# tangjiapeng/DiffuScene

Hardware: AMD Instinct MI355X
Metric: denoiser steps/sec (train + 1000-step sample) at B=256, N=80 objects (higher is better)
Workload: dtype f32 (operands split 3xbf16, 6 products, f32 accumulate); 1 GPU; uncond living/dining rooms (config/uncond/diffusion_livingrooms_instancond_lat32_v.yaml scaled to N=80), B=256 scenes per GPU, N=80, C=65, T=1000, mode=both; global_batch=256, parallelism=single

## Files before the change

__graft_entry__.py:

```python
import os
import subprocess
import sys

ROOT = os.path.dirname(os.path.abspath(__file__))
CSRC = os.path.join(ROOT, "diffuscene_amd", "csrc")
LIB = os.path.join(ROOT, "diffuscene_amd", "libdiffuscene_hip.so")

SOURCES = [
    ("gemm_mfma.hip", []),
    ("gemm_split.hip", ["-fno-slp-vectorize"]),
    ("gemm_tn_split.hip", ["-fno-slp-vectorize"]),
    ("blocks.hip", []),
    ("diffusion.hip", ["-ffp-contract=off"]),
    ("train.hip", []),
    ("retrieval.hip", ["-ffp-contract=off"]),
    ("dataset.hip", ["-ffp-contract=off"]),
    ("chamfer.hip", ["-ffp-contract=off"]),
    ("optim.hip", ["-ffp-contract=off"]),
    ("foldingnet.hip", []),
]


def _hipcc():
    for c in (os.environ.get("HIPCC"), "/opt/rocm/bin/hipcc", "hipcc"):
        if c and (os.path.isabs(c) and os.path.exists(c) or not os.path.isabs(c)):
            return c
    raise RuntimeError("hipcc not found")


def _stale(target, deps):
    if not os.path.exists(target):
        return True
    t = os.path.getmtime(target)
    return any(os.path.getmtime(d) > t for d in deps)


def _stamp_git_head():
    try:
        head = subprocess.check_output(["git", "rev-parse", "--short", "HEAD"], cwd=ROOT, stderr=subprocess.DEVNULL, text=True).strip()
        dirty = subprocess.check_output(["git", "status", "--porcelain", "-uno"], cwd=ROOT, stderr=subprocess.DEVNULL, text=True).strip()
        with open(os.path.join(ROOT, "GIT_HEAD"), "w") as f:
            f.write(head + ("+" if dirty else "") + "\n")
    except Exception:
        pass


def build(force=False):
    hipcc = _hipcc()
    headers = [os.path.join(CSRC, "dsc_common.h"), os.path.join(CSRC, "gemm_core.h"), os.path.join(CSRC, "gemm_tn_split.h"),
               os.path.join(ROOT, "include", "diffuscene_hip.h")]
    objs = []
    for src, extra in SOURCES:
        s = os.path.join(CSRC, src)
        if not os.path.exists(s):
            continue
        o = os.path.join(CSRC, src.replace(".hip", ".o"))
        if force or _stale(o, [s] + headers):
            cmd = [hipcc, "--offload-arch=gfx950", "-O3", "-std=c++17", "-fPIC", "-c", s, "-o", o] + extra
            subprocess.check_call(cmd)
        objs.append(o)
    if force or _stale(LIB, objs):
        subprocess.check_call([hipcc, "--offload-arch=gfx950", "-shared", "-fPIC", "-o", LIB] + objs)
    gsrc = os.path.join(ROOT, "tools", "guard_alloc.cpp")
    gso = os.path.join(ROOT, "tools", "_build", "libdsc_guard_alloc.so")
    if os.path.exists(gsrc) and (force or _stale(gso, [gsrc])):
        os.makedirs(os.path.dirname(gso), exist_ok=True)
        try:
            subprocess.check_call([hipcc, "-O2", "-std=c++17", "-fPIC", "-shared", gsrc, "-o", gso])
        except (subprocess.CalledProcessError, OSError) as e:
            print("warning: guard allocator (tools/guard_alloc.cpp) not built: %s -- tests/test_gpu_guard.py will skip its allocator runs" % e,
                  file=sys.stderr)
    _stamp_git_head()
    if ROOT not in sys.path:
        sys.path.insert(0, ROOT)
    import diffuscene_amd
    from diffuscene_amd import _lib
    _lib.load()
    import oracle.ref_torch


def build_asan():
    hipcc = _hipcc()
    out = os.path.join(ROOT, "diffuscene_amd", "libdiffuscene_hip_asan.so")
    objs = []
    for src, extra in SOURCES:
        s = os.path.join(CSRC, src)
        o = os.path.join(CSRC, src.replace(".hip", ".asan.o"))
        subprocess.check_call([hipcc, "--offload-arch=gfx950", "-O1", "-g", "-std=c++17", "-fPIC", "-fsanitize=address", "-fno-gpu-sanitize",
                               "-shared-libsan", "-Wno-option-ignored", "-c", s, "-o", o] + extra)
        objs.append(o)
    subprocess.check_call([hipcc, "--offload-arch=gfx950", "-shared", "-fPIC", "-fsanitize=address", "-fno-gpu-sanitize", "-shared-libsan",
                           "-Wno-option-ignored", "-o", out] + objs)
    return out


def smoke():
    if ROOT not in sys.path:
        sys.path.insert(0, ROOT)
    import torch
    assert torch.cuda.is_available(), "smoke() needs a GPU"
    from diffuscene_amd.networks.denoise_net import Unet1D
    from diffuscene_amd.networks.diffusion_ddpm import DiffusionPoint
    from oracle import ref_torch as R
    from oracle import weights as W

    kw = dict(W.UNCOND_BEDROOM)
    B, N = 4, 12
    dev = torch.device("cuda:0")
    net = Unet1D(**kw)
    sd = W.synth_state_dict(kw)
    net.load_state_dict(sd)
    net.to(dev)
    cfg = dict(objectness_dim=0, class_dim=22, angle_dim=2, objfeat_dim=32)
    diff = DiffusionPoint(net, cfg, time_num=1000, model_mean_type="v")
    x = W.synth_scene_batch(B, N, 22, 32, 0)
    t = torch.tensor([3, 250, 600, 999], dtype=torch.int64)
    cond = W.synth_condition(B, N, 128, 0).contiguous()
    noise = W.synth_noise((B, N, 62), 7)
    with torch.no_grad():
        out = net(x.to(dev), t.to(dev), cond.to(dev), None).cpu()
        ref = R.unet1d_forward(sd, kw, x, t, cond, None)
        rel = float((out - ref).abs().max() / ref.abs().max())
        assert rel < 1e-4, "Unet1D forward mismatch vs oracle: %g" % rel
        tb = R.schedule_tables(1e-4, 0.02, 1000, "v")
        step = diff.diffusion.p_sample(diff._denoise, x.to(dev), t.to(dev), cond.to(dev), None,
                                       noise_fn=lambda size, dtype, device: noise.to(device), clip_denoised=True).cpu()
        ref_step = R.p_sample_step(tb, x, t, ref, noise, True, "v")
        rel2 = float((step - ref_step).abs().max() / ref_step.abs().max())
        assert rel2 < 1e-4, "p_sample mismatch vs oracle: %g" % rel2
    print("smoke ok: forward rel err %.3g, p_sample rel err %.3g" % (rel, rel2))


if __name__ == "__main__":
    if "--asan" in sys.argv:
        print("built", build_asan())
        sys.exit(0)
    build(force="--force" in sys.argv)
    if "--smoke" in sys.argv:
        smoke()
```

diffuscene_amd/_lib.py:

```python
import ctypes as C
import os

_HERE = os.path.dirname(os.path.abspath(__file__))
LIB_PATH = os.path.join(_HERE, "libdiffuscene_hip.so")
if os.environ.get("DSC_HIP_LIB"):
    LIB_PATH = os.path.abspath(os.environ["DSC_HIP_LIB"])

ACT_NONE, ACT_GELU, ACT_SILU, ACT_LEAKY01 = 0, 1, 2, 3
SS_NONE, SS_PER_TOKEN, SS_PER_SCENE, SS_PER_SLOT, SS_BY_INDEX = 0, 1, 2, 3, 4
MEAN_EPS, MEAN_X0, MEAN_V = 0, 1, 2
TILE_GN_80_W8, TILE_GN_80_W4, TILE_160x256, TILE_160x128_W4 = 1, 2, 5, 8
TILE_WAVE_GN, TILE_WAVE_DENSE, TILE_WAVE_GN_64 = 10, 11, 12
F32_TILE_160x256, F32_TILE_160x128, F32_TILE_128x128, F32_TILE_96x128, F32_TILE_64x64 = 0, 1, 2, 3, 4
DSC_PLANES_NONE = -100
GEMM_ROW_INVARIANT = 1
WS_MAX = 64
MAX_TOKENS_PER_SCENE = 160
STATS_MAX_OBJECTS, STATS_ONE_WAVE_MAX = 160, 32

_ERR = {-1: "DSC_EINVAL (bad shape / null pointer)", -2: "DSC_EALIGN (16-byte alignment required)",
        -3: "DSC_ERANGE (size outside kernel limits)"}

c_f32p = C.c_void_p
c_i64p = C.c_void_p


class GemmArgs(C.Structure):
    _fields_ = [
        ("a1", C.c_void_p), ("lda1", C.c_int64), ("k1", C.c_int32),
        ("a2", C.c_void_p), ("lda2", C.c_int64), ("k2", C.c_int32),
        ("w", C.c_void_p), ("ldw", C.c_int64),
        ("bias", C.c_void_p),
        ("residual", C.c_void_p), ("ldr", C.c_int64),
        ("y", C.c_void_p), ("ldy", C.c_int64),
        ("m", C.c_int32), ("n", C.c_int32),
        ("act_in", C.c_int32), ("act_out", C.c_int32),
        ("batch", C.c_int32),
        ("sa1", C.c_int64), ("sa2", C.c_int64), ("sw", C.c_int64), ("sbias", C.c_int64),
        ("sres", C.c_int64), ("sy", C.c_int64),
        ("gamma", C.c_void_p), ("beta", C.c_void_p), ("eps", C.c_float),
        ("tokens_per_scene", C.c_int32),
        ("scale_shift", C.c_void_p), ("ld_ss", C.c_int64), ("ss_mode", C.c_int32),
        ("preact", C.c_void_p), ("ld_preact", C.c_int64),
        ("ss_index", C.c_void_p),
        ("w_planes", C.c_void_p),
        ("actgrad_x", C.c_void_p), ("ld_actgrad", C.c_int64),
        ("ss_rows", C.c_int32),
        ("w_planes_layout", C.c_int32),
        ("gnb_z", C.c_void_p), ("ld_gnb_z", C.c_int64),
        ("gnb_dgamma", C.c_void_p), ("gnb_dbeta", C.c_void_p), ("gnb_dbias", C.c_void_p), ("gnb_pstride", C.c_int64),
        ("gnb_dss", C.c_void_p), ("ld_gnb_dss", C.c_int64),
        ("flags", C.c_int32),
    ]


class SplitItem(C.Structure):
    _fields_ = [("w", C.c_void_p), ("ldw", C.c_int64), ("rows", C.c_int32), ("cols", C.c_int32), ("planes", C.c_void_p),
                ("transpose", C.c_int32)]


class SmallKItem(C.Structure):
    _fields_ = [("x", C.c_void_p), ("ldx", C.c_int64), ("k_in", C.c_int32), ("w", C.c_void_p), ("ldw", C.c_int64), ("bias", C.c_void_p),
                ("y", C.c_void_p), ("ldy", C.c_int64)]


class ColSpan(C.Structure):
    _fields_ = [("src_col", C.c_int32), ("dst_col", C.c_int32), ("width", C.c_int32)]


SMALLK_MAX = 4


class WsItem(C.Structure):
    _fields_ = [("w", C.c_void_p), ("out", C.c_void_p), ("rows", C.c_int32), ("cols", C.c_int32)]


class TnGroup(C.Structure):
    _fields_ = [("a1", C.c_void_p), ("lda1", C.c_int64), ("k1", C.c_int32),
                ("a2", C.c_void_p), ("lda2", C.c_int64), ("k2", C.c_int32),
                ("dy", C.c_void_p), ("ldd", C.c_int64),
                ("out", C.c_void_p), ("ldo", C.c_int64),
                ("dbias", C.c_void_p),
                ("m", C.c_int32), ("n", C.c_int32), ("kvalid", C.c_int32),
                ("tile0", C.c_int32),
                ("ws_offset", C.c_int64),
                ("tile0s", C.c_int32)]


class ColsumItem(C.Structure):
    _fields_ = [("x", C.c_void_p), ("ldx", C.c_int64), ("m", C.c_int32), ("n", C.c_int32), ("out", C.c_void_p)]


class WsBwdItem(C.Structure):
    _fields_ = [("w", C.c_void_p), ("dw_std", C.c_void_p), ("dw", C.c_void_p), ("rows", C.c_int32), ("cols", C.c_int32)]


SIGNATURES = {
    "dsc_version": (C.c_int, []),
    "dsc_gemm_f32": (C.c_int, [C.POINTER(GemmArgs), C.c_void_p]),
    "dsc_gemm_gn_silu_f32": (C.c_int, [C.POINTER(GemmArgs), C.c_void_p]),
    "dsc_split_bf16x3_f32": (C.c_int, [C.POINTER(SplitItem), C.c_int32, C.c_void_p]),
    "dsc_gemm_arithmetic": (C.c_int, [C.POINTER(GemmArgs), C.c_int32]),
    "dsc_gemm_split_tile": (C.c_int, [C.POINTER(GemmArgs), C.c_int32]),
    "dsc_gemm_f32_tile": (C.c_int, [C.POINTER(GemmArgs)]),
    "dsc_gemm_planes_layout": (C.c_int, [C.POINTER(GemmArgs), C.c_int32]),
    "dsc_get_split_wave": (C.c_int, []),
    "dsc_set_split_wave": (C.c_int, [C.c_int32]),
    "dsc_gemm_skinny": (C.c_int, [C.POINTER(GemmArgs), C.c_int32]),
    "dsc_get_skinny": (C.c_int, []),
    "dsc_set_skinny": (C.c_int, [C.c_int32]),
    "dsc_get_gemm_arithmetic": (C.c_int, []),
    "dsc_set_gemm_arithmetic": (C.c_int, [C.c_int32]),
    "dsc_gemm_layernorm_f32": (C.c_int, [C.POINTER(GemmArgs), C.c_void_p]),
    "dsc_gemm_splitk_f32": (C.c_int, [C.POINTER(GemmArgs), C.c_int32, c_f32p, C.c_int64, C.c_void_p]),
    "dsc_linear_smallk_f32": (C.c_int, [c_f32p, C.c_int64, C.c_int32, c_f32p, C.c_int64, c_f32p, c_f32p, C.c_int64,
                                        C.c_int32, C.c_int32, C.c_int32, C.c_void_p]),
    "dsc_linear_smallk_grouped_f32": (C.c_int, [C.POINTER(SmallKItem), C.c_int32, C.c_int32, C.c_int32, C.c_int32, C.c_void_p]),
    "dsc_gather_columns_f32": (C.c_int, [c_f32p, C.c_int64, c_f32p, C.c_int64, C.c_int32, C.POINTER(ColSpan), C.c_int32, C.c_void_p]),
    "dsc_weight_standardize_f32": (C.c_int, [C.POINTER(WsItem), C.c_int32, C.c_float, C.c_void_p]),
    "dsc_layernorm_f32": (C.c_int, [c_f32p, C.c_int64, c_f32p, c_f32p, C.c_int64, c_f32p, C.c_int64, C.c_int32,
                                    C.c_int32, C.c_float, C.c_void_p]),
    "dsc_linear_attention_f32": (C.c_int, [c_f32p, C.c_int64, c_f32p, C.c_int64, c_f32p, C.c_int64, c_f32p, C.c_int64,
                                           C.c_int32, C.c_int32, C.c_int32, C.c_float, C.c_void_p]),
    "dsc_attention_f32": (C.c_int, [c_f32p, C.c_int64, c_f32p, C.c_int64, c_f32p, C.c_int64, c_f32p, C.c_int64,
                                    C.c_int32, C.c_int32, C.c_float, C.c_void_p]),
    "dsc_time_embedding_f32": (C.c_int, [c_i64p, C.c_int32, C.c_int32, c_f32p, C.c_int32, c_f32p, c_f32p, C.c_void_p]),
    "dsc_activation_f32": (C.c_int, [c_f32p, c_f32p, C.c_int64, C.c_int32, C.c_void_p]),
    "dsc_q_sample_f32": (C.c_int, [c_f32p, c_f32p, c_i64p, c_f32p, c_f32p, c_f32p, c_f32p, C.c_int32, C.c_int64, C.c_int32,
                                   C.c_void_p]),
    "dsc_p_sample_f32": (C.c_int, [c_f32p, c_f32p, c_f32p, c_i64p, c_f32p, c_f32p, c_f32p, c_f32p, c_f32p, c_f32p,
                                   c_f32p, C.c_int32, C.c_int32, C.c_int32, C.c_int64, C.c_int32, C.c_void_p]),
    "dsc_device_error_count": (C.c_int64, [C.c_int32]),
    "dsc_add_scalar_i64": (C.c_int, [c_i64p, C.c_int32, C.c_int64, C.c_void_p]),
    "dsc_ddim_step_f32": (C.c_int, [c_f32p, c_f32p, c_f32p, c_i64p, c_i64p, c_i64p, c_f32p, c_f32p, c_f32p, c_f32p, c_f32p,
                                    c_f32p, c_f32p, c_f32p, c_f32p, C.c_int32, C.c_int32, C.c_int64, C.c_int32, C.c_int32,
                                    C.c_void_p]),
    "dsc_ddim_advance_i64": (C.c_int, [c_i64p, c_i64p, c_i64p, C.c_int32, C.c_int32, C.c_void_p]),
    "dsc_knn16_f32": (C.c_int, [c_f32p, C.c_int64, C.c_int32, c_f32p, c_f32p, C.c_int32, C.c_int32, C.c_void_p, C.c_void_p]),
    "dsc_rowsq_f32": (C.c_int, [c_f32p, C.c_int64, C.c_int32, C.c_int64, c_f32p, C.c_void_p]),
    "dsc_knn_cov_f32": (C.c_int, [c_f32p, C.c_int64, C.c_void_p, C.c_int32, C.c_int32, c_f32p, C.c_int64, C.c_void_p]),
    "dsc_gather_max_f32": (C.c_int, [c_f32p, C.c_int64, C.c_void_p, C.c_int32, C.c_int32, C.c_int32, c_f32p, C.c_int64,
                                     C.c_void_p, C.c_void_p]),
    "dsc_gather_max_bwd_f32": (C.c_int, [c_f32p, C.c_int64, C.c_void_p, C.c_void_p, C.c_int32, C.c_int32, C.c_int32, c_f32p,
                                         C.c_int64, C.c_void_p]),
    "dsc_bn_workspace_floats": (C.c_int64, [C.c_int64, C.c_int32]),
    "dsc_batchnorm_fwd_f32": (C.c_int, [c_f32p, C.c_int64, c_f32p, c_f32p, C.c_int64, C.c_int32, C.c_float, C.c_float,
                                        C.c_int32, c_f32p, c_f32p, c_f32p, c_f32p, c_f32p, c_f32p, c_f32p, C.c_int64,
                                        C.c_void_p]),
    "dsc_batchnorm_eval_f32": (C.c_int, [c_f32p, C.c_int64, c_f32p, c_f32p, c_f32p, c_f32p, C.c_int64, C.c_int32, C.c_int32,
                                         c_f32p, C.c_void_p]),
    "dsc_batchnorm_bwd_f32": (C.c_int, [c_f32p, c_f32p, c_f32p, c_f32p, c_f32p, C.c_int64, C.c_int32, C.c_int32, c_f32p,
                                        c_f32p, c_f32p, c_f32p, C.c_int64, C.c_void_p]),
    "dsc_rowmax_f32": (C.c_int, [c_f32p, C.c_int64, C.c_int32, C.c_int32, C.c_int32, c_f32p, C.c_void_p, C.c_void_p]),
    "dsc_rowmax_bwd_f32": (C.c_int, [c_f32p, C.c_void_p, C.c_int32, C.c_int32, C.c_int32, c_f32p, C.c_void_p]),
    "dsc_point_affine_f32": (C.c_int, [c_f32p, C.c_int64, C.c_int32, c_f32p, C.c_int64, c_f32p, C.c_int32, C.c_int32,
                                       C.c_int32, C.c_int32, c_f32p, C.c_void_p]),
    "dsc_point_affine_bwd_f32": (C.c_int, [c_f32p, c_f32p, C.c_int64, C.c_int32, c_f32p, C.c_int64, C.c_int32, C.c_int32,
                                           C.c_int32, C.c_int32, c_f32p, C.c_int64, c_f32p, C.c_int64, c_f32p, c_f32p,
                                           C.c_int64, C.c_void_p]),
    "dsc_postfilter_compact_f32": (C.c_int, [c_f32p, C.c_int32, C.c_int32, C.c_int32, C.c_int32, C.c_int32, C.c_int32, c_f32p,
                                             C.c_void_p, C.c_void_p]),
    "dsc_gemm_tn_f32": (C.c_int, [c_f32p, C.c_int64, C.c_int32, c_f32p, C.c_int64, C.c_int32, c_f32p, C.c_int64, c_f32p,
                                  C.c_int64, c_f32p, C.c_int32, C.c_int32, C.c_int32, c_f32p, C.c_int64, C.c_void_p]),
    "dsc_gemm_tn_workspace_floats": (C.c_int64, [C.c_int32, C.c_int32, C.c_int32]),
    "dsc_gemm_tn_grouped_f32": (C.c_int, [C.c_void_p, C.c_int32, C.c_int32, C.c_int32, c_f32p, C.c_int64, C.c_int64,
                                          C.c_void_p]),
    "dsc_gemm_tn_grouped_split_f32": (C.c_int, [C.c_void_p, C.c_int32, C.c_int32, C.c_void_p, C.c_int32, C.c_int32, c_f32p, C.c_int64,
                                                C.c_int64, C.c_int32, C.c_void_p]),
    "dsc_set_tn_split_form": (C.c_int, [C.c_int32]),
    "dsc_get_tn_split_form": (C.c_int, []),
    "dsc_colsum_f32": (C.c_int, [c_f32p, C.c_int64, C.c_int32, C.c_int32, c_f32p, c_f32p, C.c_int64, C.c_void_p]),
    "dsc_colsum_grouped_f32": (C.c_int, [C.c_void_p, C.c_int32, C.c_int32, C.c_void_p]),
    "dsc_gn_silu_bwd_f32": (C.c_int, [c_f32p, C.c_int64, c_f32p, C.c_int64, c_f32p, c_f32p, c_f32p, C.c_int64, C.c_int32,
                                      c_f32p, C.c_int64, c_f32p, c_f32p, c_f32p, C.c_int64, c_f32p, C.c_int64, C.c_int32,
                                      C.c_int32, C.c_int32, C.c_float, C.c_void_p]),
    "dsc_weight_standardize_bwd_f32": (C.c_int, [C.POINTER(WsBwdItem), C.c_int32, C.c_float, C.c_void_p]),
    "dsc_layernorm_bwd_f32": (C.c_int, [c_f32p, C.c_int64, c_f32p, c_f32p, C.c_int64, c_f32p, C.c_int64, c_f32p, C.c_int64, c_f32p,
                                        C.c_int32, C.c_int32, C.c_int32, C.c_float, C.c_void_p]),
    "dsc_linear_attention_bwd_f32": (C.c_int, [c_f32p, C.c_int64] * 7 + [C.c_int32, C.c_int32, C.c_int32, C.c_float,
                                                                          C.c_void_p]),
    "dsc_attention_bwd_f32": (C.c_int, [c_f32p, C.c_int64] * 7 + [C.c_int32, C.c_int32, C.c_float, C.c_void_p]),
    "dsc_retrieve_nearest_f32": (C.c_int, [c_f32p, C.c_void_p, C.c_void_p, c_f32p, C.c_void_p, C.c_void_p, C.c_int32,
                                           C.c_int32, C.c_int32, C.c_void_p, c_f32p, C.c_void_p]),
    "dsc_box_bounds_f32": (C.c_int, [c_f32p, c_f32p, c_f32p, C.c_void_p, C.c_int32, C.c_int32, c_f32p, C.c_void_p]),
    "dsc_scene_stats_f32": (C.c_int, [c_f32p, c_f32p, C.c_void_p, C.c_void_p, C.c_int32, C.c_int32, C.c_int32, C.c_int32,
                                      C.c_void_p, C.c_void_p, C.c_void_p, C.c_void_p, C.c_void_p, C.c_void_p, c_f32p, C.c_void_p]),
    "dsc_encode_scene_batch_f32": (C.c_int, [c_i64p, c_f32p, c_f32p, c_f32p, c_f32p, c_f32p, C.c_int32, C.c_int32, c_i64p,
                                             C.c_void_p, C.c_void_p, C.c_void_p, C.c_int32, C.POINTER(C.c_double), c_f32p,
                                             C.c_int64, c_i64p, C.c_int32, C.c_int32, C.c_void_p]),
    "dsc_chamfer3d_forward_f32": (C.c_int, [c_f32p, c_f32p, c_f32p, c_f32p, C.c_void_p, C.c_void_p, C.c_int32, C.c_int32,
                                            C.c_int32, C.c_void_p]),
    "dsc_chamfer3d_backward_f32": (C.c_int, [c_f32p, c_f32p, c_f32p, c_f32p, C.c_void_p, C.c_void_p, c_f32p, c_f32p,
                                             C.c_int32, C.c_int32, C.c_int32, C.c_void_p]),
    "dsc_grad_sumsq_f32": (C.c_int, [C.c_void_p, C.c_int32, C.c_void_p, C.c_void_p]),
    "dsc_clip_coef_f32": (C.c_int, [C.c_void_p, C.c_int32, C.c_float, c_f32p, c_f32p, C.c_void_p]),
    "dsc_adam_step_f32": (C.c_int, [C.c_void_p, C.c_int32, C.c_float, C.c_float, C.c_float, C.c_float, C.c_float, C.c_float,
                                    c_f32p, C.c_void_p]),
    "dsc_ddpm_loss_f32": (C.c_int, [c_f32p, c_f32p, c_f32p, c_i64p, c_f32p, c_f32p, c_f32p, c_f32p, C.POINTER(C.c_float),
                                    c_f32p, c_f32p, c_f32p] + [C.c_int32] * 12 + [C.c_float, C.c_int32, C.c_void_p]),
    "dsc_copy2d_f32": (C.c_int, [c_f32p, C.c_int64, c_f32p, C.c_int64, C.c_int32, C.c_int32, C.c_void_p]),
    "dsc_add2d_f32": (C.c_int, [c_f32p, C.c_int64, c_f32p, C.c_int64, C.c_int32, C.c_int32, C.c_void_p]),
    "dsc_activation_bwd_f32": (C.c_int, [c_f32p, c_f32p, c_f32p, C.c_int64, C.c_int32, C.c_void_p]),
    "dsc_transpose_batched_f32": (C.c_int, [C.POINTER(WsItem), C.c_int32, C.c_void_p]),
    "dsc_transpose_f32": (C.c_int, [c_f32p, C.c_int64, c_f32p, C.c_int64, C.c_int32, C.c_int32, C.c_void_p]),
    "dsc_complete_overwrite_f32": (C.c_int, [c_f32p, c_f32p, c_f32p, c_i64p, c_f32p, c_f32p, C.c_int32, C.c_int32,
                                             C.c_int32, C.c_int32, C.c_int32, C.c_void_p]),
    "dsc_complete_overwrite_ragged_f32": (C.c_int, [c_f32p, c_f32p, c_f32p, c_i64p, c_i64p, c_f32p, c_f32p, C.c_int32, C.c_int32,
                                                    C.c_int32, C.c_int32, C.c_int32, C.c_void_p]),
    "dsc_p_sample_inpaint_f32": (C.c_int, [c_f32p, c_f32p, c_f32p, c_f32p, c_f32p, c_i64p, c_i64p, c_f32p, c_f32p, c_f32p, c_f32p,
                                           c_f32p, c_f32p, c_f32p, c_f32p] + [C.c_int32] * 7 + [C.c_void_p]),
    "dsc_ddim_inpaint_step_f32": (C.c_int, [c_f32p] * 5 + [c_i64p] * 4 + [c_f32p] * 10 + [C.c_int32] * 7 + [C.c_void_p]),
    "dsc_masked_overwrite_f32": (C.c_int, [c_f32p, c_f32p, c_f32p, C.c_void_p, c_i64p, c_f32p, c_f32p, C.c_int32, C.c_int64, C.c_int32,
                                           C.c_void_p]),
    "dsc_p_sample_masked_f32": (C.c_int, [c_f32p] * 5 + [C.c_void_p, c_i64p] + [c_f32p] * 8 + [C.c_int32] * 3 + [C.c_int64, C.c_int32,
                                                                                                                  C.c_void_p]),
    "dsc_ddim_masked_step_f32": (C.c_int, [c_f32p] * 5 + [C.c_void_p] + [c_i64p] * 3 + [c_f32p] * 10 + [C.c_int32] * 2 +
                                 [C.c_int64, C.c_int32, C.c_int32, C.c_void_p]),
    "dsc_cfg_combine_f32": (C.c_int, [c_f32p, c_f32p, c_f32p, C.c_int32, C.c_int64, C.c_void_p]),
    "dsc_scene_randn_f32": (C.c_int, [c_f32p, c_i64p, c_i64p, C.c_int64, C.c_int64, C.c_int64, C.c_void_p]),
    "dsc_scene_philox_u32": (C.c_int, [C.c_void_p, c_i64p, c_i64p, C.c_int64, C.c_int64, C.c_int64, C.c_void_p]),
    "dsc_p_sample_cfg_f32": (C.c_int, [c_f32p] * 4 + [c_i64p] + [c_f32p] * 8 + [C.c_int32] * 3 + [C.c_int64, C.c_int32, C.c_void_p]),
    "dsc_ddim_cfg_step_f32": (C.c_int, [c_f32p] * 4 + [c_i64p] * 3 + [c_f32p] * 10 + [C.c_int32] * 2 +
                              [C.c_int64, C.c_int32, C.c_int32, C.c_void_p]),
    "dsc_scene_gate_f32": (C.c_int, [c_f32p, C.c_void_p, c_f32p, C.c_int32, C.c_int64, C.c_void_p]),
}

_lib = None


class HipLibraryMissing(RuntimeError):
    pass


def load():
    global _lib
    if _lib is not None:
        return _lib
    if not os.path.exists(LIB_PATH):
        raise HipLibraryMissing(
            "%s not found: build it with `python __graft_entry__.py` (hipcc --offload-arch=gfx950). "
            "diffuscene_amd has no CPU or PyTorch fallback." % LIB_PATH)
    import torch
    lib = C.CDLL(LIB_PATH)
    for name, (res, args) in SIGNATURES.items():
        try:
            fn = getattr(lib, name)
        except AttributeError as e:
            raise HipLibraryMissing("symbol %s missing from %s" % (name, LIB_PATH)) from e
        fn.restype = res
        fn.argtypes = args
    if lib.dsc_get_gemm_arithmetic() < 0:
        raise ValueError("DSC_GEMM=%r: must be 'split' (default) or 'f32'" % os.environ.get("DSC_GEMM"))
    if lib.dsc_get_tn_split_form() < 0:
        raise ValueError("DSC_TN_FORM=%r: must be '2' (default), '1' or '0'" % os.environ.get("DSC_TN_FORM"))
    if lib.dsc_get_split_wave() < 0:
        raise ValueError("DSC_WAVE=%r: must be '1' / 'auto' (default) or '0'" % os.environ.get("DSC_WAVE"))
    _lib = lib
    return lib


def split_enabled():
    return load().dsc_get_gemm_arithmetic() == 1


def gemm_mode():
    lib = load()
    if lib.dsc_get_gemm_arithmetic() != 1:
        return 0
    return (2 if lib.dsc_get_split_wave() == 1 else 1) + 10 * lib.dsc_get_tn_split_form()


def set_split_wave(on):
    prev = load().dsc_get_split_wave() == 1
    check(load().dsc_set_split_wave(1 if on else 0), "dsc_set_split_wave")
    return prev


def set_gemm_arithmetic(name):
    if name not in ("split", "f32"):
        raise ValueError("gemm arithmetic must be 'split' or 'f32', got %r" % (name,))
    prev = "split" if split_enabled() else "f32"
    check(load().dsc_set_gemm_arithmetic(1 if name == "split" else 0), "dsc_set_gemm_arithmetic")
    return prev


def device_error_count(reset=False):
    n = load().dsc_device_error_count(1 if reset else 0)
    if n < 0:
        raise RuntimeError("dsc_device_error_count failed (HIP error)")
    return int(n)


def check_indices(where):
    if os.environ.get("DSC_CHECK_INDICES", "0") == "1":
        n = device_error_count(reset=True)
        if n:
            raise IndexError("%s: %d out-of-range device timestep(s) were clamped into the schedule tables" % (where, n))


def check(rc, what):
    if rc != 0:
        raise RuntimeError("%s failed: %s" % (what, _ERR.get(rc, "hipError_t %d" % rc)))


def fn(name):
    return getattr(load(), name)
```

diffuscene_amd/csrc/gemm_mfma.hip:

```cpp
#include "gemm_core.h"
#include "gemm_skinny.h"
#include <cstdlib>

namespace {

using dsc_gemm::gemm_kernel;
constexpr int BK = 32;

int check_common(const dsc_gemm_args* a) {
    if (!a || !a->a1 || !a->w || !a->y) return DSC_EINVAL;
    if (a->m <= 0 || a->n <= 0 || a->k1 <= 0 || a->k2 < 0) return DSC_EINVAL;
    if ((a->k1 % BK) || (a->k2 % BK)) return DSC_EINVAL;
    if (a->k2 > 0 && !a->a2) return DSC_EINVAL;
    if (a->batch < 1) return DSC_EINVAL;
    if (!dsc_aligned16(a->a1) || (a->lda1 & 3) || !dsc_aligned16(a->w) || (a->ldw & 3)) return DSC_EALIGN;
    if (a->k2 > 0 && (!dsc_aligned16(a->a2) || (a->lda2 & 3))) return DSC_EALIGN;
    if (a->batch > 1 && ((a->sa1 & 3) || (a->sa2 & 3) || (a->sw & 3))) return DSC_EALIGN;
    if (a->act_in != DSC_ACT_NONE) return DSC_EINVAL;
    if (a->act_out < DSC_ACT_NONE || a->act_out > DSC_ACT_SILU) return DSC_EINVAL;
    return 0;
}

template <int TM, int TN, int WM, int WN, bool GN, int IL>
int launch_il(const dsc_gemm_args* a, int rows_per_blk, hipStream_t s) {
    constexpr int BN = 32 * TN * WN;
    const int nrb = (a->m + rows_per_blk - 1) / rows_per_blk;
    const int ncb = (a->n + BN - 1) / BN;
    dim3 grid((unsigned)(nrb * ncb), (unsigned)a->batch);
    DSC_CLEAR_STALE_ERROR();
    hipLaunchKernelGGL((gemm_kernel<TM, TN, WM, WN, GN, IL>), grid, dim3(64 * WM * WN), 0, s, *a, ncb);
    DSC_LAUNCH_CHECK();
    return 0;
}

template <int TM, int TN, int WM, int WN, bool GN, int IL = 1>
int launch(const dsc_gemm_args* a, int rows_per_blk, hipStream_t s) {
    if constexpr (IL == 0) {
        return launch_il<TM, TN, WM, WN, GN, 0>(a, rows_per_blk, s);
    } else {
        const int64_t ld_max = a->lda1 > a->ldw ? a->lda1 : a->ldw;
        const bool dma = (a->k2 == 0 || a->lda1 == a->lda2) && ld_max * 4 * (32 * TM * WM + 32 * TN * WN) < (int64_t(1) << 31);
        return dma ? launch_il<TM, TN, WM, WN, GN, 2>(a, rows_per_blk, s) : launch_il<TM, TN, WM, WN, GN, 1>(a, rows_per_blk, s);
    }
}

__global__ void splitk_reduce_kernel(const float* __restrict__ slabs, long slab, int nslab, const float* __restrict__ bias,
                                     const float* __restrict__ residual, long ldr, float* __restrict__ out, long ldo, int m, int n) {
    const long total = (long)m * n;
    for (long i = (long)blockIdx.x * blockDim.x + threadIdx.x; i < total; i += (long)gridDim.x * blockDim.x) {
        const int r = (int)(i / n), c = (int)(i - (long)r * n);
        float acc = 0.f;
        for (int s2 = 0; s2 < nslab; ++s2) acc += slabs[(long)s2 * slab + i];
        if (bias) acc += bias[c];
        if (residual) acc += residual[(long)r * ldr + c];
        out[(long)r * ldo + c] = acc;
    }
}

int g_skinny = -1;

int skinny_enabled() {
    if (g_skinny < 0) {
        const char* e = std::getenv("DSC_SKINNY");
        g_skinny = (e && e[0] == '0') ? 0 : 1;
    }
    return g_skinny;
}

struct SkinnyPlan { int rows_per_blk, ng, nrb, ncb; bool r16; };

bool skinny_plan(const dsc_gemm_args* a, bool gn, SkinnyPlan* out) {
    if (!skinny_enabled() || (a->flags & DSC_GEMM_ROW_INVARIANT)) return false;
    const int K = a->k1 + a->k2;
    if ((K % 64) || (a->n % 64)) return false;
    if (a->k2 > 0 && (a->k1 % (K / dsc_skinny::NW))) return false;
    if (a->preact && !gn) return false;
    if (a->actgrad_x || a->gnb_z) return false;
    int unit = 1;
    if (gn) {
        if (a->batch != 1) return false;
        unit = a->tokens_per_scene;
        if (unit > 32) return false;
    }
    const int ncb = a->n / 64;
    int rpb = 0;
    int64_t nrb = 0;
    bool r16 = false;
    for (int rows = ((K % 512) == 0 && unit <= 16) ? 16 : 32; rows <= 32 && !rpb; rows += 16) {
        int r = (rows / unit) * unit;
        if (r > a->m) r = (int)(((int64_t)a->m + unit - 1) / unit * unit);
        if (rows == 16 && r > 16) continue;
        const int64_t nb = ((int64_t)a->m + r - 1) / r;
        if (nb * ncb * a->batch <= 256) { rpb = r; nrb = nb; r16 = rows == 16; }
    }
    if (!rpb) return false;
    auto al = [](const void* q) { return !q || dsc_aligned16(q); };
    if (!al(a->y) || !al(a->residual) || !al(a->bias) || !al(a->preact) || !al(a->gamma) || !al(a->beta) || !al(a->scale_shift)) return false;
    if ((a->ldy & 3) || (a->residual && (a->ldr & 3)) || (a->preact && (a->ld_preact & 3)) || (a->scale_shift && (a->ld_ss & 3))) return false;
    if (a->batch > 1 && ((a->sy & 3) || (a->sres & 3) || (a->sbias & 3))) return false;
    out->rows_per_blk = rpb;
    out->r16 = r16;
    out->ng = (K % 512) == 0 ? dsc_skinny::STAGED : K <= 256 ? 1 : K <= 512 ? 2 : K <= 1024 ? 4 : 0;
    out->nrb = (int)nrb;
    out->ncb = ncb;
    return true;
}

template <bool GN, int NG, bool R16 = false>
int launch_skinny_ng(const dsc_gemm_args* a, const SkinnyPlan& sp, hipStream_t s) {
    static bool attr_set = false;
    if (!attr_set) {
        hipError_t e = hipFuncSetAttribute(reinterpret_cast<const void*>(dsc_skinny::gemm_skinny_kernel<GN, NG, R16>),
                                           hipFuncAttributeMaxDynamicSharedMemorySize, (int)dsc_skinny::lds_bytes<NG>());
        if (e != hipSuccess) return (int)e;
        attr_set = true;
    }
    DSC_CLEAR_STALE_ERROR();
    hipLaunchKernelGGL((dsc_skinny::gemm_skinny_kernel<GN, NG, R16>), dim3((unsigned)(sp.nrb * sp.ncb), (unsigned)a->batch),
                       dim3(64 * dsc_skinny::NW), dsc_skinny::lds_bytes<NG>(), s, *a, sp.ncb, sp.rows_per_blk);
    DSC_LAUNCH_CHECK();
    return 0;
}

template <bool GN>
int launch_skinny(const dsc_gemm_args* a, const SkinnyPlan& sp, hipStream_t s) {
    if (sp.r16) return launch_skinny_ng<GN, dsc_skinny::STAGED, true>(a, sp, s);
    switch (sp.ng) {
        case 1: return launch_skinny_ng<GN, 1>(a, sp, s);
        case 2: return launch_skinny_ng<GN, 2>(a, sp, s);
        case 4: return launch_skinny_ng<GN, 4>(a, sp, s);
        case dsc_skinny::STAGED: return launch_skinny_ng<GN, dsc_skinny::STAGED>(a, sp, s);
        default: return launch_skinny_ng<GN, 0>(a, sp, s);
    }
}

}

extern "C" int dsc_get_skinny(void) { return skinny_enabled(); }
extern "C" int dsc_set_skinny(int32_t on) { const int prev = skinny_enabled(); g_skinny = on ? 1 : 0; return prev; }
extern "C" int dsc_gemm_skinny(const dsc_gemm_args* a, int32_t gn) {
    if (check_common(a) || dsc_gemm_arithmetic(a, gn)) return 0;
    SkinnyPlan sp;
    return skinny_plan(a, gn != 0, &sp) ? (sp.r16 ? 2 : 1) : 0;
}

static long tile_cost(long m_rows, int rows_per_blk, int n, int bm, int bn) {
    const long nblk = ((m_rows + rows_per_blk - 1) / rows_per_blk) * ((n + bn - 1) / bn);
    return ((nblk + 255) / 256) * (long)bm * bn;
}

static int select_f32_tile(const dsc_gemm_args* a) {
    if (a->flags & DSC_GEMM_ROW_INVARIANT) return DSC_F32_TILE_64x64;
    const bool wide = (a->n % 256) == 0;
    struct Cand { int bm, bn, id; };
    const Cand cands[5] = {{160, 128, DSC_F32_TILE_160x128}, {160, 256, DSC_F32_TILE_160x256}, {128, 128, DSC_F32_TILE_128x128},
                           {96, 128, DSC_F32_TILE_96x128}, {64, 64, DSC_F32_TILE_64x64}};
    int best = -1;
    long best_cost = 0;
    for (int i = 0; i < 5; ++i) {
        if (cands[i].id == DSC_F32_TILE_160x256 && !wide) continue;
        const long c = tile_cost(a->m, cands[i].bm, a->n, cands[i].bm, cands[i].bn) * a->batch;
        if (best < 0 || c < best_cost) { best = cands[i].id; best_cost = c; }
    }
    return best;
}

extern "C" int dsc_gemm_f32_tile(const dsc_gemm_args* a) {
    const int rc = check_common(a);
    return rc ? rc : select_f32_tile(a);
}

extern "C" int dsc_gemm_f32(const dsc_gemm_args* a, dsc_stream_t stream) {
    int rc = check_common(a);
    if (rc) return rc;
    hipStream_t s = static_cast<hipStream_t>(stream);
    rc = dsc_gemm_try_split(a, false, s);
    if (rc != DSC_SPLIT_NOT_TAKEN) return rc;
    if (a->preact || a->actgrad_x || a->gnb_z) return DSC_EINVAL;
    {
        SkinnyPlan sp;
        if (skinny_plan(a, false, &sp)) return launch_skinny<false>(a, sp, s);
    }
    switch (select_f32_tile(a)) {
        case DSC_F32_TILE_160x256: return launch<5, 1, 1, 8, false>(a, 160, s);
        case DSC_F32_TILE_160x128: return launch<5, 1, 1, 4, false>(a, 160, s);
        case DSC_F32_TILE_128x128: return launch<2, 2, 2, 2, false>(a, 128, s);
        case DSC_F32_TILE_96x128: return launch<3, 1, 1, 4, false>(a, 96, s);
        default: return launch<1, 1, 2, 2, false, 0>(a, 64, s);
    }
}

extern "C" int dsc_gemm_gn_silu_f32(const dsc_gemm_args* a, dsc_stream_t stream) {
    int rc = check_common(a);
    if (rc) return rc;
    if (!a->gamma || !a->beta || !a->bias) return DSC_EINVAL;
    const int N = a->tokens_per_scene;
    if (N < 4 || N > 160) return DSC_ERANGE;
    if (a->m % N) return DSC_EINVAL;
    if (a->n % 128) return DSC_EINVAL;
    if (a->act_in != DSC_ACT_NONE) return DSC_EINVAL;
    if (!dsc_aligned16(a->gamma) || !dsc_aligned16(a->beta)) return DSC_EALIGN;
    if (a->preact && (!dsc_aligned16(a->preact) || (a->ld_preact & 3))) return DSC_EALIGN;
    if (a->ss_mode != DSC_SS_NONE) {
        if (!a->scale_shift) return DSC_EINVAL;
        if (!dsc_aligned16(a->scale_shift) || (a->ld_ss & 3)) return DSC_EALIGN;
        if (a->ss_mode < DSC_SS_NONE || a->ss_mode > DSC_SS_BY_INDEX) return DSC_EINVAL;
        if (a->ss_mode == DSC_SS_BY_INDEX && (!a->ss_index || a->ss_rows < 1)) return DSC_EINVAL;
    } else if (a->scale_shift) return DSC_EINVAL;
    hipStream_t s = static_cast<hipStream_t>(stream);
    rc = dsc_gemm_try_split(a, true, s);
    if (rc != DSC_SPLIT_NOT_TAKEN) return rc;
    {
        SkinnyPlan sp;
        if (skinny_plan(a, true, &sp)) return launch_skinny<true>(a, sp, s);
    }
    struct Cand { int bm, bn; };
    const Cand cands[5] = {{160, 128}, {160, 256}, {128, 128}, {96, 128}, {64, 64}};
    int best = -1;
    long best_cost = 0;
    const bool per_scene_ss = a->ss_mode == DSC_SS_PER_SCENE || a->ss_mode == DSC_SS_BY_INDEX;
    for (int pass = 0; pass < 2 && best < 0; ++pass)
        for (int i = 0; i < 5; ++i) {
            if (cands[i].bm < N) continue;
            if (cands[i].bn == 256 && (a->n % 256)) continue;
            if (pass == 0 && per_scene_ss && cands[i].bm / N > ((cands[i].bm == 160 && cands[i].bn == 128) ? 4 : 8)) continue;
            const int rpb = (cands[i].bm / N) * N;
            const long c = tile_cost(a->m, rpb, a->n, cands[i].bm, cands[i].bn);
            if (best < 0 || c < best_cost) { best = i; best_cost = c; }
        }
    if (best < 0) return DSC_ERANGE;
    const int rpb = (cands[best].bm / N) * N;
    switch (best) {
        case 0: return launch<5, 1, 1, 4, true>(a, rpb, s);
        case 1: return launch<5, 1, 1, 8, true>(a, rpb, s);
        case 2: return launch<2, 2, 2, 2, true>(a, rpb, s);
        case 3: return launch<3, 1, 1, 4, true>(a, rpb, s);
        default: return launch<1, 1, 2, 2, true, 0>(a, rpb, s);
    }
}

extern "C" int dsc_gemm_splitk_f32(const dsc_gemm_args* a, int32_t splits, float* workspace, int64_t workspace_floats,
                                   dsc_stream_t stream) {
    int rc = check_common(a);
    if (rc) return rc;
    if (splits < 2 || splits > 64 || !workspace) return DSC_EINVAL;
    if (a->batch != 1 || a->k2 != 0 || a->act_out != DSC_ACT_NONE) return DSC_EINVAL;
    if (a->k1 % (BK * splits)) return DSC_EINVAL;
    if (workspace_floats < (int64_t)splits * a->m * a->n) return DSC_EINVAL;
    if ((reinterpret_cast<uintptr_t>(workspace) & 15) || (((int64_t)a->m * a->n) & 3)) return DSC_EALIGN;
    dsc_gemm_args p = *a;
    const int kc = a->k1 / splits;
    p.k1 = kc;
    p.batch = splits;
    p.sa1 = kc; p.sw = kc; p.sa2 = 0; p.sbias = 0; p.sres = 0;
    p.bias = nullptr; p.residual = nullptr;
    p.y = workspace; p.ldy = a->n; p.sy = (int64_t)a->m * a->n;
    rc = dsc_gemm_f32(&p, stream);
    if (rc) return rc;
    const long total = (long)a->m * a->n;
    long blocks = (total + 255) / 256;
    if (blocks > 2048) blocks = 2048;
    DSC_CLEAR_STALE_ERROR();
    hipLaunchKernelGGL(splitk_reduce_kernel, dim3((unsigned)blocks), dim3(256), 0, static_cast<hipStream_t>(stream), workspace,
                       (long)a->m * a->n, splits, a->bias, a->residual, (long)a->ldr, a->y, (long)a->ldy, a->m, a->n);
    DSC_LAUNCH_CHECK();
    return 0;
}

extern "C" int dsc_gemm_layernorm_f32(const dsc_gemm_args* a, dsc_stream_t stream) {
    int rc = check_common(a);
    if (rc) return rc;
    if (a->n != 512 || a->batch != 1 || a->act_out != DSC_ACT_NONE || !a->gamma) return DSC_EINVAL;
    if (!dsc_aligned16(a->gamma) || !dsc_aligned16(a->y) || (a->ldy & 3)) return DSC_EALIGN;
    if (a->residual && (!dsc_aligned16(a->residual) || (a->ldr & 3))) return DSC_EALIGN;
    if (a->bias && !dsc_aligned16(a->bias)) return DSC_EALIGN;
    const int64_t ld_max = a->lda1 > a->ldw ? a->lda1 : a->ldw;
    if (!(a->k2 == 0 || a->lda1 == a->lda2) || ld_max * 4 * (96 + 512) >= (int64_t(1) << 31)) return DSC_ERANGE;
    const int nrb = (a->m + 95) / 96;
    DSC_CLEAR_STALE_ERROR();
    hipLaunchKernelGGL((gemm_kernel<3, 2, 1, 8, false, 2, 0, true>), dim3((unsigned)nrb, 1), dim3(512), 0,
                       static_cast<hipStream_t>(stream), *a, 1);
    DSC_LAUNCH_CHECK();
    return 0;
}
```

diffuscene_amd/csrc/gemm_split.hip:

```cpp
#include "dsc_common.h"
#include "gemm_split_wave.h"
#include <atomic>
#include <cstring>

#ifndef DSC_SPLIT_DSPREAD
#define DSC_SPLIT_DSPREAD true
#endif

namespace dsc_split {

typedef unsigned u32x4 __attribute__((ext_vector_type(4)));
typedef __bf16 bf16x8 __attribute__((ext_vector_type(8)));
typedef __bf16 bf16x2 __attribute__((ext_vector_type(2)));

constexpr int BK = 32;

__device__ __forceinline__ unsigned cvt_pk_bf16(float a, float b) {
    f32x2 v = {a, b};
    return __builtin_bit_cast(unsigned, __builtin_convertvector(v, bf16x2));
}
__device__ __forceinline__ float bf_lo(unsigned p) { return __builtin_bit_cast(float, p << 16); }
__device__ __forceinline__ float bf_hi(unsigned p) { return __builtin_bit_cast(float, p & 0xffff0000u); }

__device__ __forceinline__ void split8(const f32x4 lo, const f32x4 hi, bf16x8& p1, bf16x8& p2, bf16x8& p3) {
// ... 246 lines not shown
            if constexpr (DSPREAD) {
                if (i * PER < NI) {
#pragma unroll
                    for (int q = 0; q < PER; ++q) {
                        __builtin_amdgcn_sched_group_barrier(0x008, 2, 0);
                        __builtin_amdgcn_sched_group_barrier(0x020, 1, 0);
                    }
                }
            }
            if (i >= RB - NIT) {
#pragma unroll
                for (int q = 0; q < NMMA - 2; ++q) {
                    __builtin_amdgcn_sched_group_barrier(0x008, 1, 0);
                    __builtin_amdgcn_sched_group_barrier(0x002, (44 + NMMA - 3) / (NMMA - 2), 0);
                }
                __builtin_amdgcn_sched_group_barrier(0x008, 1, 0);
                __builtin_amdgcn_sched_group_barrier(0x200, 3, 0);
            }
            __builtin_amdgcn_sched_barrier(0);
        }
    }
    __builtin_amdgcn_s_waitcnt(0x0f70);

    const int cbase = col0 + wn * 64 + 4 * g;
    const int srow = wm * ntok;
    bool valid[RB];
#pragma unroll
    for (int i = 0; i < RB; ++i) valid[i] = i * 16 + l15 < ntok && srow + i * 16 + l15 < rows_here;
    float* const ob = p.y + (int64_t)z * p.sy + (int64_t)(row0 + srow + l15) * p.ldy + cbase;
    const float* const rbp = p.residual ? p.residual + (int64_t)z * p.sres + (int64_t)(row0 + srow + l15) * p.ldr + cbase : nullptr;
    if constexpr (!GN) {
        float* const ub = p.preact ? p.preact + (int64_t)z * p.sy + (int64_t)(row0 + srow + l15) * p.ld_preact + cbase : nullptr;
        const float* const gb = p.actgrad_x ? p.actgrad_x + (int64_t)z * p.sy + (int64_t)(row0 + srow + l15) * p.ld_actgrad + cbase : nullptr;
#pragma unroll
        for (int i = 0; i < RB; ++i) {
            if (valid[i]) {
#pragma unroll
                for (int j = 0; j < 4; ++j) {
                    f32x4 y = acc[i][j];
                    if (ub) *reinterpret_cast<f32x4*>(ub + (int64_t)i * 16 * p.ld_preact + j * 16) = y;
                    if (gb) {
                        const f32x4 u = *reinterpret_cast<const f32x4*>(gb + (int64_t)i * 16 * p.ld_actgrad + j * 16);
#pragma unroll
                        for (int e = 0; e < 4; ++e) y[e] *= dsc_act_grad(u[e], p.act_out);
                    } else if (p.act_out != DSC_ACT_NONE) {
#pragma unroll
                        for (int e = 0; e < 4; ++e) y[e] = dsc_act(y[e], p.act_out);
                    }
                    if (rbp) y += *reinterpret_cast<const f32x4*>(rbp + (int64_t)i * 16 * p.ldr + j * 16);
                    *reinterpret_cast<f32x4*>(ob + (int64_t)i * 16 * p.ldy + j * 16) = y;
                }
            }
        }
    } else {
        const int scene = min(row0 / ntok + wm, p.m / ntok - 1);
        const bool per_row = p.ss_mode == DSC_SS_PER_TOKEN || p.ss_mode == DSC_SS_PER_SLOT;
        f32x4 ga[4], be[4], sc[4], sh[4];
        int64_t ssrow = scene;
        if (p.ss_mode == DSC_SS_BY_INDEX) ssrow = dsc_clamp_index(p.ss_index[scene], p.ss_rows);
#pragma unroll
        for (int j = 0; j < 4; ++j) {
            ga[j] = *reinterpret_cast<const f32x4*>(p.gamma + cbase + j * 16);
            be[j] = *reinterpret_cast<const f32x4*>(p.beta + cbase + j * 16);
            if (p.ss_mode == DSC_SS_PER_SCENE || p.ss_mode == DSC_SS_BY_INDEX) {
                const float* ssr = p.scale_shift + ssrow * p.ld_ss + cbase + j * 16;
                sc[j] = *reinterpret_cast<const f32x4*>(ssr);
                sh[j] = *reinterpret_cast<const f32x4*>(ssr + p.n);
            } else {
                sc[j] = f32x4{0.f, 0.f, 0.f, 0.f};
                sh[j] = sc[j];
            }
        }
        if (p.preact) {
            float* const pb = p.preact + (int64_t)(row0 + srow + l15) * p.ld_preact + cbase;
#pragma unroll
            for (int i = 0; i < RB; ++i)
                if (valid[i]) {
#pragma unroll
                    for (int j = 0; j < 4; ++j) *reinterpret_cast<f32x4*>(pb + (int64_t)i * 16 * p.ld_preact + j * 16) = acc[i][j];
                }
        }
        const float inv_cnt = 1.f / (float)(ntok * 64);
        float s0 = 0.f;
#pragma unroll
        for (int i = 0; i < RB; ++i)
#pragma unroll
            for (int j = 0; j < 4; ++j)
                s0 += valid[i] ? (acc[i][j][0] + acc[i][j][1]) + (acc[i][j][2] + acc[i][j][3]) : 0.f;
        const float mean = wave_sum_dpp(s0) * inv_cnt;
        float q0 = 0.f;
#pragma unroll
        for (int i = 0; i < RB; ++i)
#pragma unroll
            for (int j = 0; j < 4; ++j)
#pragma unroll
                for (int e = 0; e < 4; ++e) {
                    const float d = valid[i] ? acc[i][j][e] - mean : 0.f;
                    q0 = fmaf(d, d, q0);
                }
        const float rstd = 1.f / sqrtf(wave_sum_dpp(q0) * inv_cnt + p.eps);
#pragma unroll
        for (int j = 0; j < 4; ++j)
#pragma unroll
            for (int e = 0; e < 4; ++e) {
                const float a = rstd * ga[j][e], sp1 = sc[j][e] + 1.f;
                ga[j][e] = a * sp1;
                be[j][e] = fmaf(be[j][e] - mean * a, sp1, sh[j][e]);
            }
#pragma unroll
        for (int i = 0; i < RB; ++i) {
            if (valid[i]) {
#pragma unroll
                for (int j = 0; j < 4; ++j) {
                    f32x4 y, s1 = {1.f, 1.f, 1.f, 1.f}, s2 = {0.f, 0.f, 0.f, 0.f};
                    if (per_row) {
                        const int64_t row = p.ss_mode == DSC_SS_PER_TOKEN ? (int64_t)row0 + srow + i * 16 + l15 : (int64_t)i * 16 + l15;
                        const float* ssr = p.scale_shift + row * p.ld_ss + cbase + j * 16;
                        s1 = *reinterpret_cast<const f32x4*>(ssr) + 1.f;
                        s2 = *reinterpret_cast<const f32x4*>(ssr + p.n);
                    }
#pragma unroll
                    for (int e = 0; e < 4; ++e) {
                        float t = fmaf(acc[i][j][e], ga[j][e], be[j][e]);
                        if (per_row) t = fmaf(t, s1[e], s2[e]);
                        y[e] = dsc_silu_fast(t);
                    }
                    if (rbp) y += *reinterpret_cast<const f32x4*>(rbp + (int64_t)i * 16 * p.ldr + j * 16);
                    *reinterpret_cast<f32x4*>(ob + (int64_t)i * 16 * p.ldy + j * 16) = y;
                }
            }
        }
    }
}

template <bool GN, int WM, int WN, int RB, bool DSPREAD = DSC_SPLIT_DSPREAD>
__global__ __launch_bounds__(64 * WM * WN, 1) void gemm_split_kernel(const dsc_gemm_args p, const int ntok) {
    __shared__ __attribute__((aligned(16))) char smem[split_smem_bytes<WM, WN, RB>()];
    gemm_split_tile<GN, WM, WN, RB, DSPREAD>(p, ntok, blockIdx.x, blockIdx.y, smem);
}

template <bool GN, int WM, int WN, int RB>
int launch(const dsc_gemm_args* a, int ntok, hipStream_t s) {
    constexpr int BN = 64 * WN;
    const int scenes = (a->m + ntok - 1) / ntok;
    const unsigned grid = (unsigned)(((scenes + WM - 1) / WM) * (a->n / BN));
    DSC_CLEAR_STALE_ERROR();
    hipLaunchKernelGGL((gemm_split_kernel<GN, WM, WN, RB>), dim3(grid, (unsigned)a->batch), dim3(64 * WM * WN), 0, s, *a, ntok);
    DSC_LAUNCH_CHECK();
    return 0;
}

}

enum { T_GN_32 = 0, T_GN_80_W8, T_GN_80_W4, T_GN_48, T_GN_64, T_160x256, T_256x128, T_128x128, T_160x128_W4, T_64x256, T_WAVE_GN, T_WAVE_DENSE, T_WAVE_GN_64 };

static std::atomic<int> g_gemm_arith{-1000};

extern "C" int dsc_get_gemm_arithmetic(void) {
    int m = g_gemm_arith.load(std::memory_order_relaxed);
    if (m == -1000) {
        const char* e = getenv("DSC_GEMM");
        m = (!e || !e[0] || !strcmp(e, "split")) ? 1 : !strcmp(e, "f32") ? 0 : DSC_EINVAL;
        g_gemm_arith.store(m, std::memory_order_relaxed);
    }
    return m;
}

extern "C" int dsc_set_gemm_arithmetic(int32_t mode) {
    if (mode != 0 && mode != 1) return DSC_EINVAL;
    g_gemm_arith.store(mode, std::memory_order_relaxed);
    return 0;
}

static std::atomic<int> g_split_wave{-1000};

extern "C" int dsc_get_split_wave(void) {
    int m = g_split_wave.load(std::memory_order_relaxed);
    if (m == -1000) {
        const char* e = getenv("DSC_WAVE");
        m = (!e || !e[0] || !strcmp(e, "1") || !strcmp(e, "auto")) ? 1 : !strcmp(e, "0") ? 0 : DSC_EINVAL;
        g_split_wave.store(m, std::memory_order_relaxed);
    }
    return m;
}

extern "C" int dsc_set_split_wave(int32_t mode) {
    if (mode != 0 && mode != 1) return DSC_EINVAL;
    g_split_wave.store(mode, std::memory_order_relaxed);
    return 0;
}

static int select_wave(const dsc_gemm_args* a, bool gn) {
    if (dsc_get_split_wave() != 1) return -1;
    const int K = a->k1 + a->k2;
    if ((a->n % 128) || (a->k1 % 64) || (a->k2 % 64) || K < 256) return -1;
    if (a->batch != 1 && (gn || a->sw != (int64_t)a->n * K || a->ldw != K || (a->sy & 3) || (a->sres & 3) || (a->sbias & 3))) return -1;
    if (!dsc_aligned16(a->y) || (a->ldy & 3) || a->ldy < a->n) return -1;
    if (a->bias && !dsc_aligned16(a->bias)) return -1;
    if (a->residual && (!dsc_aligned16(a->residual) || (a->ldr & 3) || a->ldr < a->n)) return -1;
    if (a->preact && (!dsc_aligned16(a->preact) || (a->ld_preact & 3) || a->ld_preact < a->n || a->batch != 1)) return -1;
    if (a->actgrad_x && (gn || !dsc_aligned16(a->actgrad_x) || (a->ld_actgrad & 3) || a->ld_actgrad < a->n || a->batch != 1)) return -1;
    if (3LL * a->batch * a->n * K * 2 >= 0x7fffffffLL) return -1;
    const int64_t ld_max = a->lda1 > a->lda2 ? a->lda1 : a->lda2;
    if (ld_max * 4 * 96 >= 0x7fffffffLL) return -1;
    long waves;
    if (a->gnb_z) {
        const int N = a->tokens_per_scene;
        if (gn || a->batch != 1 || N <= 64 || N > 80 || (a->m % N) || a->bias || a->residual || a->preact || a->actgrad_x || a->act_out != DSC_ACT_NONE) return -1;
        if (!a->gamma || !a->beta || !a->gnb_dgamma || !a->gnb_dbeta || !a->gnb_dbias || (a->ss_mode != DSC_SS_NONE && a->ss_mode != DSC_SS_PER_SCENE)) return -1;
        if (!dsc_aligned16(a->gnb_z) || (a->ld_gnb_z & 3) || a->ld_gnb_z < a->n || !dsc_aligned16(a->gamma) || !dsc_aligned16(a->beta)) return -1;
        if (!dsc_aligned16(a->gnb_dgamma) || !dsc_aligned16(a->gnb_dbeta) || !dsc_aligned16(a->gnb_dbias) || (a->gnb_pstride & 3)) return -1;
        if (a->ss_mode == DSC_SS_PER_SCENE && (!a->scale_shift || !dsc_aligned16(a->scale_shift) || (a->ld_ss & 3))) return -1;
        if (a->gnb_dss && (!dsc_aligned16(a->gnb_dss) || (a->ld_gnb_dss & 3))) return -1;
        waves = (long)(a->m / N) * (a->n / 128);
        const long r = (waves + 1023) / 1024;
        return waves * 5 >= r * 1024 * 4 ? T_WAVE_DENSE : -1;
    }
    if (gn) {
        const int N = a->tokens_per_scene;
        if (N <= 16 || N > 80) return -1;
        const bool perrow = a->ss_mode == DSC_SS_PER_TOKEN || a->ss_mode == DSC_SS_PER_SLOT;
        if (perrow && a->ld_ss < 2 * (int64_t)a->n) return -1;
        waves = (long)(a->m / N) * (a->n / 128);
    } else {
        waves = (long)((a->m + 79) / 80) * (a->n / 128) * a->batch;
    }
    const long rounds = (waves + 1023) / 1024;
    if (waves * 5 >= rounds * 1024 * 4) return gn ? T_WAVE_GN : T_WAVE_DENSE;
    if (gn && a->tokens_per_scene > 64) {
        const long w4 = 2 * waves, r4 = (w4 + 1023) / 1024;
        if (r4 == 1 && w4 * 5 >= 1024 * 4) return T_WAVE_GN_64;
    }
    return -1;
}

static int select_block_tile(const dsc_gemm_args* a, bool gn);

static int select_tile(const dsc_gemm_args* a, bool gn, bool assume_planes = false) {
    if (dsc_get_gemm_arithmetic() != 1 || (!assume_planes && !a->w_planes)) return -1;
    if (a->flags & DSC_GEMM_ROW_INVARIANT) return -1;
    const int w = select_wave(a, gn);
    return w >= 0 ? w : select_block_tile(a, gn);
}

static int select_block_tile(const dsc_gemm_args* a, bool gn) {
    if (a->gnb_z) return -1;
    const int K = a->k1 + a->k2;
    if (a->batch != 1 && (gn || a->sw != (int64_t)a->n * K || a->ldw != K || (a->sy & 3) || (a->sres & 3) || (a->sbias & 3))) return -1;
    if ((a->n % 128) || (K % 32)) return -1;
    if (!dsc_aligned16(a->w_planes) || !dsc_aligned16(a->y) || (a->ldy & 3)) return -1;
    if (a->bias && !dsc_aligned16(a->bias)) return -1;
    if (a->residual && (!dsc_aligned16(a->residual) || (a->ldr & 3))) return -1;
    if (!gn && a->preact && (!dsc_aligned16(a->preact) || (a->ld_preact & 3) || a->batch != 1)) return -1;
    if (a->actgrad_x && (gn || !dsc_aligned16(a->actgrad_x) || (a->ld_actgrad & 3) || a->batch != 1)) return -1;
    if (3LL * a->batch * a->n * K * 2 >= 0x7fffffffLL) return -1;
    const int64_t ld_max = a->lda1 > a->lda2 ? a->lda1 : a->lda2;
    if (ld_max * 4 * 320 >= 0x7fffffffLL) return -1;
    const bool wide = (a->n % 256) == 0;
    constexpr long MIN_BLOCKS = 160;
    if (gn) {
        const int N = a->tokens_per_scene;
        if (N <= 16 || N > 80) return -1;
        const long S = a->m / N;
        if (N <= 32) return ((S + 3) / 4) * (a->n / 128) >= MIN_BLOCKS ? T_GN_32 : -1;
        const long b8 = wide ? ((S + 1) / 2) * (a->n / 256) : 0, b4 = ((S + 1) / 2) * (a->n / 128);
        if (N > 64) return b8 >= MIN_BLOCKS + 32 ? T_GN_80_W8 : b4 >= MIN_BLOCKS ? T_GN_80_W4 : -1;
        if (b8 < MIN_BLOCKS) return -1;
        return N <= 48 ? T_GN_48 : T_GN_64;
    }
    struct Cand { int bm, bn, id; };
    const Cand cands[5] = {{160, 256, T_160x256}, {256, 128, T_256x128}, {160, 128, T_160x128_W4}, {128, 128, T_128x128}, {64, 256, T_64x256}};
    int best = -1;
    long best_cost = 0, best_blk = 0;
    for (int i = 0; i < 5; ++i) {
        if (cands[i].bn == 256 && !wide) continue;
        const long nblk = (long)((a->m + cands[i].bm - 1) / cands[i].bm) * (a->n / cands[i].bn) * a->batch;
        const long c = ((nblk + 255) / 256) * (long)cands[i].bm * cands[i].bn;
        if (best < 0 || c < best_cost) { best = cands[i].id; best_cost = c; best_blk = nblk; }
    }
    return best_blk >= MIN_BLOCKS ? best : -1;
}

int dsc_gemm_try_split(const dsc_gemm_args* a, bool gn, hipStream_t s) {
    using namespace dsc_split;
    if (dsc_get_gemm_arithmetic() < 0 || dsc_get_split_wave() < 0) return DSC_EINVAL;
    const int N = a->tokens_per_scene;
    const int tile = select_tile(a, gn);
    if (tile < 0) return DSC_SPLIT_NOT_TAKEN;
    const int want = (tile == T_WAVE_GN || tile == T_WAVE_DENSE || tile == T_WAVE_GN_64) ? DSC_PLANES_FRAGMENT : DSC_PLANES_ROWMAJOR;
    if (a->w_planes_layout != want) return DSC_EINVAL;
    switch (tile) {
        case T_GN_32: return launch<true, 4, 2, 2>(a, N, s);
        case T_GN_80_W8: return launch<true, 2, 4, 5>(a, N, s);
        case T_GN_80_W4: return launch<true, 2, 2, 5>(a, N, s);
        case T_GN_48: return launch<true, 2, 4, 3>(a, N, s);
        case T_GN_64: return launch<true, 2, 4, 4>(a, N, s);
        case T_160x256: return launch<false, 2, 4, 5>(a, 80, s);
        case T_256x128: return launch<false, 4, 2, 4>(a, 64, s);
        case T_128x128: return launch<false, 4, 2, 2>(a, 32, s);
        case T_160x128_W4: return launch<false, 2, 2, 5>(a, 80, s);
        case T_64x256: return launch<false, 2, 4, 2>(a, 32, s);
        case T_WAVE_DENSE:
            if (a->gnb_z) return dsc_wave::launch<false, 5, false, 8, true>(a, a->w_planes, N, s);
            return dsc_wave::launch<false, 5>(a, a->w_planes, 80, s);
        case T_WAVE_GN_64:
            return (a->ss_mode == DSC_SS_PER_TOKEN || a->ss_mode == DSC_SS_PER_SLOT) ? dsc_wave::launch<true, 5, true, 4>(a, a->w_planes, N, s)
                                                                                     : dsc_wave::launch<true, 5, false, 4>(a, a->w_planes, N, s);
        case T_WAVE_GN: {
            const bool perrow = a->ss_mode == DSC_SS_PER_TOKEN || a->ss_mode == DSC_SS_PER_SLOT;
            const int rb = (N + 15) / 16;
            if (perrow) {
                return rb == 5 ? dsc_wave::launch<true, 5, true>(a, a->w_planes, N, s) : rb == 4 ? dsc_wave::launch<true, 4, true>(a, a->w_planes, N, s)
                     : rb == 3 ? dsc_wave::launch<true, 3, true>(a, a->w_planes, N, s) : dsc_wave::launch<true, 2, true>(a, a->w_planes, N, s);
            }
            return rb == 5 ? dsc_wave::launch<true, 5>(a, a->w_planes, N, s) : rb == 4 ? dsc_wave::launch<true, 4>(a, a->w_planes, N, s)
                 : rb == 3 ? dsc_wave::launch<true, 3>(a, a->w_planes, N, s) : dsc_wave::launch<true, 2>(a, a->w_planes, N, s);
        }
        default: return DSC_SPLIT_NOT_TAKEN;
    }
}

extern "C" int dsc_gemm_arithmetic(const dsc_gemm_args* a, int32_t gn) {
    if (!a || a->m <= 0 || a->n <= 0 || a->k1 <= 0) return DSC_EINVAL;
    return select_tile(a, gn != 0) >= 0 ? 1 : 0;
}

extern "C" int dsc_gemm_split_tile(const dsc_gemm_args* a, int32_t gn) {
    if (!a || a->m <= 0 || a->n <= 0 || a->k1 <= 0) return DSC_EINVAL;
    return select_tile(a, gn != 0);
}

extern "C" int dsc_gemm_planes_layout(const dsc_gemm_args* a, int32_t gn) {
    if (!a || a->m <= 0 || a->n <= 0 || a->k1 <= 0) return DSC_EINVAL;
    const int tile = select_tile(a, gn != 0, true);
    return tile < 0 ? DSC_PLANES_NONE : (tile == T_WAVE_GN || tile == T_WAVE_DENSE || tile == T_WAVE_GN_64) ? DSC_PLANES_FRAGMENT : DSC_PLANES_ROWMAJOR;
}

extern "C" int dsc_split_bf16x3_f32(const dsc_split_item* items, int32_t count, dsc_stream_t stream) {
    using namespace dsc_split;
    if (!items || count < 1 || count > DSC_WS_MAX) return DSC_EINVAL;
    SplitBatch b;
    long max_items = 0;
    for (int i = 0; i < count; ++i) {
        const dsc_split_item& it = items[i];
        if (!it.w || !it.planes || it.rows <= 0 || it.cols <= 0) return DSC_EINVAL;
        if (it.transpose & ~(DSC_SPLIT_TRANSPOSE | DSC_SPLIT_FRAGMENT)) return DSC_EINVAL;
        const bool tr = (it.transpose & DSC_SPLIT_TRANSPOSE) != 0;
        const int co = tr ? it.rows : it.cols, ro = tr ? it.cols : it.rows;
        if (co % 8) return DSC_EINVAL;
        if ((it.transpose & DSC_SPLIT_FRAGMENT) && ((ro % 16) || (co % 32))) return DSC_EINVAL;
        if (!dsc_aligned16(it.planes) || (!tr && (!dsc_aligned16(it.w) || (it.ldw & 3)))) return DSC_EALIGN;
        b.it[i] = it;
        const long n = (long)it.rows * it.cols / 8;
        if (n > max_items) max_items = n;
    }
    long bx = (max_items + 255) / 256;
    if (bx > 1024) bx = 1024;
    DSC_CLEAR_STALE_ERROR();
    hipLaunchKernelGGL(split_planes_kernel, dim3((unsigned)bx, (unsigned)count), dim3(256), 0, static_cast<hipStream_t>(stream), b);
    DSC_LAUNCH_CHECK();
    return 0;
}
```

diffuscene_amd/csrc/gemm_split_wave.h:

```cpp
#pragma once
#include "dsc_common.h"
#include <utility>

#ifndef DSC_WAVE_STAMP_ARGS
#define DSC_WAVE_STAMP_ARGS
#define DSC_WAVE_STAMP_PASS
#define DSC_WAVE_STAMP_DECL
#define DSC_WAVE_STAMP_KERNEL(id)
#define DSC_WAVE_STAMP_TILE(id)
#define DSC_WAVE_STAMP_FLUSH(kt)
#define DSC_WAVE_STAMP_END
#endif

namespace dsc_wave {

typedef unsigned u32x4 __attribute__((ext_vector_type(4)));
typedef __bf16 bf16x8 __attribute__((ext_vector_type(8)));
typedef __bf16 bf16x2 __attribute__((ext_vector_type(2)));

constexpr int BK = 32;
constexpr int WAVES = 4;

__device__ __forceinline__ unsigned cvt_pk_bf16(float a, float b) {
    f32x2 v = {a, b};
    return __builtin_bit_cast(unsigned, __builtin_convertvector(v, bf16x2));
}
__device__ __forceinline__ float bf_lo(unsigned p) { return __builtin_bit_cast(float, p << 16); }
__device__ __forceinline__ float bf_hi(unsigned p) { return __builtin_bit_cast(float, p & 0xffff0000u); }

__device__ __forceinline__ void split8(const f32x4 lo, const f32x4 hi, bf16x8& p1, bf16x8& p2, bf16x8& p3) {
    u32x4 a, b, c;
#pragma unroll
    for (int q = 0; q < 4; ++q) {
        const float x0 = q < 2 ? lo[2 * q] : hi[2 * q - 4], x1 = q < 2 ? lo[2 * q + 1] : hi[2 * q - 3];
        const unsigned u1 = cvt_pk_bf16(x0, x1);
        const float r0 = x0 - bf_lo(u1), r1 = x1 - bf_hi(u1);
        const unsigned u2 = cvt_pk_bf16(r0, r1);
        const float s0 = r0 - bf_lo(u2), s1 = r1 - bf_hi(u2);
        a[q] = u1;
        b[q] = u2;
        c[q] = cvt_pk_bf16(s0, s1);
    }
    p1 = __builtin_bit_cast(bf16x8, a);
    p2 = __builtin_bit_cast(bf16x8, b);
    p3 = __builtin_bit_cast(bf16x8, c);
}

template <int RB>
constexpr int wave_smem_bytes() { return WAVES * 2 * 3 * (16 * RB) * 64; }

template <bool GN, int RB, bool PERROW = false, int J = 8, bool GB = false>
__global__ __launch_bounds__(64 * WAVES, 1) void gemm_split_wave_kernel(const dsc_gemm_args p, const uint16_t* const planes_f, const int ntok DSC_WAVE_STAMP_ARGS) {
    static_assert(J == 8 || J == 4, "wave tile: 128 or 64 channels");
    static_assert(!GB || (!GN && J == 8), "the GroupNorm-backward epilogue rides on the dense 80 x 128 form");
    constexpr int NWF = 3 * J;
    constexpr int CW = 16 * J;
    constexpr int ROWS = 16 * RB, XP = ROWS * 64, STAGE = 3 * XP;
    constexpr int NWB = RB > 4 ? RB - 2 : RB > 3 ? RB - 1 : RB;
    constexpr int PERW = (NWF + NWB - 1) / NWB;
    __shared__ __attribute__((aligned(16))) char smem[wave_smem_bytes<RB>()];
    const int lane = threadIdx.x & 63;
    const int wave = __builtin_amdgcn_readfirstlane(threadIdx.x >> 6);
    const int K = p.k1 + p.k2, KT = K / BK;
    const int scenes = (p.m + ntok - 1) / ntok;
    const int sgs = (scenes + WAVES - 1) / WAVES, chunks = p.n / CW;
    const int bid = blockIdx.x;
    int sg, ch;
    if ((sgs & 7) == 0) {
        const int xcd = bid & 7, idx = bid >> 3;
        sg = xcd * (sgs >> 3) + idx / chunks;
        ch = idx % chunks;
    } else {
        sg = bid / chunks;
        ch = bid % chunks;
    }
    const int scene = sg * WAVES + wave;
    if (scene >= scenes) return;
    DSC_WAVE_STAMP_DECL
    DSC_WAVE_STAMP_KERNEL(0)
    const int z = blockIdx.y;
    const int row0 = scene * ntok, col0 = ch * CW;
    const int rows_here = min(ntok, p.m - row0);
    const float* const xb1 = p.a1 + (int64_t)z * p.sa1 + (int64_t)row0 * p.lda1;
    const float* const xb2 = p.a2 ? p.a2 + (int64_t)z * p.sa2 + (int64_t)row0 * p.lda2 : xb1;
    const float* const bias = p.bias ? p.bias + (int64_t)z * p.sbias : nullptr;
    const int64_t rec1 = ((int64_t)(p.m - row0 - 1) * p.lda1 + p.k1) * 4;
    const int64_t rec2 = p.a2 ? ((int64_t)(p.m - row0 - 1) * p.lda2 + p.k2) * 4 : rec1;
    const int64_t recw = (int64_t)3 * p.batch * p.n * K * 2;
    const int64_t rec1c = rec1 < 0x7fffffffLL ? rec1 : 0x7fffffffLL, rec2c = rec2 < 0x7fffffffLL ? rec2 : 0x7fffffffLL;
#if defined(__HIP_DEVICE_COMPILE__)
    const __amdgpu_buffer_rsrc_t r1 = __builtin_amdgcn_make_buffer_rsrc(const_cast<float*>(xb1), 0, (int)rec1c, 0x00020000);
    const __amdgpu_buffer_rsrc_t r2 = __builtin_amdgcn_make_buffer_rsrc(const_cast<float*>(xb2), 0, (int)rec2c, 0x00020000);
#endif
#if defined(__HIP_DEVICE_COMPILE__)
    const __amdgpu_buffer_rsrc_t rw = __builtin_amdgcn_make_buffer_rsrc(const_cast<uint16_t*>(planes_f), 0, (int)recw, 0x00020000);
#endif
    const int plane_bytes = p.batch * p.n * K * 2;
    const int nb0 = (z * p.n + col0) / 16;

    const int q4 = lane & 3, r16 = lane >> 2, g = lane >> 4, l15 = lane & 15;
    const int tvo1 = (r16 * (int)p.lda1 + q4 * 8) * 4, tvo2 = (r16 * (int)p.lda2 + q4 * 8) * 4;
    const int ildso = r16 * 64 + ((q4 ^ ((r16 >> 1) & 3)) << 4);
    const int xoff = l15 * 64 + ((g ^ ((l15 >> 1) & 3)) << 4);
    const int wvo = lane * 16;
    char* const wl = smem + wave * (2 * STAGE);

    f32x4 acc[RB][J];
#pragma unroll
    for (int j = 0; j < J; ++j) {
        f32x4 b4 = {0.f, 0.f, 0.f, 0.f};
        if (bias) b4 = *reinterpret_cast<const f32x4*>(bias + col0 + j * 16 + 4 * g);
#pragma unroll
        for (int i = 0; i < RB; ++i) acc[i][j] = b4;
    }

    f32x4 ld[RB][2];
    bf16x8 wf[2][J][3], xf[2][3];
    const int lda2e = p.a2 ? (int)p.lda2 : (int)p.lda1, kshift = p.a2 ? p.k1 : 0;
    const int tvo2e = p.a2 ? tvo2 : tvo1;
    auto load_tok = [&](int kt, int u, auto segc) {
#if defined(__HIP_DEVICE_COMPILE__)
        constexpr int SEG = decltype(segc)::value;
        const int k0 = kt * BK;
        if constexpr (SEG == 0) {
            const int so = (u * 16 * (int)p.lda1 + k0) * 4;
            ld[u][0] = __builtin_bit_cast(f32x4, __builtin_amdgcn_raw_buffer_load_b128(r1, tvo1, so, 0));
            ld[u][1] = __builtin_bit_cast(f32x4, __builtin_amdgcn_raw_buffer_load_b128(r1, tvo1 + 16, so, 0));
        } else {
            const int so = (u * 16 * lda2e + k0 - kshift) * 4;
            ld[u][0] = __builtin_bit_cast(f32x4, __builtin_amdgcn_raw_buffer_load_b128(r2, tvo2e, so, 0));
            ld[u][1] = __builtin_bit_cast(f32x4, __builtin_amdgcn_raw_buffer_load_b128(r2, tvo2e + 16, so, 0));
        }
#else
        (void)kt; (void)u;
#endif
    };
    auto load_w = [&](int kt, int j, int pl) -> bf16x8 {
#if defined(__HIP_DEVICE_COMPILE__)
        return __builtin_bit_cast(bf16x8, __builtin_amdgcn_raw_buffer_load_b128(rw, wvo, pl * plane_bytes + ((nb0 + j) * KT + kt) * 1024, 0));
#else
        (void)kt; (void)j; (void)pl;
        return bf16x8{};
#endif
    };
    constexpr int NMMA = 6 * J;

    auto tile = [&](const int kt, auto curc, auto segc) {
        constexpr int CUR = decltype(curc)::value, NXT = CUR ^ 1;
        char* const cur = wl + CUR * STAGE;
        char* const nxt = wl + NXT * STAGE;
        const int kn1 = min(kt + 1, KT - 1), kn2 = min(kt + 2, KT - 1);
        constexpr int X0 = CUR ? (RB & 1) : 0;
        DSC_WAVE_STAMP_TILE(0)
        auto block = [&](auto ic) {
            constexpr int i = decltype(ic)::value;
            constexpr int NR = 3;
            constexpr int W0 = i * PERW < NWF ? i * PERW : NWF, W1 = (i + 1) * PERW < NWF ? (i + 1) * PERW : NWF;
            constexpr int VPS = J == 8 ? 2 : 4, NVS = 44 / VPS;
            constexpr int S0 = NR + (W1 - W0), S1 = S0 + NVS, S2 = S1 + 3, S3 = S2 + 1;
            static_assert(S3 <= NMMA, "one MFMA per filler slot");
            unsigned su1[4], su2[4], su3[4];
            float sr0[4], sr1[4], st0[4], st1[4];
            auto xin = [&](int q, int h) -> float { return q < 2 ? ld[i][0][2 * q + h] : ld[i][1][2 * q - 4 + h]; };
            auto split_op = [&](auto nc) {
                constexpr int n = decltype(nc)::value;
                constexpr int q = 2 * (n / 22) + (n & 1), o = (n % 22) >> 1;
                if constexpr (o == 0) su1[q] = cvt_pk_bf16(xin(q, 0), xin(q, 1));
                if constexpr (o == 1) st0[q] = bf_lo(su1[q]);
                if constexpr (o == 2) st1[q] = bf_hi(su1[q]);
                if constexpr (o == 3) sr0[q] = xin(q, 0) - st0[q];
                if constexpr (o == 4) sr1[q] = xin(q, 1) - st1[q];
                if constexpr (o == 5) su2[q] = cvt_pk_bf16(sr0[q], sr1[q]);
                if constexpr (o == 6) st0[q] = bf_lo(su2[q]);
                if constexpr (o == 7) st1[q] = bf_hi(su2[q]);
                if constexpr (o == 8) sr0[q] = sr0[q] - st0[q];
                if constexpr (o == 9) sr1[q] = sr1[q] - st1[q];
                if constexpr (o == 10) su3[q] = cvt_pk_bf16(sr0[q], sr1[q]);
            };
            char* const d0 = nxt + i * 1024 + ildso;
            auto filler = [&](auto kc) {
                constexpr int k = decltype(kc)::value;
                if constexpr (k < NR) {
                    if constexpr (i + 1 < RB) xf[(X0 + i + 1) & 1][k] = *reinterpret_cast<const bf16x8*>(cur + k * XP + (i + 1) * 1024 + xoff);
                    else xf[(X0 + i + 1) & 1][k] = *reinterpret_cast<const bf16x8*>(nxt + k * XP + xoff);
                } else if constexpr (k < S0) {
                    constexpr int w = W0 + (k - NR);
                    wf[NXT][w / 3][w % 3] = load_w(kn1, w / 3, w % 3);
                } else if constexpr (k < S1) {
                    dsc_static_for<VPS>([&](auto vc) { split_op(std::integral_constant<int, VPS * (k - S0) + decltype(vc)::value>{}); });
                } else if constexpr (k < S2) {
                    constexpr int pl = k - S1;
                    const u32x4 v = pl == 0 ? u32x4{su1[0], su1[1], su1[2], su1[3]} : pl == 1 ? u32x4{su2[0], su2[1], su2[2], su2[3]}
                                                                                              : u32x4{su3[0], su3[1], su3[2], su3[3]};
                    *reinterpret_cast<u32x4*>(d0 + pl * XP) = v;
                } else if constexpr (k == S2) {
                    load_tok(kn2, i, segc);
                }
            };
            auto product = [&](auto pc) {
                constexpr int pr = decltype(pc)::value;
                constexpr int wp = pr == 0 ? 2 : (pr == 1 || pr >= 4) ? 0 : 1;
                constexpr int xp = pr == 0 ? 0 : pr == 1 ? 2 : pr == 2 ? 1 : pr == 3 ? 0 : pr == 4 ? 1 : 0;
                dsc_static_for<J>([&](auto jc) {
                    constexpr int j = decltype(jc)::value;
                    acc[i][j] = __builtin_amdgcn_mfma_f32_16x16x32_bf16(wf[CUR][j][wp], xf[(X0 + i) & 1][xp], acc[i][j], 0, 0, 0);
                    filler(std::integral_constant<int, pr * J + j>{});
                    __builtin_amdgcn_sched_barrier(0);
                });
            };
            dsc_static_for<6>(product);
            DSC_WAVE_STAMP_TILE(1 + i)
        };
        dsc_static_for<RB>(block);
        DSC_WAVE_STAMP_FLUSH(kt)
    };

    using std::integral_constant;
#pragma unroll
    for (int u = 0; u < RB; ++u) load_tok(0, u, integral_constant<int, 0>{});
#pragma unroll
    for (int w = 0; w < NWF; ++w) wf[0][w / 3][w % 3] = load_w(0, w / 3, w % 3);
#pragma unroll
    for (int u = 0; u < RB; ++u) {
        bf16x8 a, b, c;
        split8(ld[u][0], ld[u][1], a, b, c);
        char* d0 = wl + u * 1024 + ildso;
        *reinterpret_cast<bf16x8*>(d0) = a;
        *reinterpret_cast<bf16x8*>(d0 + XP) = b;
        *reinterpret_cast<bf16x8*>(d0 + 2 * XP) = c;
        load_tok(1, u, integral_constant<int, 0>{});
    }
#pragma unroll
    for (int pl = 0; pl < 3; ++pl) xf[0][pl] = *reinterpret_cast<const bf16x8*>(wl + pl * XP + xoff);
    const int KT1 = p.k1 / BK;
    int kt = 0;
    DSC_WAVE_STAMP_KERNEL(1)
    for (; kt + 2 < KT1; kt += 2) {
        tile(kt, integral_constant<int, 0>{}, integral_constant<int, 0>{});
        tile(kt + 1, integral_constant<int, 1>{}, integral_constant<int, 0>{});
    }
    f32x4 ep_ga[2], ep_be[2], ep_sc[2], ep_sh[2];
    if constexpr (GN) {
        const bool per_scene_e = p.ss_mode == DSC_SS_PER_SCENE || p.ss_mode == DSC_SS_BY_INDEX;
        int64_t ssrow_e = scene;
        if (p.ss_mode == DSC_SS_BY_INDEX) ssrow_e = dsc_clamp_index(p.ss_index[scene], p.ss_rows);
#pragma unroll
        for (int c2 = 0; c2 < J / 4; ++c2) {
            const int ch = col0 + 64 * c2 + 4 * (lane & 15);
            ep_ga[c2] = *reinterpret_cast<const f32x4*>(p.gamma + ch);
            ep_be[c2] = *reinterpret_cast<const f32x4*>(p.beta + ch);
            ep_sc[c2] = f32x4{0.f, 0.f, 0.f, 0.f};
            ep_sh[c2] = ep_sc[c2];
            if (per_scene_e) {
                const float* ssr = p.scale_shift + ssrow_e * p.ld_ss + ch;
                ep_sc[c2] = *reinterpret_cast<const f32x4*>(ssr);
                ep_sh[c2] = *reinterpret_cast<const f32x4*>(ssr + p.n);
            }
        }
    }
    for (; kt < KT; kt += 2) {
        tile(kt, integral_constant<int, 0>{}, integral_constant<int, 1>{});
        tile(kt + 1, integral_constant<int, 1>{}, integral_constant<int, 1>{});
    }

    DSC_WAVE_STAMP_KERNEL(2)
    constexpr int ERS = 64 * 4 + 16;
    static_assert(ROWS * ERS <= 2 * STAGE, "the transposed cell fits the wave's LDS image");
    const int er = lane >> 4, ec = lane & 15;
#if defined(__HIP_DEVICE_COMPILE__)
    auto row_rsrc = [&](const float* base, int64_t ld, int rows, int cols) {
        return __builtin_amdgcn_make_buffer_rsrc(const_cast<float*>(base), 0, rows > 0 ? (int)(((int64_t)(rows - 1) * ld + cols) * 4) : 0, 0x00020000);
    };
    const __amdgpu_buffer_rsrc_t ry = row_rsrc(p.y + (int64_t)z * p.sy + (int64_t)row0 * p.ldy, p.ldy, rows_here, p.n);
    const __amdgpu_buffer_rsrc_t rr = row_rsrc(p.residual ? p.residual + (int64_t)z * p.sres + (int64_t)row0 * p.ldr : p.y, p.ldr, p.residual ? rows_here : 0, p.n);
    const __amdgpu_buffer_rsrc_t rpa = row_rsrc(p.preact ? p.preact + (int64_t)z * p.sy + (int64_t)row0 * p.ld_preact : p.y, p.ld_preact, p.preact ? rows_here : 0, p.n);
    auto ld4 = [&](const __amdgpu_buffer_rsrc_t& r, int voff, int soff) { return __builtin_bit_cast(f32x4, __builtin_amdgcn_raw_buffer_load_b128(r, voff, soff, 0)); };
    auto st4 = [&](const f32x4 v, const __amdgpu_buffer_rsrc_t& r, int voff, int soff) { __builtin_amdgcn_raw_buffer_store_b128(__builtin_bit_cast(u32x4, v), r, voff, soff, 0); };
#else
    const int ry = 0, rr = 0, rpa = 0;
    auto ld4 = [&](int, int, int) { return f32x4{}; };
    auto st4 = [&](const f32x4, int, int, int) {};
#endif
    const bool has_res = p.residual != nullptr, has_pre = p.preact != nullptr;
    auto to_lds = [&](const int c2) {
#pragma unroll
        for (int i = 0; i < RB; ++i)
#pragma unroll
            for (int j = 0; j < 4; ++j) *reinterpret_cast<f32x4*>(wl + (i * 16 + l15) * ERS + (j * 16 + 4 * g) * 4) = acc[i][4 * c2 + j];
    };
    constexpr int NQ = ROWS / 4, QH = NQ % 10 == 0 ? 10 : NQ % 8 == 0 ? 8 : NQ % 6 == 0 ? 6 : 4;
    static_assert(NQ % QH == 0, "row groups per pass");
    if constexpr (GB) {
        const float inv_cnt = 1.f / (float)(ntok * 64);
        const bool per_scene = p.ss_mode == DSC_SS_PER_SCENE && p.scale_shift;
#if defined(__HIP_DEVICE_COMPILE__)
        const __amdgpu_buffer_rsrc_t rz = row_rsrc(p.gnb_z + (int64_t)row0 * p.ld_gnb_z, p.ld_gnb_z, rows_here, p.n);
#else
        const int rz = 0;
#endif
        dsc_static_for<2>([&](auto c2c) {
            constexpr int c2 = decltype(c2c)::value;
            const int ch = col0 + 64 * c2 + 4 * ec, cc = ch * 4;
            const int vy = er * (int)p.ldy * 4 + cc, vz = er * (int)p.ld_gnb_z * 4 + cc;
            f32x4 zv[NQ], dv[NQ];
#pragma unroll
            for (int q = 0; q < NQ; ++q) zv[q] = ld4(rz, vz, 4 * q * (int)p.ld_gnb_z * 4);
            const f32x4 ga = *reinterpret_cast<const f32x4*>(p.gamma + ch), be = *reinterpret_cast<const f32x4*>(p.beta + ch);
            f32x4 s1 = {1.f, 1.f, 1.f, 1.f}, sh = {0.f, 0.f, 0.f, 0.f};
            if (per_scene) {
                const float* ssr = p.scale_shift + (int64_t)scene * p.ld_ss + ch;
                s1 = *reinterpret_cast<const f32x4*>(ssr) + 1.f;
                sh = *reinterpret_cast<const f32x4*>(ssr + p.n);
            }
            to_lds(c2);
            float s = 0.f;
#pragma unroll
            for (int q = 0; q < NQ; ++q) {
                dv[q] = *reinterpret_cast<const f32x4*>(wl + (4 * q + er) * ERS + ec * 16);
                const bool ok = 4 * q + er < rows_here;
                if (!ok) dv[q] = f32x4{0.f, 0.f, 0.f, 0.f};
                s += ok ? (zv[q][0] + zv[q][1]) + (zv[q][2] + zv[q][3]) : 0.f;
            }
            const float mu = wave_sum_dpp(s) * inv_cnt;
            s = 0.f;
#pragma unroll
            for (int q = 0; q < NQ; ++q) {
                const bool ok = 4 * q + er < rows_here;
#pragma unroll
                for (int e = 0; e < 4; ++e) { const float d = ok ? zv[q][e] - mu : 0.f; s = fmaf(d, d, s); }
            }
            const float rs = 1.0f / sqrtf(wave_sum_dpp(s) * inv_cnt + p.eps);
            float S1 = 0.f, S2 = 0.f;
            f32x4 Gg = {0.f, 0.f, 0.f, 0.f}, Gb = Gg, Gsc = Gg, Gsh = Gg, Gz = Gg;
#pragma unroll
            for (int q = 0; q < NQ; ++q) {
#pragma unroll
                for (int e = 0; e < 4; ++e) {
                    const float xh = (zv[q][e] - mu) * rs;
                    const float gh = ga[e] * xh + be[e];
                    const float u = gh * s1[e] + sh[e];
                    const float sig = __builtin_amdgcn_rcpf(1.0f + __expf(-u));
                    const float du = dv[q][e] * (sig * (1.0f + u * (1.0f - sig)));
                    const float dgh = du * s1[e];
                    const float dxh = dgh * ga[e];
                    S1 += dxh; S2 += dxh * xh;
                    Gg[e] += dgh * xh; Gb[e] += dgh; Gsc[e] += du * gh; Gsh[e] += du;
                    zv[q][e] = xh;
                    dv[q][e] = dxh;
                }
            }
            const float m1 = wave_sum_dpp(S1) * inv_cnt, m2 = wave_sum_dpp(S2) * inv_cnt;
#pragma unroll
            for (int q = 0; q < NQ; ++q) {
                const bool ok = 4 * q + er < rows_here;
                f32x4 dzv;
#pragma unroll
                for (int e = 0; e < 4; ++e) { dzv[e] = rs * (dv[q][e] - m1 - zv[q][e] * m2); Gz[e] += ok ? dzv[e] : 0.f; }
                st4(dzv, ry, vy, 4 * q * (int)p.ldy * 4);
            }
            auto fold = [&](f32x4 v) {
#pragma unroll
                for (int e = 0; e < 4; ++e) { v[e] += __shfl_xor(v[e], 16, 64); v[e] += __shfl_xor(v[e], 32, 64); }
                return v;
            };
            Gg = fold(Gg); Gb = fold(Gb); Gz = fold(Gz);
            if (per_scene && p.gnb_dss) { Gsc = fold(Gsc); Gsh = fold(Gsh); }
            if (lane < 16) {
                const int64_t o = (int64_t)scene * p.gnb_pstride + ch;
                *reinterpret_cast<f32x4*>(p.gnb_dgamma + o) = Gg;
                *reinterpret_cast<f32x4*>(p.gnb_dbeta + o) = Gb;
                *reinterpret_cast<f32x4*>(p.gnb_dbias + o) = Gz;
                if (per_scene && p.gnb_dss) {
                    *reinterpret_cast<f32x4*>(p.gnb_dss + (int64_t)scene * p.ld_gnb_dss + ch) = Gsc;
                    *reinterpret_cast<f32x4*>(p.gnb_dss + (int64_t)scene * p.ld_gnb_dss + p.n + ch) = Gsh;
                }
            }
        });
    } else if constexpr (!GN) {
#if defined(__HIP_DEVICE_COMPILE__)
        const __amdgpu_buffer_rsrc_t rg = row_rsrc(p.actgrad_x ? p.actgrad_x + (int64_t)z * p.sy + (int64_t)row0 * p.ld_actgrad : p.y, p.ld_actgrad, p.actgrad_x ? rows_here : 0, p.n);
#else
        const int rg = 0;
#endif
        auto cell = [&](auto c2c, auto modec, auto actc) {
            constexpr int c2 = decltype(c2c)::value, MODE = decltype(modec)::value, ACT = decltype(actc)::value;
            const int cc = (col0 + 64 * c2 + 4 * ec) * 4;
            const int vy = er * (int)p.ldy * 4 + cc, vr = er * (int)p.ldr * 4 + cc, vp = er * (int)p.ld_preact * 4 + cc, vg = er * (int)p.ld_actgrad * 4 + cc;
            to_lds(c2);
#pragma unroll 1
            for (int h = 0; h < NQ; h += QH) {
                f32x4 rres[QH], gx[QH];
                if (has_res) {
#pragma unroll
                    for (int qq = 0; qq < QH; ++qq) rres[qq] = ld4(rr, vr, 4 * (h + qq) * (int)p.ldr * 4);
                }
                if constexpr (MODE == 2) {
#pragma unroll
                    for (int qq = 0; qq < QH; ++qq) gx[qq] = ld4(rg, vg, 4 * (h + qq) * (int)p.ld_actgrad * 4);
                }
#pragma unroll
                for (int qq = 0; qq < QH; ++qq) {
                    f32x4 y = *reinterpret_cast<const f32x4*>(wl + (4 * (h + qq) + er) * ERS + ec * 16);
                    if (has_pre) st4(y, rpa, vp, 4 * (h + qq) * (int)p.ld_preact * 4);
#pragma unroll
                    for (int e = 0; e < 4; ++e) {
                        if constexpr (MODE == 1) y[e] = dsc_act(y[e], ACT);
                        if constexpr (MODE == 2) y[e] *= dsc_act_grad(gx[qq][e], ACT);
                    }
                    if (has_res) y += rres[qq];
                    st4(y, ry, vy, 4 * (h + qq) * (int)p.ldy * 4);
                }
            }
        };
        auto cells = [&](auto modec, auto actc) {
            cell(std::integral_constant<int, 0>{}, modec, actc);
            if constexpr (J == 8) cell(std::integral_constant<int, 1>{}, modec, actc);
        };
        using std::integral_constant;
        const int act = p.act_out;
        if (p.actgrad_x) {
            if (act == DSC_ACT_GELU) cells(integral_constant<int, 2>{}, integral_constant<int, DSC_ACT_GELU>{});
            else if (act == DSC_ACT_SILU) cells(integral_constant<int, 2>{}, integral_constant<int, DSC_ACT_SILU>{});
            else if (act == DSC_ACT_LEAKY01) cells(integral_constant<int, 2>{}, integral_constant<int, DSC_ACT_LEAKY01>{});
            else cells(integral_constant<int, 0>{}, integral_constant<int, DSC_ACT_NONE>{});
        } else {
            if (act == DSC_ACT_GELU) cells(integral_constant<int, 1>{}, integral_constant<int, DSC_ACT_GELU>{});
            else if (act == DSC_ACT_SILU) cells(integral_constant<int, 1>{}, integral_constant<int, DSC_ACT_SILU>{});
            else if (act == DSC_ACT_LEAKY01) cells(integral_constant<int, 1>{}, integral_constant<int, DSC_ACT_LEAKY01>{});
            else cells(integral_constant<int, 0>{}, integral_constant<int, DSC_ACT_NONE>{});
        }
    } else {
#if defined(__HIP_DEVICE_COMPILE__)
        const __amdgpu_buffer_rsrc_t rs = row_rsrc(PERROW ? p.scale_shift + (p.ss_mode == DSC_SS_PER_TOKEN ? (int64_t)row0 * p.ld_ss : 0) : p.y, p.ld_ss,
                                                   PERROW ? rows_here : 0, 2 * p.n);
#else
        const int rs = 0;
#endif
        const float inv_cnt = 1.f / (float)(ntok * 64);
        const bool vlast = (RB - 1) * 16 + l15 < rows_here;
#pragma unroll
        for (int c2 = 0; c2 < J / 4; ++c2) {
            const int ch = col0 + 64 * c2 + 4 * ec;
            const f32x4 ga = ep_ga[c2], be = ep_be[c2], sc = ep_sc[c2], sh = ep_sh[c2];
            to_lds(c2);
            float s0 = 0.f;
#pragma unroll
            for (int i = 0; i < RB; ++i)
#pragma unroll
                for (int j = 0; j < 4; ++j) {
                    const f32x4 a = acc[i][4 * c2 + j];
                    const float t = (a[0] + a[1]) + (a[2] + a[3]);
                    s0 += (i < RB - 1 || vlast) ? t : 0.f;
                }
            const float mean = wave_sum_dpp(s0) * inv_cnt;
            float q0 = 0.f;
#pragma unroll
            for (int i = 0; i < RB; ++i)
#pragma unroll
                for (int j = 0; j < 4; ++j)
#pragma unroll
                    for (int e = 0; e < 4; ++e) {
                        const float d = (i < RB - 1 || vlast) ? acc[i][4 * c2 + j][e] - mean : 0.f;
                        q0 = fmaf(d, d, q0);
                    }
            const float rstd = 1.f / sqrtf(wave_sum_dpp(q0) * inv_cnt + p.eps);
            if (c2 == 0) { DSC_WAVE_STAMP_KERNEL(3) }
            f32x4 A, B;
#pragma unroll
            for (int e = 0; e < 4; ++e) {
                const float a = rstd * ga[e], sp1 = sc[e] + 1.f;
                A[e] = a * sp1;
                B[e] = fmaf(be[e] - mean * a, sp1, sh[e]);
            }
            const int cc = ch * 4;
            const int vy = er * (int)p.ldy * 4 + cc, vr = er * (int)p.ldr * 4 + cc, vp = er * (int)p.ld_preact * 4 + cc, vs = er * (int)p.ld_ss * 4 + cc;
            if (c2 == 0) { DSC_WAVE_STAMP_KERNEL(4) }
#pragma unroll
            for (int h = 0; h < NQ; h += QH) {
                f32x4 rres[QH], s1[QH], s2[QH];
                if (has_res) {
#pragma unroll
                    for (int qq = 0; qq < QH; ++qq) rres[qq] = ld4(rr, vr, 4 * (h + qq) * (int)p.ldr * 4);
                }
                if constexpr (PERROW) {
#pragma unroll
                    for (int qq = 0; qq < QH; ++qq) {
                        s1[qq] = ld4(rs, vs, 4 * (h + qq) * (int)p.ld_ss * 4);
                        s2[qq] = ld4(rs, vs + p.n * 4, 4 * (h + qq) * (int)p.ld_ss * 4);
                    }
                }
#pragma unroll
                for (int qq = 0; qq < QH; ++qq) {
                    const f32x4 zv = *reinterpret_cast<const f32x4*>(wl + (4 * (h + qq) + er) * ERS + ec * 16);
                    if (has_pre) st4(zv, rpa, vp, 4 * (h + qq) * (int)p.ld_preact * 4);
                    f32x4 y;
#pragma unroll
                    for (int e = 0; e < 4; ++e) {
                        float t = fmaf(zv[e], A[e], B[e]);
                        if constexpr (PERROW) t = fmaf(t, s1[qq][e] + 1.f, s2[qq][e]);
                        y[e] = dsc_silu_fast(t);
                    }
                    if (has_res) y += rres[qq];
                    st4(y, ry, vy, 4 * (h + qq) * (int)p.ldy * 4);
                }
            }
            if (c2 == 0) { DSC_WAVE_STAMP_KERNEL(5) }
        }
    }
    DSC_WAVE_STAMP_END
}

template <bool GN, int RB, bool PERROW = false, int J = 8, bool GB = false>
int launch(const dsc_gemm_args* a, const uint16_t* planes_f, int ntok, hipStream_t s) {
    const int scenes = (a->m + ntok - 1) / ntok;
    const unsigned grid = (unsigned)(((scenes + WAVES - 1) / WAVES) * (a->n / (16 * J)));
    DSC_CLEAR_STALE_ERROR();
    hipLaunchKernelGGL((gemm_split_wave_kernel<GN, RB, PERROW, J, GB>), dim3(grid, (unsigned)a->batch), dim3(64 * WAVES), 0, s, *a, planes_f, ntok DSC_WAVE_STAMP_PASS);
    DSC_LAUNCH_CHECK();
    return 0;
}

}
```

diffuscene_amd/engine.py:

```python
import ctypes as C

import torch

from . import _lib, ops
from ._lib import ACT_GELU, ACT_NONE, ACT_SILU, SS_BY_INDEX, SS_NONE, SS_PER_SCENE, SS_PER_SLOT, SS_PER_TOKEN

D = 512
HID = 128
DEC_PAD = 32


def _own(t):
    if isinstance(t, torch.nn.Parameter):
        return t.detach()
    if isinstance(t, (tuple, list)):
        return tuple(_own(u) for u in t)
    return t


class StalePlanError(RuntimeError):
    pass


class _Pool:
# ... 14 lines not shown
        return t

    def put(self, t):
        self.free_list.setdefault((t.shape[0], t.shape[1]), []).append(t)


class Plan:

    def __init__(self, eng, B, N, ctx_mode, ctx_dim, L, text_dim, time_table=False):
        self.eng, self.B, self.N, self.M = eng, B, N, B * N
        self.generation = eng.generation
        dev = eng.device
        self.pool = _Pool(dev)
        self.keep = []
        self.steps = []
        self.pre_steps = []
        net = eng.net
        C_in = net.channels
        self.x_in = torch.empty((self.M, C_in), device=dev, dtype=torch.float32)
        self.t_in = torch.empty((B,), device=dev, dtype=torch.int64)
        ctx_rows = {SS_NONE: 0, SS_PER_SLOT: N, SS_PER_TOKEN: self.M}[ctx_mode]
        self.ctx_in = torch.empty((ctx_rows, ctx_dim), device=dev, dtype=torch.float32) if ctx_rows else None
        self.cross_in = torch.empty((B * L, text_dim), device=dev, dtype=torch.float32) if L else None
        self.ctx_mode = ctx_mode
        self.L = L
        self.time_table = time_table
        self.out = torch.empty((self.M, net.out_dim), device=dev, dtype=torch.float32)
        self._build()
        self.tiled_steps = self.steps

    def gemm_args(self):
        kinds = {id(_lib.fn("dsc_gemm_gn_silu_f32")): "gn", id(_lib.fn("dsc_gemm_f32")): "plain"}
        out = []
        for f, a in self.steps:
            k = kinds.get(id(f))
            if k is not None:
                out.append((k, a[0]._obj))
        return out

    def gemm(self, a, w, out, bias=None, a2=None, residual=None, act_in=ACT_NONE, act_out=ACT_NONE, row_invariant=False):
        g = ops.make_gemm_args(a, w, out, bias, a2, residual, act_in, act_out, row_invariant=row_invariant)
        lay = ops.planes_layout(g)
        pl = self.eng.planes_of(w, lay) if lay >= 0 else None
        if pl is not None:
            ops.attach_planes(g, pl, layout=lay)
        self.keep.append(_own((g, a, w, out, bias, a2, residual, pl)))
        self.steps.append((_lib.fn("dsc_gemm_f32"), (C.byref(g),)))
        return out

    def gemm_batched(self, a, w, out, bias, batch, sa, sw, sy, sbias, act_out=ACT_NONE):
        stacked = w._base if w._base is not None else w
        g = ops.make_gemm_args(a, w, out, bias, None, None, ACT_NONE, act_out)
        g.batch, g.sa1, g.sw, g.sy, g.sbias = batch, sa, sw, sy, sbias
        whole = (stacked.dim() == 2 and stacked.is_contiguous() and w.data_ptr() == stacked.data_ptr()
                 and stacked.shape[0] == batch * w.shape[0] and stacked.shape[1] == w.shape[1] and sw == w.shape[0] * w.shape[1])
        lay = ops.planes_layout(g) if whole else -1
        pl = self.eng.planes_of(stacked, lay) if lay >= 0 else None
        if pl is not None:
            ops.attach_planes(g, pl, layout=lay)
        self.keep.append(_own((g, a, w, out, bias, pl)))
        self.steps.append((_lib.fn("dsc_gemm_f32"), (C.byref(g),)))
        return out

    def gemm_gn(self, a, w, out, bias, gamma, beta, a2=None, ss=None, ss_mode=SS_NONE, residual=None):
        g = ops.make_gemm_args(a, w, out, bias, a2, residual, gamma=gamma, beta=beta, eps=1e-5,
                               tokens_per_scene=self.N, scale_shift=ss, ss_mode=ss_mode if ss is not None else SS_NONE,
                               ss_index=self.t_in if (ss is not None and ss_mode == SS_BY_INDEX) else None)
        lay = ops.planes_layout(g, gn=True)
        pl = self.eng.planes_of(w, lay) if lay >= 0 else None
        if pl is not None:
            ops.attach_planes(g, pl, gn=True, layout=lay)
        self.keep.append(_own((g, a, w, out, bias, a2, residual, gamma, beta, ss, pl)))
        self.steps.append((_lib.fn("dsc_gemm_gn_silu_f32"), (C.byref(g),)))
        return out

    def call(self, name, *args, keep=()):
        self.keep.append(_own(keep))
        self.steps.append((_lib.fn(name), args))

    def hoist(self, first):
        if self.time_table:
            self.pre_steps += self.steps[first:]
            del self.steps[first:]
            return True
        return False

    def check_current(self):
        if self.generation != self.eng.generation:
            raise StalePlanError("diffuscene_amd: this launch plan was built for parameter storages the model no longer uses (flat storage "
                                 "of the first training step, module.to(), load into new tensors): rebuild it -- DenoiserEngine.prepare() / "
                                 "graph_sample_loop() do -- instead of running or replaying it")

    def run_pre(self):
        self.check_current()
        s = ops.stream_ptr()
        for f, a in self.pre_steps:
            rc = f(*a, s)
            if rc:
                _lib.check(rc, f.__name__)

    def layernorm(self, x, g, out, residual=None):
        self.call("dsc_layernorm_f32", x.data_ptr(), x.stride(0), g.data_ptr(),
                  residual.data_ptr() if residual is not None else None,
                  residual.stride(0) if residual is not None else 0,
                  out.data_ptr(), out.stride(0), x.shape[0], x.shape[1], 1e-5, keep=(x, g, out, residual))
        return out

    def out_proj_ln(self, a, conv, ln_gain, residual):
        M = self.M
        out = self.pool.get(M, D)
        if (M + 95) // 96 >= 160:
            g = ops.make_gemm_args(a, conv.weight, out, conv.bias, None, residual, gamma=ln_gain.view(-1), beta=ln_gain.view(-1),
                                   eps=1e-5)
            self.keep.append(_own((g, a, conv.weight, out, conv.bias, residual, ln_gain)))
            self.steps.append((_lib.fn("dsc_gemm_layernorm_f32"), (C.byref(g),)))
            return out
        o = self.gemm(a, conv.weight, self.pool.get(M, D), conv.bias)
        self.layernorm(o, ln_gain, out, residual=residual)
        self.pool.put(o)
        return out

    def resblock(self, rb, x, x2, ss, ss_mode):
        e, M = self.eng, self.M
        h = self.pool.get(M, D)
        self.gemm_gn(x, e.ws[id(rb.block1.proj)], h, rb.block1.proj.bias, rb.block1.norm.weight, rb.block1.norm.bias,
                     a2=x2, ss=ss, ss_mode=ss_mode)
        if rb.has_res_conv:
            r = self.pool.get(M, D)
            self.gemm(x, rb.res_conv.weight, r, rb.res_conv.bias, a2=x2)
        else:
            r = x
        out = self.pool.get(M, D)
        self.gemm_gn(h, e.ws[id(rb.block2.proj)], out, rb.block2.proj.bias, rb.block2.norm.weight, rb.block2.norm.bias,
                     residual=r)
        self.pool.put(h)
        if rb.has_res_conv:
            self.pool.put(r)
        return out

    def t_ss(self, rb):
        i = self.eng.t_index[id(rb)]
        return self.ss_t[:, i * 2 * D:(i + 1) * 2 * D], (SS_BY_INDEX if self.time_table else SS_PER_SCENE)

    def c_ss(self, rb):
        if self.ss_c is None:
            return None, SS_NONE
        i = self.eng.c_index[id(rb)]
        return self.ss_c[:, i * 2 * D:(i + 1) * 2 * D], self.ctx_mode

    def linattn(self, blk, x):
        M, B, N = self.M, self.B, self.N
        att = blk.fn.fn
        y = self.layernorm(x, blk.fn.norm.g, self.pool.get(M, D))
        qkv = self.gemm(y, att.to_qkv.weight, self.pool.get(M, 3 * HID))
        self.pool.put(y)
        a = self.pool.get(M, HID)
        self.call("dsc_linear_attention_f32", qkv.data_ptr(), 3 * HID, qkv.data_ptr() + 4 * HID, 3 * HID,
                  qkv.data_ptr() + 8 * HID, 3 * HID, a.data_ptr(), HID, B, N, N, float(att.scale), keep=(qkv, a))
        self.pool.put(qkv)
        out = self.out_proj_ln(a, att.to_out[0], att.to_out[1].g, x)
        self.pool.put(a)
        return out

    def crossattn(self, blk, x):
        M, B, N, L = self.M, self.B, self.N, self.L
        att = blk.fn.fn
        y = self.layernorm(x, blk.fn.norm.g, self.pool.get(M, D))
        q = self.gemm(y, att.to_q.weight, self.pool.get(M, HID))
        self.pool.put(y)
        first = len(self.steps)
        kv = self.gemm(self.cross_in, att.to_kv.weight, self.pool.get(B * L, 2 * HID))
        kv_is_invariant = self.hoist(first)
        a = self.pool.get(M, HID)
        self.call("dsc_linear_attention_f32", q.data_ptr(), HID, kv.data_ptr(), 2 * HID, kv.data_ptr() + 4 * HID,
                  2 * HID, a.data_ptr(), HID, B, N, L, float(att.scale), keep=(q, kv, a))
        self.pool.put(q)
        if not kv_is_invariant:
            self.pool.put(kv)
        out = self.out_proj_ln(a, att.to_out[0], att.to_out[1].g, x)
        self.pool.put(a)
        return out

    def fullattn(self, blk, x):
        M, B, N = self.M, self.B, self.N
        att = blk.fn.fn
        y = self.layernorm(x, blk.fn.norm.g, self.pool.get(M, D))
        qkv = self.gemm(y, att.to_qkv.weight, self.pool.get(M, 3 * HID))
        self.pool.put(y)
        a = self.pool.get(M, HID)
        self.call("dsc_attention_f32", qkv.data_ptr(), 3 * HID, qkv.data_ptr() + 4 * HID, 3 * HID,
                  qkv.data_ptr() + 8 * HID, 3 * HID, a.data_ptr(), HID, B, N, float(att.scale), keep=(qkv, a))
        self.pool.put(qkv)
        out = self.gemm(a, att.to_out.weight, self.pool.get(M, D), att.to_out.bias, residual=x)
        self.pool.put(a)
        return out

    def _build(self):
        e, net, M, B = self.eng, self.eng.net, self.M, self.B
        pool = self.pool
        if self.time_table:
            self.ss_t = e.ss_table()
        else:
            temb = pool.get(B, D)
            self.call("dsc_time_embedding_f32", self.t_in.data_ptr(), B, D, e.time_table.data_ptr(),
                      e.time_table.shape[0], e.time_freq.data_ptr(), temb.data_ptr(), keep=(temb,))
            t1 = self.gemm(temb, net.time_mlp[1].weight, pool.get(B, 4 * D), net.time_mlp[1].bias, act_out=ACT_GELU, row_invariant=True)
            t2 = self.gemm(t1, net.time_mlp[3].weight, pool.get(B, 4 * D), net.time_mlp[3].bias, act_out=ACT_SILU, row_invariant=True)
            self.ss_t = self.gemm(t2, e.t_pack_w, pool.get(B, e.t_pack_w.shape[0]), e.t_pack_b, row_invariant=True)
        if self.ctx_in is not None:
            first = len(self.steps)
            cact = pool.get(self.ctx_in.shape[0], self.ctx_in.shape[1])
            self.call("dsc_activation_f32", self.ctx_in.data_ptr(), cact.data_ptr(), self.ctx_in.numel(), ACT_SILU,
                      keep=(cact,))
            self.ss_c = self.gemm(cact, e.c_pack_w, pool.get(self.ctx_in.shape[0], e.c_pack_w.shape[0]), e.c_pack_b)
            self.hoist(first)
        else:
            self.ss_c = None
        if net.seperate_all:
            bb, nc, no, nf = net.bbox_dim, net.class_dim, net.objectness_dim, net.objfeat_dim
            emb = pool.get(M, D)
            H = len(e.enc_heads)
            h1 = pool.get(M, H * D)
            items = (_lib.SmallKItem * H)()
            for i, (seq, c0, k) in enumerate(e.enc_heads):
                xs = self.x_in[:, c0:c0 + k]
                items[i].x, items[i].ldx, items[i].k_in = xs.data_ptr(), self.x_in.stride(0), k
                items[i].w, items[i].ldw, items[i].bias = seq[0].weight.data_ptr(), k, seq[0].bias.data_ptr()
                items[i].y, items[i].ldy = h1.data_ptr() + 4 * i * D, H * D
            self.call("dsc_linear_smallk_grouped_f32", items, H, M, D, ACT_GELU,
                      keep=(items, h1, [(seq[0].weight, seq[0].bias) for seq, _, _ in e.enc_heads]))
            h2 = pool.get(M, H * 2 * D)
            self.gemm_batched(h1[:, :D], e.enc_w2[:2 * D], h2[:, :2 * D], e.enc_b2[:2 * D], H, D, 2 * D * D, 2 * D, 2 * D,
                              act_out=ACT_GELU)
            pool.put(h1)
            self.gemm(h2, e.enc_w3, emb, e.enc_b3)
            pool.put(h2)
            x = self.gemm(emb, net.init_conv.weight, pool.get(M, D), net.init_conv.bias)
            pool.put(emb)
        else:
            x = pool.get(M, D)
            k = net.channels
            self.call("dsc_linear_smallk_f32", self.x_in.data_ptr(), self.x_in.stride(0), k,
                      net.init_conv.weight.data_ptr(), k, net.init_conv.bias.data_ptr(), x.data_ptr(), D, M, D,
                      ACT_NONE, keep=(x, net.init_conv.weight, net.init_conv.bias))
        r = x
        skips = []
        text = net.text_condition

        def step(rb, xin, x2, ss_pair, free_in=True):
            out = self.resblock(rb, xin, x2, *ss_pair)
            if free_in and xin is not r and all(xin is not s for s in skips):
                pool.put(xin)
            return out

        for lvl in net.downs:
            b0, b1, ac, b2, la, down = lvl
            x = step(b0, x, None, self.c_ss(b0))
            x = step(b1, x, None, self.t_ss(b1))
            skips.append(x)
            if text:
                x = self.crossattn(ac, x)
            x = step(b2, x, None, self.t_ss(b2))
            xo = self.linattn(la, x)
            pool.put(x)
            x = xo
            skips.append(x)
            if isinstance(down, torch.nn.Conv1d):
                x = self.gemm(x, down.weight, pool.get(M, D), down.bias)
        x = step(net.mid_block0, x, None, self.c_ss(net.mid_block0))
        x = step(net.mid_block1, x, None, self.t_ss(net.mid_block1))
        if text:
            xo = self.crossattn(net.mid_attn_cross, x)
            pool.put(x)
            x = xo
        xo = self.fullattn(net.mid_attn, x)
        pool.put(x)
        x = step(net.mid_block2, xo, None, self.t_ss(net.mid_block2))
        for lvl in net.ups:
            b0, b1, ac, b2, la, up = lvl
            x = step(b0, x, None, self.c_ss(b0))
            s = skips.pop()
            xo = self.resblock(b1, x, s, *self.t_ss(b1))
            pool.put(x)
            pool.put(s)
            x = xo
            if text:
                xo = self.crossattn(ac, x)
                pool.put(x)
                x = xo
            s = skips.pop()
            xo = self.resblock(b2, x, s, *self.t_ss(b2))
            pool.put(x)
            pool.put(s)
            xo2 = self.linattn(la, xo)
            pool.put(xo)
            x = xo2
            if isinstance(up, torch.nn.Conv1d):
                xo = self.gemm(x, up.weight, pool.get(M, D), up.bias)
                pool.put(x)
                x = xo
        xo = self.resblock(net.final_res_block, x, r, *self.t_ss(net.final_res_block))
        pool.put(x)
        x = xo
        if net.seperate_all:
            Hd = len(e.dec_heads)
            d1 = self.gemm(x, e.dec_w1, pool.get(M, Hd * 2 * D), e.dec_b1, act_out=ACT_GELU)
            d2 = pool.get(M, Hd * D)
            self.gemm_batched(d1[:, :2 * D], e.dec_w2[:D], d2[:, :D], e.dec_b2[:D], Hd, 2 * D, D * 2 * D, D, D, act_out=ACT_GELU)
            pool.put(d1)
            P = e.dec_pad
            pad = pool.get(M, Hd * P)
            self.gemm_batched(d2[:, :D], e.dec_w3p[:P], pad[:, :P], e.dec_b3p[:P], Hd, D, P * D, P, P)
            spans = (_lib.ColSpan * Hd)()
            col = 0
            for i, (seq, width) in enumerate(e.dec_heads):
# ... 199 lines not shown
```

diffuscene_amd/ops.py:

```python
import ctypes as C
import numbers

import torch

from . import _lib
from ._lib import (ACT_GELU, ACT_NONE, ACT_SILU, MEAN_EPS, MEAN_V, MEAN_X0, SS_NONE, SS_PER_SCENE,
                   SS_PER_SLOT, SS_PER_TOKEN, GemmArgs, SplitItem, WsItem)


def stream_ptr():
    return torch.cuda.current_stream().cuda_stream


def _dev(t, name="tensor", dtype=torch.float32):
    if not isinstance(t, torch.Tensor) or not t.is_cuda:
        raise RuntimeError("diffuscene_amd: %s must live on a HIP device (no CPU fallback exists)" % name)
    if t.dtype != dtype:
        raise RuntimeError("diffuscene_amd: %s must be %s, got %s" % (name, dtype, t.dtype))
    return t


def _mat(t, name):
    _dev(t, name)
    if t.dim() != 2 or (t.shape[1] > 1 and t.stride(1) != 1):
        raise RuntimeError("diffuscene_amd: %s must be a 2-D tensor with contiguous rows, got shape %s strides %s"
                           % (name, tuple(t.shape), t.stride()))
    return t.data_ptr(), (t.stride(0) if t.shape[0] > 1 else t.shape[1])


def as2d(w):
    return w.view(w.shape[0], w.shape[1]) if w.dim() == 3 else w


def make_gemm_args(a, w, y, bias=None, a2=None, residual=None, act_in=ACT_NONE, act_out=ACT_NONE,
                   gamma=None, beta=None, eps=1e-5, tokens_per_scene=0, scale_shift=None, ss_mode=SS_NONE, preact=None,
                   ss_index=None, w_planes=None, actgrad_x=None, gnb=None, row_invariant=False):
    g = GemmArgs()
    g.a1, g.lda1 = _mat(a, "a")
    g.k1 = a.shape[1]
    if a2 is not None:
        g.a2, g.lda2 = _mat(a2, "a2")
        g.k2 = a2.shape[1]
        if a2.shape[0] != a.shape[0]:
            raise RuntimeError("a and a2 row mismatch")
    w2 = as2d(w)
    g.w, g.ldw = _mat(w2, "w")
    if w2.shape[1] != g.k1 + g.k2:
        raise RuntimeError("weight K (%d) != activation K (%d)" % (w2.shape[1], g.k1 + g.k2))
    g.m, g.n = a.shape[0], w2.shape[0]
    g.y, g.ldy = _mat(y, "y")
    if tuple(y.shape) != (g.m, g.n):
        raise RuntimeError("output shape %s != (%d, %d)" % (tuple(y.shape), g.m, g.n))
    if bias is not None:
        g.bias = _dev(bias, "bias").data_ptr()
    if residual is not None:
        g.residual, g.ldr = _mat(residual, "residual")
    g.act_in, g.act_out, g.batch = act_in, act_out, 1
    if row_invariant:
        g.flags |= _lib.GEMM_ROW_INVARIANT
    if gamma is not None:
        g.gamma, g.beta, g.eps = _dev(gamma).data_ptr(), _dev(beta).data_ptr(), eps
        g.tokens_per_scene = tokens_per_scene
    if scale_shift is not None:
        g.scale_shift, g.ld_ss = _mat(scale_shift, "scale_shift")
        g.ss_mode = ss_mode
    if preact is not None:
        g.preact, g.ld_preact = _mat(preact, "preact")
    if actgrad_x is not None:
        g.actgrad_x, g.ld_actgrad = _mat(actgrad_x, "actgrad_x")
        if tuple(actgrad_x.shape) != (g.m, g.n):
            raise RuntimeError("actgrad_x shape %s != (%d, %d)" % (tuple(actgrad_x.shape), g.m, g.n))
    if gnb is not None:
        g.gnb_z, g.ld_gnb_z = _mat(gnb["z"], "gnb z")
        g.gnb_dgamma, g.gnb_dbeta, g.gnb_dbias = gnb["dgamma"], gnb["dbeta"], gnb["dbias"]
        g.gnb_pstride = gnb["pstride"]
        if gnb.get("dss") is not None:
            g.gnb_dss, g.ld_gnb_dss = _mat(gnb["dss"], "gnb dss")
    if ss_index is not None:
        if scale_shift is None:
            raise RuntimeError("ss_index (DSC_SS_BY_INDEX) needs the scale_shift table it indexes")
        g.ss_index = _dev(ss_index, "ss_index", torch.int64).data_ptr()
        g.ss_rows = scale_shift.shape[0]
    if w_planes is not None:
        if (w_planes.dtype != torch.int16 or w_planes.dim() != 3 or w_planes.shape[0] != 3 or w_planes.shape[1] % g.n
                or w_planes.shape[2] != g.k1 + g.k2 or not w_planes.is_contiguous()):
            raise RuntimeError("w_planes must be a contiguous int16 tensor of shape (3, %d, %d)" % (g.n, g.k1 + g.k2))
        attach_planes(g, w_planes, gn=gamma is not None and gnb is None)
    return g


PLANES_ROWMAJOR, PLANES_FRAGMENT = 0, 1


def planes_layout(g, gn=False):
    r = _lib.fn("dsc_gemm_planes_layout")(C.byref(g), 1 if gn else 0)
    if r == _lib.DSC_PLANES_NONE:
        return -1
    if r < 0:
        _lib.check(r, "dsc_gemm_planes_layout")
    return r


def fragment_major(planes):
    _, n, k = planes.shape
    return planes.view(3, n // 16, 16, k // 32, 4, 8).permute(0, 1, 3, 4, 2, 5).contiguous().view(3, n, k)


def attach_planes(g, planes, gn=False, layout=None):
    want = planes_layout(g, gn)
    if layout is None:
        layout = getattr(planes, "_dsc_layout", PLANES_ROWMAJOR)
        if want == PLANES_FRAGMENT and layout == PLANES_ROWMAJOR:
            cached = getattr(planes, "_dsc_fragment", None)
            if cached is None or cached[0] != planes._version:
                cached = planes._dsc_fragment = (planes._version, fragment_major(planes))
            planes, layout = cached[1], PLANES_FRAGMENT
            g._planes_keep = planes
    g.w_planes = planes.data_ptr()
    g.w_planes_layout = layout
    return g


def planes_wanted(n, k):
    return n % 128 == 0 and k % 32 == 0 and 6 * n * k < 0x7fffffff


def split_planes(items, stream=None):
    out, batch = [], []
    for w, planes, tr in items:
        tr = int(tr)
        frag, tr = tr & 2, tr & 1
        w2 = as2d(_dev(w, "w"))
        ptr, ldw = _mat(w2, "w")
        r, c = w2.shape
        shape = (3, c, r) if tr else (3, r, c)
        if planes is None:
            planes = torch.empty(shape, device=w2.device, dtype=torch.int16)
        elif tuple(planes.shape) != shape or planes.dtype != torch.int16 or not planes.is_contiguous():
            raise RuntimeError("split_planes: planes must be contiguous int16 %s" % (shape,))
        planes._dsc_layout = PLANES_FRAGMENT if frag else PLANES_ROWMAJOR
        planes._dsc_fragment = None
        out.append(planes)
        batch.append((ptr, ldw, r, c, planes.data_ptr(), (1 if tr else 0) | frag, w2, planes))
    for i in range(0, len(batch), _lib.WS_MAX):
        part = batch[i:i + _lib.WS_MAX]
        arr = (SplitItem * len(part))()
        for j, (ptr, ldw, r, c, pp, tr, _, _) in enumerate(part):
            arr[j].w, arr[j].ldw, arr[j].rows, arr[j].cols, arr[j].planes, arr[j].transpose = ptr, ldw, r, c, pp, tr
        _lib.check(_lib.fn("dsc_split_bf16x3_f32")(arr, len(part), stream if stream is not None else stream_ptr()),
                   "dsc_split_bf16x3_f32")
    return out


def gemm_uses_split(g, gn=False):
    return _lib.fn("dsc_gemm_arithmetic")(C.byref(g), 1 if gn else 0) == 1


def gemm_would_use_split(g, gn=False):
    return planes_layout(g, gn) >= 0


def run_gemm(g, gn=False, stream=None):
    name = "dsc_gemm_gn_silu_f32" if gn else "dsc_gemm_f32"
    _lib.check(_lib.fn(name)(C.byref(g), stream if stream is not None else stream_ptr()), name)


def gemm(a, w, bias=None, a2=None, residual=None, act_in=ACT_NONE, act_out=ACT_NONE, out=None, w_planes=None, row_invariant=False):
    w2 = as2d(w)
    if out is None:
        out = torch.empty((a.shape[0], w2.shape[0]), device=a.device, dtype=torch.float32)
    run_gemm(make_gemm_args(a, w, out, bias, a2, residual, act_in, act_out, w_planes=w_planes, row_invariant=row_invariant))
    return out


def gemm_gn_silu(a, w_std, bias, gamma, beta, tokens_per_scene, a2=None, scale_shift=None, ss_mode=SS_NONE,
                 residual=None, eps=1e-5, out=None, preact=None, w_planes=None, ss_index=None):
    w2 = as2d(w_std)
    if out is None:
        out = torch.empty((a.shape[0], w2.shape[0]), device=a.device, dtype=torch.float32)
    run_gemm(make_gemm_args(a, w_std, out, bias, a2, residual, gamma=gamma, beta=beta, eps=eps,
                            tokens_per_scene=tokens_per_scene, scale_shift=scale_shift, ss_mode=ss_mode,
                            preact=preact, w_planes=w_planes, ss_index=ss_index), gn=True)
    return out


def linear_smallk(x, w, bias, act_out=ACT_NONE, out=None):
    xp, ldx = _mat(x, "x")
    w2 = as2d(w)
    wp, ldw = _mat(w2, "w")
    if out is None:
        out = torch.empty((x.shape[0], w2.shape[0]), device=x.device, dtype=torch.float32)
    yp, ldy = _mat(out, "y")
    _lib.check(_lib.fn("dsc_linear_smallk_f32")(xp, ldx, x.shape[1], wp, ldw,
                                                bias.data_ptr() if bias is not None else None,
                                                yp, ldy, x.shape[0], w2.shape[0], act_out, stream_ptr()),
               "dsc_linear_smallk_f32")
    return out


def make_ws_items(pairs):
    arr = (WsItem * len(pairs))()
    for i, (w, o) in enumerate(pairs):
        w2, o2 = as2d(_dev(w)), as2d(_dev(o))
        if not (w2.is_contiguous() and o2.is_contiguous()):
            raise RuntimeError("weight_standardize needs contiguous matrices")
# ... 680 lines not shown
```

diffuscene_amd/train_plan.py:

```python
import ctypes as C
import os

import torch

from ._lib import ACT_GELU, ACT_NONE, ACT_SILU, SS_NONE, SS_PER_SCENE, SS_PER_SLOT, SS_PER_TOKEN

D = 512
HID = 128


def _as2d(w):
    return w.view(w.shape[0], w.shape[1]) if w.dim() == 3 else w


class H:
    __slots__ = ("t", "g", "ng", "act_of", "g_pre", "uses", "gn_of", "gn_part")

    def __init__(self, t, needs_grad=True):
        self.t, self.g, self.ng = t, None, needs_grad
        self.uses = 0
        self.act_of = None
        self.g_pre = None
        self.gn_of = None
        self.gn_part = None
# ... 39 lines not shown
    depth = max(len(l) for l in lists)
    out = []
    for pos in range(depth):
        for x in range(n_xcd):
            out.append(lists[x][pos] if pos < len(lists[x]) else (-1, -1))
    return out


class HipBackend:

    name = "hip"

    def __init__(self, device):
        from . import _lib
        _lib.load()
        self.lib = _lib
        self.device = device
        self.keep = []
        self.scratch_floats = 0
        self.scratch = None
        self._scratch_users = []
        self.split = _lib.split_enabled()
        self._planes = {}
        self._planes_new = []
        self.plane_bytes = 0
        self.transposed_of = {}
        self.f32_reads = set()

    def planes_of(self, w, rows, layout=0):
        from . import ops
        if not self.split or rows < 256 or w.dim() != 2 or w.stride(1) != 1 or not ops.planes_wanted(w.shape[0], w.shape[1]):
            return None
        key = (w.data_ptr(), tuple(w.shape), w.stride(0), layout)
        ent = self._planes.get(key)
        if ent is None:
            planes = torch.empty((3,) + tuple(w.shape), device=self.device, dtype=torch.int16)
            self.plane_bytes += planes.numel() * 2
            src = self.transposed_of.get(w.data_ptr())
            if src is not None and (not w.is_contiguous() or tuple(src.shape) != (w.shape[1], w.shape[0])):
                src = None
            if src is None:
                self.f32_reads.add(w.untyped_storage().data_ptr())
            ent = self._planes[key] = (w, planes, src, 2 * layout)
            self._planes_new.append(ent)
        return ent[1]

    def split_steps(self):
        from . import ops
        ents, self._planes_new = self._planes_new, []
        steps = []
        for i in range(0, len(ents), self.lib.WS_MAX):
            part = ents[i:i + self.lib.WS_MAX]
            arr = (self.lib.SplitItem * len(part))()
            for j, (w, planes, src, frag) in enumerate(part):
                if src is not None:
                    ptr, ldw = ops._mat(src, "w")
                    arr[j].w, arr[j].ldw, arr[j].rows, arr[j].cols, arr[j].planes, arr[j].transpose = (
                        ptr, ldw, src.shape[0], src.shape[1], planes.data_ptr(), 1 | frag)
                    continue
                ptr, ldw = ops._mat(w, "w")
                arr[j].w, arr[j].ldw, arr[j].rows, arr[j].cols, arr[j].planes, arr[j].transpose = (
                    ptr, ldw, w.shape[0], w.shape[1], planes.data_ptr(), frag)
            steps.append(self._call("dsc_split_bf16x3_f32", arr, len(part), keep=(arr, part)))
        return steps

    def _mat(self, t):
        from .ops import _mat
        return _mat(t, "plan tensor")

    def _call(self, name, *args, keep=()):
        from .engine import _own
        self.keep.append(_own(keep))
        return (self.lib.fn(name), args, name)

    def finalize(self):
        self.scratch = torch.empty(max(self.scratch_floats, 1), device=self.device, dtype=torch.float32)
        for fix in self._scratch_users:
            fix(self.scratch)

    def _with_scratch(self, floats, build):
        self.scratch_floats = max(self.scratch_floats, int(floats))
        holder = {}

        def fix(scr):
            holder["step"] = build(scr.data_ptr(), scr.numel())
        self._scratch_users.append(fix)
        return holder

    def fuse_act_ok(self, a, w, out, a2=None, bias=None, preact=None, actgrad_x=None):
        from . import ops
        if not self.split or a.shape[0] < 256 or os.environ.get("DSC_FUSE_ACT", "1") == "0":
            return False
        g = ops.make_gemm_args(a, w, out, bias, a2, act_out=ACT_GELU if (preact is not None or actgrad_x is not None) else ACT_NONE,
                               preact=preact, actgrad_x=actgrad_x)
        lay = ops.planes_layout(g)
        return lay >= 0 and self.planes_of(w, a.shape[0], lay) is not None

    def gemm(self, a, w, out, bias=None, a2=None, residual=None, act_out=ACT_NONE, preact=None, actgrad_x=None):
        from . import ops
        m, K = a.shape
        if preact is not None or actgrad_x is not None:
            g = ops.make_gemm_args(a, w, out, bias, a2, residual, ACT_NONE, act_out, preact=preact, actgrad_x=actgrad_x)
            lay = ops.planes_layout(g)
            pl = self.planes_of(w, m, lay) if lay >= 0 else None
            if pl is None:
                raise RuntimeError("HipBackend.gemm: an activation epilogue was planned for a launch the split kernel does not take")
            ops.attach_planes(g, pl, layout=lay)
            return self._call("dsc_gemm_f32", C.byref(g), keep=(g, a, w, out, bias, a2, residual, pl, preact, actgrad_x))
        tiles = ((m + 63) // 64) * ((out.shape[1] + 63) // 64)
        if a2 is None and act_out == ACT_NONE and tiles < 256 and K >= 1024 and (m * out.shape[1]) % 4 == 0:
            splits = next((s for s in (8, 4, 2) if K % (32 * s) == 0 and K // s >= 128), 0)
            if splits:
                fn = self.lib.fn("dsc_gemm_splitk_f32")
                floats = splits * m * out.shape[1]
                g = ops.make_gemm_args(a, w, out, bias, a2, residual, ACT_NONE, act_out)
                from .engine import _own
                self.keep.append(_own((g, a, w, out, bias, residual)))
                self.f32_reads.add(w.untyped_storage().data_ptr())
                return self._with_scratch(floats, lambda wp, wn: (fn, (C.byref(g), splits, wp, wn), "dsc_gemm_splitk_f32"))
        g = ops.make_gemm_args(a, w, out, bias, a2, residual, ACT_NONE, act_out)
        lay = ops.planes_layout(g)
        pl = self.planes_of(w, m, lay) if lay >= 0 else None
        if pl is not None:
            ops.attach_planes(g, pl, layout=lay)
        else:
            self.f32_reads.add(w.untyped_storage().data_ptr())
        return self._call("dsc_gemm_f32", C.byref(g), keep=(g, a, w, out, bias, a2, residual, pl))

    def _gnbwd_args(self, dy, wt, dz, gn, part):
        from . import ops
        Cc = dz.shape[1]
        pp, ps = (part.data_ptr(), part.stride(0)) if part is not None else (0x100000, 3 * Cc)
        g = ops.make_gemm_args(dy, wt, dz, gamma=gn["gamma"], beta=gn["beta"], eps=1e-5, tokens_per_scene=gn["n_tok"],
                               scale_shift=gn["ss"], ss_mode=gn["ss_mode"] if gn["ss"] is not None else SS_NONE,
                               gnb=dict(z=gn["z"], dgamma=pp + 4 * Cc, dbeta=pp + 8 * Cc, dbias=pp, pstride=ps, dss=gn["dss"]))
        return g

    def fuse_gnbwd_ok(self, dy, wt, like, gn):
        from . import ops
        if not self.split or os.environ.get("DSC_FUSE_GNBWD", "1") == "0" or gn["ss_mode"] not in (SS_NONE, SS_PER_SCENE):
            return False
        g = self._gnbwd_args(dy, wt, like, gn, None)
        return ops.planes_layout(g) == ops.PLANES_FRAGMENT and self.planes_of(wt, dy.shape[0], ops.PLANES_FRAGMENT) is not None

    def gemm_gnbwd(self, dy, wt, dz, gn, part):
        from . import ops
        g = self._gnbwd_args(dy, wt, dz, gn, part)
        lay = ops.planes_layout(g)
        pl = self.planes_of(wt, dy.shape[0], lay) if lay >= 0 else None
        if pl is None:
            raise RuntimeError("HipBackend.gemm_gnbwd: planned for a launch the wave-autonomous kernel does not take")
        ops.attach_planes(g, pl, layout=lay)
        return self._call("dsc_gemm_f32", C.byref(g), keep=(g, dy, wt, dz, gn["z"], gn["gamma"], gn["beta"], gn["ss"], gn["dss"], part, pl))

    def gemm_long_k(self, a, w, out, residual=None):
        from . import ops
        m, K = a.shape
        n = out.shape[1]
        if (m * n) % 4 or K % 32:
            return None
        splits = long_k_splits(K)
        if not splits:
            return None
        fn = self.lib.fn("dsc_gemm_splitk_f32")
        g = ops.make_gemm_args(a, w, out, None, None, residual, ACT_NONE, ACT_NONE)
        from .engine import _own
        self.keep.append(_own((g, a, w, out, residual)))
        self.f32_reads.add(w.untyped_storage().data_ptr())
        floats = splits * m * n
        return self._with_scratch(floats, lambda wp, wn: (fn, (C.byref(g), splits, wp, wn), "dsc_gemm_splitk_f32"))

    def gemm_gn(self, a, w, out, bias, gamma, beta, n_tok, a2=None, ss=None, ss_mode=SS_NONE, residual=None, preact=None):
        from . import ops
        g = ops.make_gemm_args(a, w, out, bias, a2, residual, gamma=gamma, beta=beta, eps=1e-5, tokens_per_scene=n_tok,
                               scale_shift=ss, ss_mode=ss_mode if ss is not None else SS_NONE, preact=preact)
        lay = ops.planes_layout(g, gn=True)
        pl = self.planes_of(w, a.shape[0], lay) if lay >= 0 else None
        if pl is not None:
            ops.attach_planes(g, pl, gn=True, layout=lay)
        else:
            self.f32_reads.add(w.untyped_storage().data_ptr())
        return self._call("dsc_gemm_gn_silu_f32", C.byref(g), keep=(g, a, w, out, bias, gamma, beta, a2, ss, residual, preact, pl))

    def smallk(self, x, w, bias, out, act_out=ACT_NONE):
        xp, ldx = self._mat(x)
        wp, ldw = self._mat(w)
        yp, ldy = self._mat(out)
        return self._call("dsc_linear_smallk_f32", xp, ldx, x.shape[1], wp, ldw, bias.data_ptr() if bias is not None else None,
                          yp, ldy, x.shape[0], w.shape[0], act_out, keep=(x, w, bias, out))

    def ws(self, weights, outs):
        from . import ops
        steps = []
        for i in range(0, len(weights), self.lib.WS_MAX):
            arr = ops.make_ws_items(list(zip(weights[i:i + self.lib.WS_MAX], outs[i:i + self.lib.WS_MAX])))
            steps.append(self._call("dsc_weight_standardize_f32", arr, len(arr), 1e-5, keep=(arr, weights, outs)))
        return steps

    def time_embedding(self, t, table, freq, out):
        return self._call("dsc_time_embedding_f32", t.data_ptr(), t.shape[0], out.shape[1], table.data_ptr(), table.shape[0],
                          freq.data_ptr(), out.data_ptr(), keep=(t, table, freq, out))

    def act(self, x, out, kind):
        assert x.is_contiguous() and out.is_contiguous()
        return self._call("dsc_activation_f32", x.data_ptr(), out.data_ptr(), x.numel(), kind, keep=(x, out))

    def layernorm(self, x, g, out, residual=None):
        xp, ldx = self._mat(x)
        yp, ldy = self._mat(out)
        rp, ldr = self._mat(residual) if residual is not None else (None, 0)
        return self._call("dsc_layernorm_f32", xp, ldx, g.data_ptr(), rp, ldr, yp, ldy, x.shape[0], x.shape[1], 1e-5,
                          keep=(x, g, out, residual))

    def linattn(self, q, k, v, out, scenes, nq, nk, scale):
        a = []
        for t in (q, k, v, out):
            a += list(self._mat(t))
        return self._call("dsc_linear_attention_f32", *a, scenes, nq, nk, scale, keep=(q, k, v, out))

    def attn(self, q, k, v, out, scenes, n, scale):
        a = []
        for t in (q, k, v, out):
            a += list(self._mat(t))
        return self._call("dsc_attention_f32", *a, scenes, n, scale, keep=(q, k, v, out))

    def q_sample(self, x0, noise, t, sqrt_ac, sqrt_1mac, xt, v):
        b = x0.shape[0]
        return self._call("dsc_q_sample_f32", x0.data_ptr(), noise.data_ptr(), t.data_ptr(), sqrt_ac.data_ptr(),
                          sqrt_1mac.data_ptr(), xt.data_ptr(), v.data_ptr() if v is not None else None, b, x0.numel() // b,
                          int(sqrt_ac.numel()), keep=(x0, noise, t, sqrt_ac, sqrt_1mac, xt, v))

    def loss(self, target, out, x_t, t, tb, ca, cb, bounds, dims, separate, iou, mean_type, losses, parts, dout, scale):
        B, N, Cc = out.shape
        barr = (C.c_float * 12)(*[float(v) for v in bounds]) if bounds is not None else None
        return self._call("dsc_ddpm_loss_f32", target.data_ptr(), out.data_ptr(), x_t.data_ptr(), t.data_ptr(),
                          tb["loss_weight"].data_ptr(), ca.data_ptr() if ca is not None else None,
                          cb.data_ptr() if cb is not None else None, tb["alphas_cumprod"].data_ptr(), barr,
                          losses.data_ptr(), parts.data_ptr(), dout.data_ptr(), B, N, Cc, dims["translation_dim"],
                          dims["size_dim"], dims["bbox_dim"], dims["class_dim"], dims["objectness_dim"], dims["objfeat_dim"],
                          1 if separate else 0, 1 if iou else 0, mean_type, float(scale), int(tb["loss_weight"].numel()),
                          keep=(target, out, x_t, t, tb, ca, cb, barr, losses, parts, dout))

    def gemm_tn(self, a, dy, out, a2=None, kvalid=None, dbias=None):
        ap, lda = self._mat(a)
        dp, ldd = self._mat(dy)
        a2p, lda2, k2 = (None, 0, 0)
        if a2 is not None:
            a2p, lda2 = self._mat(a2)
            k2 = a2.shape[1]
        k1 = a.shape[1]
        kv = (k1 + k2) if kvalid is None else kvalid
        m, n = dy.shape
        op, ldo = self._mat(out)
        wsf = self.lib.fn("dsc_gemm_tn_workspace_floats")(m, n, kv)
        fn = self.lib.fn("dsc_gemm_tn_f32")
        self.keep.append((a, dy, out, a2, dbias))
        dbp = dbias.data_ptr() if dbias is not None else None
        return self._with_scratch(wsf, lambda wp, wn: (fn, (ap, lda, k1, a2p, lda2, k2, dp, ldd, op, ldo, dbp, m, n, kv,
                                                            wp if wsf else None, wn if wsf else 0), "dsc_gemm_tn_f32"))

    def gemm_tn_grouped(self, items):
        import numpy as np
        items = sorted(items, key=lambda it: -it["dy"].shape[0])
        arr = (self.lib.TnGroup * len(items))()
        tile0, ws_off = 0, 0
        tile0s = 0
        use_split = self.split
        per_group = []
        shapes = [(it["dy"].shape[0], it["dy"].shape[1], it["a"].shape[1] + (it["a2"].shape[1] if it.get("a2") is not None else 0))
                  for it in items]
        for i, it in enumerate(items):
            a, dy, out, a2, dbias = it["a"], it["dy"], it["out"], it.get("a2"), it.get("dbias")
            ap, lda = self._mat(a)
            dp, ldd = self._mat(dy)
            op, ldo = self._mat(out)
            k1 = a.shape[1]
            a2p, lda2, k2 = (None, 0, 0)
            if a2 is not None:
                a2p, lda2 = self._mat(a2)
                k2 = a2.shape[1]
            m, n = dy.shape
            kv = (k1 + k2) if it.get("kvalid") is None else it["kvalid"]
            if (k1 & 3) or (k2 & 3) or (n & 3) or (k2 > 0 and k1 % 128) or not (1 <= kv <= k1 + k2):
                raise RuntimeError("gemm_tn_grouped: bad shape m=%d n=%d k1=%d k2=%d kvalid=%d" % (m, n, k1, k2, kv))
            if (ap % 16) or (lda & 3) or (dp % 16) or (ldd & 3) or (k2 and ((a2p % 16) or (lda2 & 3))):
                raise RuntimeError("gemm_tn_grouped: operands must be 16-byte aligned with row strides multiple of 4")
            if a.shape[0] != m or (a2 is not None and a2.shape[0] != m) or tuple(out.shape) != (n, kv):
                raise RuntimeError("gemm_tn_grouped: shape mismatch")
            g = arr[i]
            g.a1, g.lda1, g.k1, g.a2, g.lda2, g.k2 = ap, lda, k1, a2p, lda2, k2
            g.dy, g.ldd, g.out, g.ldo = dp, ldd, op, ldo
            g.dbias = dbias.data_ptr() if dbias is not None else None
            g.m, g.n, g.kvalid, g.tile0 = m, n, kv, tile0
            nt = ((n + 127) // 128) * ((k1 + k2 + 127) // 128)
            tile0 += nt
            g.tile0s = tile0s
            nts = ((n + 255) // 256) * ((k1 + k2 + 127) // 128)
            tile0s += nts
            if m * max(lda, ldd, lda2) * 4 >= 0x7fffffff:
                use_split = False
            per_group.append((n, kv, ldo))
        total = tile0
        if use_split:
            tile_k = 256 if (self.lib.fn("dsc_get_tn_split_form")() == 2
                             and all(not (it.get("a2") is not None and it["a"].shape[1] % 256) for it in items)) else 128
            rounds = int(os.environ.get("DSC_TN_ROUNDS", "3" if tile_k == 128 else "2"))
# ... 233 lines not shown
        S = u.stride(0)
        cu, cv = u.storage_offset() % S, v.storage_offset() % S
        if cu + u.shape[1] > S or cv + v.shape[1] > S:
            return True
        return not (cu + u.shape[1] <= cv or cv + v.shape[1] <= cu)

    def g_alias(self, h, src):
        if not h.ng:
            return
        if h.g is None:
            h.g = src
        else:
            self._guard(h.g)
            self.emit(self.be.add(h.g, src))
            self.n_adds += 1

    def g_target(self, h):
        if h.g is None:
            h.g = self.new(*h.t.shape)
            return h.g, False
        self._guard(h.g)
        return h.g, True

    def g_write(self, h, produce):
        if not h.ng:
            return
        if h.g is None:
            h.g = self.new(*h.t.shape)
            produce(h.g)
        else:
            tmp = self.new(*h.t.shape)
            produce(tmp)
            self._guard(h.g)
            self.emit(self.be.add(h.g, tmp))
            self.n_adds += 1

    def g_write_add(self, h, produce):
        if not h.ng:
            return
        old = h.g
        dst = self.new(*h.t.shape)
        produce(dst, old)
        h.g = dst

    @staticmethod
    def _use(*handles):
        for h in handles:
            if h is not None:
                h.uses += 1

    def g_gemm(self, a, a2, dy, wt):
        k1 = a.t.shape[1]
        K = wt.shape[0]
        if a2 is None:
            if not a.ng:
                return
            if (a.act_of is not None and a.uses == 1 and a.g is None and a.g_pre is None and dy.shape[1] <= 4096
                    and hasattr(self.be, "fuse_act_ok") and self.be.fuse_act_ok(dy, wt, a.t, actgrad_x=a.act_of[0])):
                u, kind = a.act_of
                a.g_pre = self.new(*a.t.shape)
                self.emit(self.be.gemm(dy, wt, a.g_pre, act_out=kind, actgrad_x=u))
                return
            if (a.gn_of is not None and a.uses == 1 and a.g is None and a.g_pre is None and hasattr(self.be, "fuse_gnbwd_ok")):
                gn = a.gn_of
                if self.be.fuse_gnbwd_ok(dy, wt, a.t, gn):
                    dz = self.new(*a.t.shape)
                    part = self.new(a.t.shape[0] // gn["n_tok"], 3 * a.t.shape[1])
                    a.g_pre, a.gn_part = dz, part
                    self.emit(self.be.gemm_gnbwd(dy, wt, dz, gn, part))
                    return
            dst, acc = self.g_target(a)
            self._gemm_acc(dy, wt, dst, acc)
            return
        want1, want2 = a.ng, a2.ng
        if not (want1 or want2):
            return
        pair_fresh = a.g is None and a2.g is None and want1 and want2
        same_parent = (a.g is not None and a2.g is not None and a.g.stride(0) == K and a2.g.stride(0) == K
                       and a2.g.data_ptr() == a.g.data_ptr() + 4 * k1)
        if pair_fresh:
            buf = self.new(dy.shape[0], K)
            a.g, a2.g = buf[:, :k1], buf[:, k1:]
            self._gemm_acc(dy, wt, buf, False)
        elif same_parent:
            buf = torch.as_strided(a.g, (a.g.shape[0], K), (K, 1))
            self._guard(buf)
            self._gemm_acc(dy, wt, buf, True)
        else:
            tmp = self.new(dy.shape[0], K)
            self._gemm_acc(dy, wt, tmp, False)
            if want1:
                self.g_alias(a, tmp[:, :k1])
            if want2:
                self.g_alias(a2, tmp[:, k1:])

    def _gemm_acc(self, dy, wt, dst, acc):
        n = dy.shape[1]
        if n > 4096 and hasattr(self.be, "gemm_long_k"):
            step = self.be.gemm_long_k(dy, wt, dst, dst if acc else None)
            if step is not None:
                self.emit(step)
                return
        if n > 4096:
            for c0 in range(0, n, 2048):
                c1 = min(c0 + 2048, n)
                self.emit(self.be.gemm(dy[:, c0:c1], wt[:, c0:c1], dst, residual=dst if (acc or c0 > 0) else None))
        else:
            self.emit(self.be.gemm(dy, wt, dst, residual=dst if acc else None))

    def tn(self, a, dy, out, a2=None, kvalid=None, dbias=None, params=(), after=None):
        self._tn_pending.append({"a": a, "dy": dy, "out": out, "a2": a2, "kvalid": kvalid, "dbias": dbias,
                                 "params": tuple(p for p in params if p is not None), "after": after})
        if self.tn_flush_floats and sum(it["out"].numel() for it in self._tn_pending) >= self.tn_flush_floats:
            self.flush_tn()

    def colsum_later(self, x, out, params=(), after=None):
        if not hasattr(self.be, "colsum_grouped"):
            self.emit(self.be.colsum(x, out))
            if after is not None:
                after()
            self.wrote(*params)
            return
        self._cs_pending.append({"x": x, "out": out, "params": tuple(params), "after": after})

    def flush_tn(self):
        cs, self._cs_pending = self._cs_pending, []
        if cs:
            self.emit(self.be.colsum_grouped([(it["x"], it["out"]) for it in cs]))
            for it in cs:
                if it["after"] is not None:
                    it["after"]()
            self.wrote(*[p for it in cs for p in it["params"]])
        items, self._tn_pending = self._tn_pending, []
        if not items:
            return
        self.emit(self.be.gemm_tn_grouped(items))
        for it in items:
            if it["after"] is not None:
                it["after"]()
        self.wrote(*[p for it in items for p in it["params"]])

    def wT(self, w2d, npad=None):
        n, K = w2d.shape
        if npad is None or npad == n:
            buf = self.new(K, n)
            self._transposes.append((w2d, buf))
            if hasattr(self.be, "transposed_of"):
                self.be.transposed_of[buf.data_ptr()] = w2d
            return buf
        buf = self.zeros(K, npad)
        self._transposes.append((w2d, buf[:, :n]))
        return buf

    def linear(self, a, weight, bias, a2=None, residual=None, out=None, act_out=ACT_NONE, wt=None, act=None):
        w2 = _as2d(weight)
        n, K = w2.shape
        rows = a.t.shape[0]
        y = H(out if out is not None else self.new(rows, n))
        self._use(a, a2, residual)
        assert act_out == ACT_NONE, "training keeps the pre-activation (its backward needs it): use act="
        fused = (act is not None and residual is None and out is None and hasattr(self.be, "fuse_act_ok")
                 and self.be.fuse_act_ok(a.t, w2, y.t, a2.t if a2 is not None else None, bias=bias, preact=y.t))
        if fused:
            ya_t = self.new(rows, n)
            self.emit(self.be.gemm(a.t, w2, ya_t, bias, a2.t if a2 is not None else None, None, act, preact=y.t))
        else:
            self.emit(self.be.gemm(a.t, w2, y.t, bias, a2.t if a2 is not None else None,
                                   residual.t if residual is not None else None, act_out))

        def bw():
            dy = y.g
            if dy is None:
                return
            npad = (n + 31) // 32 * 32
            if npad != n:
                dyp = self.zeros(rows, npad)
                self.emit(self.be.copy(dyp[:, :n], dy))
            elif not self._dense_ok(dy):
                dyp = self.new(rows, n)
                self.emit(self.be.copy(dyp, dy))
            else:
                dyp = dy
            if a.ng or (a2 is not None and a2.ng):
                self.g_gemm(a, a2, dyp, wt if wt is not None else self.wT(w2, npad))
            gw = self.gview(weight)
            gb = self.flat.grad_view(bias) if bias is not None else None
            if npad != n:
                tw = self.new(npad, K)
                tb = self.new(1, npad) if bias is not None else None

                def unpad():
                    self.emit(self.be.copy(gw, tw[:n]))
                    if bias is not None:
                        self.emit(self.be.copy(gb.view(1, n), tb[:, :n]))
                self.tn(a.t, dyp, tw, a2.t if a2 is not None else None, dbias=tb.view(-1) if tb is not None else None,
                        params=(weight, bias), after=unpad)
            else:
                self.tn(a.t, dyp, gw, a2.t if a2 is not None else None, dbias=gb, params=(weight, bias))
            if residual is not None:
                self.g_alias(residual, dy)
        self._tape.append(bw)
        if act is None:
            return y
        return self.act(y, act, out=ya_t if fused else None)

    def smallk(self, x_slice, weight, bias):
        w2 = _as2d(weight)
        n, k = w2.shape
        rows = x_slice.shape[0]
        y = H(self.new(rows, n))
        self.emit(self.be.smallk(x_slice, w2, bias, y.t))
        xpad = self.zeros(rows, 32 if k <= 32 else 64)
        self.emit(self.be.copy(xpad[:, :k], x_slice))

        def bw():
            if y.g is None:
                return
            self.tn(xpad, y.g, self.gview(weight), kvalid=k, dbias=self.flat.grad_view(bias), params=(weight, bias))
        self._tape.append(bw)
        return y

    def act(self, x, kind, out=None):
        y = H(out if out is not None else self.new(*x.t.shape))
        if out is None:
            self.emit(self.be.act(x.t, y.t, kind))
        y.act_of = (x.t, kind)

        def bw():
            if y.g_pre is not None:
                self.g_alias(x, y.g_pre)
                if y.g is None:
                    return
            if y.g is None or not x.ng:
                return
            dy = y.g
            if not dy.is_contiguous():
                d = self.new(*dy.shape)
                self.emit(self.be.copy(d, dy))
                dy = d
            self.g_write(x, lambda dst: self.emit(self.be.act_bwd(x.t, dy, dst, kind)))
        self._tape.append(bw)
        return y

    def conv_gn(self, a, blk, a2=None, ss=None, ss_mode=SS_NONE, dss=None, residual=None):
        conv, norm = blk.proj, blk.norm
        w_std = self.ws_std[id(conv)]
        rows = a.t.shape[0]
        y, z = H(self.new(rows, D)), self.new(rows, D)
        self._use(a, a2, residual)
        self.emit(self.be.gemm_gn(a.t, w_std, y.t, conv.bias, norm.weight, norm.bias, self.N, a2.t if a2 is not None else None,
                                  ss, ss_mode, residual.t if residual is not None else None, z))

        if residual is None:
            y.gn_of = dict(z=z, gamma=norm.weight, beta=norm.bias, ss=ss, ss_mode=ss_mode if ss is not None else SS_NONE,
                           dss=dss if (ss is not None and ss_mode == SS_PER_SCENE) else None, n_tok=self.N)

        def bw():
            dy = y.g
            if dy is None and y.g_pre is None:
                return
            scenes = rows // self.N
            slot_tmp = None
            if y.g_pre is not None:
                dz, part = y.g_pre, y.gn_part
            else:
                dz = self.new(rows, D)
                part = self.new(scenes, 3 * D)
                dss_arg = dss
                if ss is not None and ss_mode == SS_PER_SLOT:
                    slot_tmp = self.new(rows, 2 * D)
                    dss_arg = slot_tmp
                self.emit(self.be.gn_bwd(z, dy, norm.weight, norm.bias, ss, ss_mode, dz, part, dss_arg, scenes, self.N))
            o_b, o_g, o_be = (self.flat.grad_range(p)[0] for p in (conv.bias, norm.weight, norm.bias))
            if o_g == o_b + D and o_be == o_g + D:
                self.colsum_later(part, self.flat.G[o_b:o_b + 3 * D], params=(conv.bias, norm.weight, norm.bias))
            else:
                tmp = self.new(1, 3 * D)

                def scatter(tmp=tmp):
                    for i, p in enumerate((conv.bias, norm.weight, norm.bias)):
                        self.emit(self.be.copy(self.flat.grad_view(p).view(1, D), tmp[:, i * D:(i + 1) * D]))
                self.colsum_later(part, tmp.view(-1), params=(conv.bias, norm.weight, norm.bias), after=scatter)
            if slot_tmp is not None:
                red = self.new(self.N, 2 * D)
                self.emit(self.be.colsum(slot_tmp.view(scenes, self.N * 2 * D), red.view(-1)))
                self.emit(self.be.copy(dss, red))
            self.g_gemm(a, a2, dz, self.ws_t[id(conv)])
            self.tn(a.t, dz, self.dws[id(conv)], a2.t if a2 is not None else None)
            self._ws_pending.append(conv)
            if residual is not None:
                self.g_alias(residual, dy)
        self._tape.append(bw)
        return y

    def resblock(self, rb, a, a2, ss_pair, post=None):
        if post is not None:
            self._tape.append(post)
        ss, mode, dss = ss_pair
        h = self.conv_gn(a, rb.block1, a2=a2, ss=ss, ss_mode=mode, dss=dss)
        r = self.linear(a, rb.res_conv.weight, rb.res_conv.bias, a2=a2) if rb.has_res_conv else a
        return self.conv_gn(h, rb.block2, residual=r)

    def layernorm(self, x, gain, residual=None):
        g = gain.view(-1)
        y = H(self.new(*x.t.shape))
        self._use(x, residual)
        self.emit(self.be.layernorm(x.t, g, y.t, residual.t if residual is not None else None))

        def bw():
            dy = y.g
            if dy is None:
                return
            M_ = x.t.shape[0]
            nblk = min((M_ + 3) // 4, 512)
            part = self.new(nblk, x.t.shape[1])
            self.g_write_add(x, lambda dst, addend: self.emit(self.be.layernorm_bwd(x.t, g, dy, dst, part, addend)))
            self.colsum_later(part, self.flat.grad_view(gain).view(-1), params=(gain,))
            if residual is not None:
                self.g_alias(residual, dy)
        self._tape.append(bw)
        return y

    def linattn(self, blk, a):
        att = blk.fn.fn
        B, N = self.B, self.N
        y = self.layernorm(a, blk.fn.norm.g)
        qkv = self.linear(y, att.to_qkv.weight, None)
        o = H(self.new(self.M, HID))
        q, k, v = qkv.t[:, :HID], qkv.t[:, HID:2 * HID], qkv.t[:, 2 * HID:]
        self.emit(self.be.linattn(q, k, v, o.t, B, N, N, float(att.scale)))

        def bw():
            if o.g is None:
                return
            d = self.new(self.M, 3 * HID)
            qkv.g = d
            self.emit(self.be.linattn_bwd(q, k, v, o.g, d[:, :HID], d[:, HID:2 * HID], d[:, 2 * HID:], B, N, N,
                                          float(att.scale)))
        self._tape.append(bw)
        p = self.linear(o, att.to_out[0].weight, att.to_out[0].bias)
        return self.layernorm(p, att.to_out[1].g, residual=a)

    def crossattn(self, blk, a):
        att = blk.fn.fn
        B, N, L = self.B, self.N, self.L
        y = self.layernorm(a, blk.fn.norm.g)
        qh = self.linear(y, att.to_q.weight, None)
        kv = self.linear(self.cross_in, att.to_kv.weight, None)
        o = H(self.new(self.M, HID))
        self.emit(self.be.linattn(qh.t, kv.t[:, :HID], kv.t[:, HID:], o.t, B, N, L, float(att.scale)))

        def bw():
            if o.g is None:
                return
            dq, dkv = self.new(self.M, HID), self.new(B * L, 2 * HID)
            qh.g, kv.g = dq, dkv
            self.emit(self.be.linattn_bwd(qh.t, kv.t[:, :HID], kv.t[:, HID:], o.g, dq, dkv[:, :HID], dkv[:, HID:], B, N, L,
                                          float(att.scale)))
        self._tape.append(bw)
        p = self.linear(o, att.to_out[0].weight, att.to_out[0].bias)
        return self.layernorm(p, att.to_out[1].g, residual=a)

    def fullattn(self, blk, a):
        att = blk.fn.fn
        B, N = self.B, self.N
        y = self.layernorm(a, blk.fn.norm.g)
        qkv = self.linear(y, att.to_qkv.weight, None)
        o = H(self.new(self.M, HID))
        q, k, v = qkv.t[:, :HID], qkv.t[:, HID:2 * HID], qkv.t[:, 2 * HID:]
        self.emit(self.be.attn(q, k, v, o.t, B, N, float(att.scale)))

        def bw():
            if o.g is None:
                return
            d = self.new(self.M, 3 * HID)
            qkv.g = d
            self.emit(self.be.attn_bwd(q, k, v, o.g, d[:, :HID], d[:, HID:2 * HID], d[:, 2 * HID:], B, N, float(att.scale)))
        self._tape.append(bw)
        return self.linear(o, att.to_out.weight, att.to_out.bias, residual=a)

    def encoder(self, seq, c0, k, acc):
        xf = self.x_t.view(self.M, -1)
        h = self.act(self.smallk(xf[:, c0:c0 + k], seq[0].weight, seq[0].bias), ACT_GELU)
        h = self.linear(h, seq[2].weight, seq[2].bias, act=ACT_GELU)
        return self.linear(h, seq[4].weight, seq[4].bias, residual=acc)

    def _build(self):
        net, be, B, N, M = self.net, self.be, self.B, self.N, self.M
        diff = self.diff
        tb = self._tables if self._tables is not None else diff.tables(self.device)
        self.tb = tb
        fl = self.flat
        want_v = diff.model_mean_type == "v"
        self.v_buf = self.new3(B, N, net.channels) if want_v else None
        self.emit(be.q_sample(self.x0, self.noise, self.t, tb["sqrt_alphas_cumprod"], tb["sqrt_one_minus_alphas_cumprod"],
                              self.x_t, self.v_buf))
        self.target = {"v": self.v_buf, "eps": self.noise, "x0": self.x0}[diff.model_mean_type]
        blocks = net.resblocks_in_order()
        ws_mods = []
        for rb, _ in blocks:
            ws_mods += [rb.block1.proj, rb.block2.proj]
        self.ws_mods = ws_mods
        self.ws_std = {id(m): self.new(*_as2d(m.weight).shape) for m in ws_mods}
        self.dws = {id(m): self.new(*_as2d(m.weight).shape) for m in ws_mods}
        self.ws_t = {id(m): self.new(_as2d(m.weight).shape[1], _as2d(m.weight).shape[0]) for m in ws_mods}
        self._ws_pending = []
        self.emit(be.ws([_as2d(m.weight) for m in ws_mods], [self.ws_std[id(m)] for m in ws_mods]))
        self._fwd_split_at = len(self.fwd)
        for m in ws_mods:
            self._transposes.append((self.ws_std[id(m)], self.ws_t[id(m)]))
            if hasattr(be, "transposed_of"):
                be.transposed_of[self.ws_t[id(m)].data_ptr()] = self.ws_std[id(m)]
        t_blocks = [rb for rb, kind in blocks if kind == "t"]
        c_blocks = [rb for rb, kind in blocks if kind == "c" and rb.mlp is not None]
        t_index = {id(rb): i for i, rb in enumerate(t_blocks)}
        c_index = {id(rb): i for i, rb in enumerate(c_blocks)}
        eng_table = net.time_table.to(self.device)
        eng_freq = net.time_freq.to(self.device)
        temb = H(self.new(B, D), needs_grad=False)
        self.emit(be.time_embedding(self.t, eng_table, eng_freq, temb.t))
        t1 = self.linear(temb, net.time_mlp[1].weight, net.time_mlp[1].bias, act=ACT_GELU)
        t2 = self.linear(t1, net.time_mlp[3].weight, net.time_mlp[3].bias, act=ACT_SILU)
        tw, tgw = fl.packed["t_w"]
        tbias, tgb = fl.packed["t_b"]
        ss_t = H(self.new(B, tw.shape[0]))
        self.emit(be.gemm(t2.t, tw, ss_t.t, tbias))
        dss_t = self.new(B, tw.shape[0])
        ss_t.g = dss_t
        tw_t = self.wT(tw)

        def bw_time_pack():
            self.g_gemm(t2, None, dss_t, tw_t)
            if self.per_block_grads:
                return
            self.tn(t2.t, dss_t, tgw, dbias=tgb, after=lambda: (self.wrote_range(*fl.pack_range["t_w"]),
                                                                 self.wrote_range(*fl.pack_range["t_b"])))
        self._tape.append(bw_time_pack)
        self._t_pack = (t2, dss_t, tgw, tgb)

        ss_c = dss_c = None
        if self.ctx_in is not None and c_blocks:
            cact = self.act(self.ctx_in, ACT_SILU)
            cw, cgw = fl.packed["c_w"]
            cb, cgb = fl.packed["c_b"]
            ss_c = H(self.new(self.ctx_in.t.shape[0], cw.shape[0]))
            self.emit(be.gemm(cact.t, cw, ss_c.t, cb))
            dss_c = self.new(self.ctx_in.t.shape[0], cw.shape[0])
            ss_c.g = dss_c
            cw_t = self.wT(cw)

            def bw_ctx_pack():
                self.g_gemm(cact, None, dss_c, cw_t)
                self.tn(cact.t, dss_c, cgw, dbias=cgb, after=lambda: (self.wrote_range(*fl.pack_range["c_w"]),
                                                                      self.wrote_range(*fl.pack_range["c_b"])))
            self._tape.append(bw_ctx_pack)

        def t_ss(rb):
            i = t_index[id(rb)]
            sl = slice(i * 2 * D, (i + 1) * 2 * D)
            return ss_t.t[:, sl], SS_PER_SCENE, dss_t[:, sl]

        def c_ss(rb):
            if ss_c is None:
                return None, SS_NONE, None
            i = c_index[id(rb)]
            sl = slice(i * 2 * D, (i + 1) * 2 * D)
            return ss_c.t[:, sl], self.ctx_mode, dss_c[:, sl]

        self._post_count = 0

        def post_flush():
            self._post_count += 1
            if self._post_count % 7 == 0:
                self._flush_ws_pending()

        def cblock(rb, a):
            return self.resblock(rb, a, None, c_ss(rb), post=post_flush if self.per_block_grads else None)

        def tb_(rb, a, a2=None):
            post = None
            if self.per_block_grads:
                i = t_index[id(rb)]
                sl = slice(i * 2 * D, (i + 1) * 2 * D)
# ... 169 lines not shown
```

include/diffuscene_hip.h:

```cpp
#ifndef DIFFUSCENE_HIP_H
#define DIFFUSCENE_HIP_H

#include <stdint.h>

#ifdef __cplusplus
extern "C" {
#endif

typedef void* dsc_stream_t;

#define DSC_EINVAL   (-1)
#define DSC_EALIGN   (-2)
#define DSC_ERANGE   (-3)

#define DSC_ACT_NONE 0
#define DSC_ACT_GELU 1
#define DSC_ACT_SILU 2
#define DSC_ACT_LEAKY01 3

#define DSC_SS_NONE      0
#define DSC_SS_PER_TOKEN 1
#define DSC_SS_PER_SCENE 2
#define DSC_SS_PER_SLOT  3
#define DSC_SS_BY_INDEX  4

#define DSC_HEADS    4
#define DSC_DIM_HEAD 32

int dsc_version(void);

typedef struct dsc_gemm_args {
    const float* a1; int64_t lda1; int32_t k1;
    const float* a2; int64_t lda2; int32_t k2;
    const float* w;  int64_t ldw;
    const float* bias;
    const float* residual; int64_t ldr;
    float* y; int64_t ldy;
    int32_t m, n;
    int32_t act_in;
    int32_t act_out;
    int32_t batch; int64_t sa1, sa2, sw, sbias, sres, sy;
    const float* gamma; const float* beta; float eps;
    int32_t tokens_per_scene;
    const float* scale_shift; int64_t ld_ss; int32_t ss_mode;
    float* preact; int64_t ld_preact;
    const int64_t* ss_index;
    const uint16_t* w_planes;
    const float* actgrad_x; int64_t ld_actgrad;
    int32_t ss_rows;
    int32_t w_planes_layout;
    const float* gnb_z; int64_t ld_gnb_z;
    float* gnb_dgamma; float* gnb_dbeta; float* gnb_dbias; int64_t gnb_pstride;
    float* gnb_dss; int64_t ld_gnb_dss;
    int32_t flags;
} dsc_gemm_args;
#define DSC_GEMM_ROW_INVARIANT 1
#define DSC_PLANES_ROWMAJOR 0
#define DSC_PLANES_FRAGMENT 1
#define DSC_PLANES_NONE (-100)

int dsc_gemm_f32(const dsc_gemm_args* args, dsc_stream_t stream);

int dsc_gemm_arithmetic(const dsc_gemm_args* args, int32_t gn);

#define DSC_TILE_GN_32       0
#define DSC_TILE_GN_80_W8    1
#define DSC_TILE_GN_80_W4    2
#define DSC_TILE_GN_48       3
#define DSC_TILE_GN_64       4
#define DSC_TILE_160x256     5
#define DSC_TILE_256x128     6
#define DSC_TILE_128x128     7
#define DSC_TILE_160x128_W4  8
#define DSC_TILE_64x256      9
#define DSC_TILE_WAVE_GN     10
#define DSC_TILE_WAVE_DENSE  11
#define DSC_TILE_WAVE_GN_64  12
int dsc_gemm_split_tile(const dsc_gemm_args* args, int32_t gn);

#define DSC_F32_TILE_160x256 0
#define DSC_F32_TILE_160x128 1
#define DSC_F32_TILE_128x128 2
#define DSC_F32_TILE_96x128  3
#define DSC_F32_TILE_64x64   4
int dsc_gemm_f32_tile(const dsc_gemm_args* args);

int dsc_gemm_planes_layout(const dsc_gemm_args* args, int32_t gn);

int dsc_get_split_wave(void);
int dsc_set_split_wave(int32_t mode);

int dsc_gemm_skinny(const dsc_gemm_args* args, int32_t gn);
int dsc_get_skinny(void);
int dsc_set_skinny(int32_t on);

int dsc_get_gemm_arithmetic(void);
int dsc_set_gemm_arithmetic(int32_t mode);

#define DSC_SPLIT_TRANSPOSE 1
#define DSC_SPLIT_FRAGMENT  2
typedef struct dsc_split_item { const float* w; int64_t ldw; int32_t rows, cols; uint16_t* planes; int32_t transpose; } dsc_split_item;
int dsc_split_bf16x3_f32(const dsc_split_item* items, int32_t count, dsc_stream_t stream);

int dsc_gemm_gn_silu_f32(const dsc_gemm_args* args, dsc_stream_t stream);

int dsc_gemm_splitk_f32(const dsc_gemm_args* a, int32_t splits, float* workspace, int64_t workspace_floats, dsc_stream_t stream);

int dsc_gemm_layernorm_f32(const dsc_gemm_args* a, dsc_stream_t stream);

int dsc_linear_smallk_f32(const float* x, int64_t ldx, int32_t k_in, const float* w, int64_t ldw,
                          const float* bias, float* y, int64_t ldy, int32_t m, int32_t n,
                          int32_t act_out, dsc_stream_t stream);
#define DSC_SMALLK_MAX 4
typedef struct dsc_smallk_item { const float* x; int64_t ldx; int32_t k_in; const float* w; int64_t ldw; const float* bias;
                                 float* y; int64_t ldy; } dsc_smallk_item;
int dsc_linear_smallk_grouped_f32(const dsc_smallk_item* items, int32_t count, int32_t m, int32_t n, int32_t act_out,
                                  dsc_stream_t stream);
typedef struct dsc_col_span { int32_t src_col, dst_col, width; } dsc_col_span;
int dsc_gather_columns_f32(float* dst, int64_t ldd, const float* src, int64_t lds, int32_t rows, const dsc_col_span* spans,
                           int32_t count, dsc_stream_t stream);

#define DSC_WS_MAX 64
typedef struct dsc_ws_item { const float* w; float* out; int32_t rows; int32_t cols; } dsc_ws_item;
int dsc_weight_standardize_f32(const dsc_ws_item* items, int32_t count, float eps, dsc_stream_t stream);

int dsc_layernorm_f32(const float* x, int64_t ldx, const float* g, const float* residual, int64_t ldr,
                      float* y, int64_t ldy, int32_t m, int32_t d, float eps, dsc_stream_t stream);

int dsc_linear_attention_f32(const float* q, int64_t ldq, const float* k, int64_t ldk,
                             const float* v, int64_t ldv, float* out, int64_t ldo,
                             int32_t scenes, int32_t nq, int32_t nk, float scale, dsc_stream_t stream);

int dsc_attention_f32(const float* q, int64_t ldq, const float* k, int64_t ldk,
                      const float* v, int64_t ldv, float* out, int64_t ldo,
                      int32_t scenes, int32_t n, float scale, dsc_stream_t stream);

int dsc_time_embedding_f32(const int64_t* t, int32_t b, int32_t dim, const float* table, int32_t table_rows,
                           const float* freq, float* out, dsc_stream_t stream);

int dsc_activation_f32(const float* x, float* y, int64_t count, int32_t act, dsc_stream_t stream);


int64_t dsc_device_error_count(int32_t reset);

int dsc_q_sample_f32(const float* x0, const float* noise, const int64_t* t,
                     const float* sqrt_ac, const float* sqrt_1mac,
                     float* x_t, float* v_out, int32_t b, int64_t inner, int32_t num_timesteps, dsc_stream_t stream);

#define DSC_MEAN_EPS 0
#define DSC_MEAN_X0  1
#define DSC_MEAN_V   2
int dsc_p_sample_f32(const float* x_t, const float* model_out, const float* noise, const int64_t* t,
                     const float* ca, const float* cb, const float* coef1, const float* coef2,
                     const float* sigma, float* out, float* x0_out ,
                     int32_t mean_type, int32_t clip, int32_t b, int64_t inner, int32_t num_timesteps,
                     dsc_stream_t stream);

int dsc_add_scalar_i64(int64_t* t, int32_t count, int64_t delta, dsc_stream_t stream);

int dsc_ddim_step_f32(const float* x_t, const float* model_out, const float* noise, const int64_t* step,
                      const int64_t* times, const int64_t* times_next, const float* sqrt_alpha_next,
                      const float* c_noise, const float* sigma, const float* ca, const float* cb,
                      const float* sqrt_recip_ac, const float* sqrt_recipm1_ac, float* out, float* x0_out,
                      int32_t mean_type, int32_t b, int64_t inner, int32_t num_steps, int32_t num_timesteps,
                      dsc_stream_t stream);

int dsc_ddim_advance_i64(int64_t* step, const int64_t* times, int64_t* t, int32_t count, int32_t num_steps,
                         dsc_stream_t stream);

int dsc_postfilter_compact_f32(const float* samples, int32_t b, int32_t n, int32_t c, int32_t empty_col, int32_t mode,
                               int32_t keep_empty, float* packed, int32_t* counts, dsc_stream_t stream);

int dsc_complete_overwrite_f32(float* x, const float* partial, const float* noise, const int64_t* t,
                               const float* sqrt_ac, const float* sqrt_1mac,
                               int32_t b, int32_t n, int32_t p, int32_t c, int32_t num_timesteps, dsc_stream_t stream);

int dsc_complete_overwrite_ragged_f32(float* x, const float* partial, const float* noise, const int64_t* counts,
                                      const int64_t* t, const float* sqrt_ac, const float* sqrt_1mac,
                                      int32_t b, int32_t n, int32_t pmax, int32_t c, int32_t num_timesteps, dsc_stream_t stream);

int dsc_p_sample_inpaint_f32(const float* x_t, const float* model_out, const float* noise, const float* partial,
                             const float* noise_p, const int64_t* counts, const int64_t* t, const float* ca, const float* cb,
                             const float* coef1, const float* coef2, const float* sigma, const float* sqrt_ac,
                             const float* sqrt_1mac, float* out, int32_t mean_type, int32_t clip,
                             int32_t b, int32_t n, int32_t pmax, int32_t c, int32_t num_timesteps, dsc_stream_t stream);

int dsc_ddim_inpaint_step_f32(const float* x_t, const float* model_out, const float* noise, const float* partial,
                              const float* noise_p, const int64_t* counts, const int64_t* step, const int64_t* times,
                              const int64_t* times_next, const float* sqrt_alpha_next, const float* c_noise, const float* sigma,
                              const float* ca, const float* cb, const float* sqrt_recip_ac, const float* sqrt_recipm1_ac,
                              const float* sqrt_ac, const float* sqrt_1mac, float* out, int32_t mean_type,
                              int32_t b, int32_t n, int32_t pmax, int32_t c, int32_t num_steps, int32_t num_timesteps,
                              dsc_stream_t stream);

int dsc_masked_overwrite_f32(float* x, const float* known, const float* noise, const uint8_t* mask, const int64_t* t,
                             const float* sqrt_ac, const float* sqrt_1mac, int32_t b, int64_t inner, int32_t num_timesteps,
                             dsc_stream_t stream);

int dsc_p_sample_masked_f32(const float* x_t, const float* model_out, const float* noise, const float* known,
                            const float* noise_k, const uint8_t* mask, const int64_t* t, const float* ca, const float* cb,
                            const float* coef1, const float* coef2, const float* sigma, const float* sqrt_ac,
                            const float* sqrt_1mac, float* out, int32_t mean_type, int32_t clip, int32_t b, int64_t inner,
                            int32_t num_timesteps, dsc_stream_t stream);

int dsc_ddim_masked_step_f32(const float* x_t, const float* model_out, const float* noise, const float* known,
                             const float* noise_k, const uint8_t* mask, const int64_t* step, const int64_t* times,
                             const int64_t* times_next, const float* sqrt_alpha_next, const float* c_noise, const float* sigma,
                             const float* ca, const float* cb, const float* sqrt_recip_ac, const float* sqrt_recipm1_ac,
                             const float* sqrt_ac, const float* sqrt_1mac, float* out, int32_t mean_type,
                             int32_t b, int64_t inner, int32_t num_steps, int32_t num_timesteps, dsc_stream_t stream);

int dsc_cfg_combine_f32(const float* model_out, const float* scale, float* out, int32_t b, int64_t inner, dsc_stream_t stream);

int dsc_p_sample_cfg_f32(const float* x_t, const float* model_out, const float* scale, const float* noise, const int64_t* t,
                         const float* ca, const float* cb, const float* coef1, const float* coef2, const float* sigma,
                         float* out, float* x_dup , float* x0_out , int32_t mean_type,
                         int32_t clip, int32_t b, int64_t inner, int32_t num_timesteps, dsc_stream_t stream);

int dsc_ddim_cfg_step_f32(const float* x_t, const float* model_out, const float* scale, const float* noise, const int64_t* step,
                          const int64_t* times, const int64_t* times_next, const float* sqrt_alpha_next, const float* c_noise,
                          const float* sigma, const float* ca, const float* cb, const float* sqrt_recip_ac,
                          const float* sqrt_recipm1_ac, float* out, float* x_dup , float* x0_out ,
                          int32_t mean_type, int32_t b, int64_t inner, int32_t num_steps, int32_t num_timesteps,
                          dsc_stream_t stream);

int dsc_scene_gate_f32(const float* x, const uint8_t* keep, float* y, int32_t b, int64_t inner, dsc_stream_t stream);

int dsc_scene_randn_f32(float* out, const int64_t* seeds, const int64_t* draw, int64_t stream, int64_t b, int64_t per_scene,
                        dsc_stream_t hip_stream);
int dsc_scene_philox_u32(uint32_t* out, const int64_t* seeds, const int64_t* draw, int64_t stream, int64_t b, int64_t per_scene,
                         dsc_stream_t hip_stream);


int dsc_gemm_tn_f32(const float* a1, int64_t lda1, int32_t k1, const float* a2, int64_t lda2, int32_t k2,
                    const float* dy, int64_t ldd, float* out, int64_t ldo, float* dbias ,
                    int32_t m, int32_t n, int32_t kvalid, float* workspace, int64_t workspace_floats, dsc_stream_t stream);
int64_t dsc_gemm_tn_workspace_floats(int32_t m, int32_t n, int32_t k);

typedef struct dsc_tn_group {
    const float* a1; int64_t lda1; int32_t k1;
    const float* a2; int64_t lda2; int32_t k2;
    const float* dy; int64_t ldd;
    float* out; int64_t ldo;
// ... 133 lines not shown
```

Measured before the change: 63.60 steps/s.

## Fuse linear attention into the to_qkv wave GEMM epilogue

Adds a linear-attention epilogue to the wave-autonomous split-bf16 GEMM. Each wave computes q, k and v for one attention head of one scene, applies the softmax over k, forms the context, and writes the attention output directly. For training it can also store the raw qkv rows needed by backward. This removes a separate linear-attention kernel launch and the qkv round trip through global memory, in both sampling and training. In exchange the epilogue is heavier (LDS staging, shuffles) and only applies when N is in 65..80, with a wave-count occupancy gate.

```diff
diff --git a/__graft_entry__.py b/__graft_entry__.py
--- a/__graft_entry__.py
+++ b/__graft_entry__.py
@@ -35,6 +35,10 @@
     return any(os.path.getmtime(d) > t for d in deps)
 
 
+def _headers():
+    return sorted(os.path.join(CSRC, f) for f in os.listdir(CSRC) if f.endswith(".h")) + [os.path.join(ROOT, "include", "diffuscene_hip.h")]
+
+
 def _stamp_git_head():
     try:
         head = subprocess.check_output(["git", "rev-parse", "--short", "HEAD"], cwd=ROOT, stderr=subprocess.DEVNULL, text=True).strip()
@@ -47,8 +51,7 @@
 
 def build(force=False):
     hipcc = _hipcc()
-    headers = [os.path.join(CSRC, "dsc_common.h"), os.path.join(CSRC, "gemm_core.h"), os.path.join(CSRC, "gemm_tn_split.h"),
-               os.path.join(ROOT, "include", "diffuscene_hip.h")]
+    headers = _headers()
     objs = []
     for src, extra in SOURCES:
         s = os.path.join(CSRC, src)
diff --git a/diffuscene_amd/_lib.py b/diffuscene_amd/_lib.py
--- a/diffuscene_amd/_lib.py
+++ b/diffuscene_amd/_lib.py
@@ -10,7 +10,7 @@
 SS_NONE, SS_PER_TOKEN, SS_PER_SCENE, SS_PER_SLOT, SS_BY_INDEX = 0, 1, 2, 3, 4
 MEAN_EPS, MEAN_X0, MEAN_V = 0, 1, 2
 TILE_GN_80_W8, TILE_GN_80_W4, TILE_160x256, TILE_160x128_W4 = 1, 2, 5, 8
-TILE_WAVE_GN, TILE_WAVE_DENSE, TILE_WAVE_GN_64 = 10, 11, 12
+TILE_WAVE_GN, TILE_WAVE_DENSE, TILE_WAVE_GN_64, TILE_WAVE_LINATTN = 10, 11, 12, 13
 F32_TILE_160x256, F32_TILE_160x128, F32_TILE_128x128, F32_TILE_96x128, F32_TILE_64x64 = 0, 1, 2, 3, 4
 DSC_PLANES_NONE = -100
 GEMM_ROW_INVARIANT = 1
@@ -19,7 +19,8 @@
 STATS_MAX_OBJECTS, STATS_ONE_WAVE_MAX = 160, 32
 
 _ERR = {-1: "DSC_EINVAL (bad shape / null pointer)", -2: "DSC_EALIGN (16-byte alignment required)",
-        -3: "DSC_ERANGE (size outside kernel limits)"}
+        -3: "DSC_ERANGE (size outside kernel limits)",
+        -4: "DSC_ENOTFUSED (the fused epilogue asked for does not run for this launch)"}
 
 c_f32p = C.c_void_p
 c_i64p = C.c_void_p
@@ -51,6 +52,9 @@
         ("gnb_dgamma", C.c_void_p), ("gnb_dbeta", C.c_void_p), ("gnb_dbias", C.c_void_p), ("gnb_pstride", C.c_int64),
         ("gnb_dss", C.c_void_p), ("ld_gnb_dss", C.c_int64),
         ("flags", C.c_int32),
+        ("la_out", C.c_void_p), ("ld_la_out", C.c_int64),
+        ("la_qkv", C.c_void_p), ("ld_la_qkv", C.c_int64),
+        ("la_scale", C.c_float),
     ]
 
 
@@ -106,6 +110,8 @@
     "dsc_gemm_planes_layout": (C.c_int, [C.POINTER(GemmArgs), C.c_int32]),
     "dsc_get_split_wave": (C.c_int, []),
     "dsc_set_split_wave": (C.c_int, [C.c_int32]),
+    "dsc_get_fuse_linattn": (C.c_int, []),
+    "dsc_set_fuse_linattn": (C.c_int, [C.c_int32]),
     "dsc_gemm_skinny": (C.c_int, [C.POINTER(GemmArgs), C.c_int32]),
     "dsc_get_skinny": (C.c_int, []),
     "dsc_set_skinny": (C.c_int, [C.c_int32]),
@@ -255,6 +261,8 @@
         raise ValueError("DSC_TN_FORM=%r: must be '2' (default), '1' or '0'" % os.environ.get("DSC_TN_FORM"))
     if lib.dsc_get_split_wave() < 0:
         raise ValueError("DSC_WAVE=%r: must be '1' / 'auto' (default) or '0'" % os.environ.get("DSC_WAVE"))
+    if lib.dsc_get_fuse_linattn() < 0:
+        raise ValueError("DSC_FUSE_LINATTN=%r: must be '1' (default) or '0'" % os.environ.get("DSC_FUSE_LINATTN"))
     _lib = lib
     return lib
 
@@ -267,12 +275,18 @@
     lib = load()
     if lib.dsc_get_gemm_arithmetic() != 1:
         return 0
-    return (2 if lib.dsc_get_split_wave() == 1 else 1) + 10 * lib.dsc_get_tn_split_form()
+    return (2 if lib.dsc_get_split_wave() == 1 else 1) + 10 * lib.dsc_get_tn_split_form() + 100 * lib.dsc_get_fuse_linattn()
 
 
 def set_split_wave(on):
     prev = load().dsc_get_split_wave() == 1
     check(load().dsc_set_split_wave(1 if on else 0), "dsc_set_split_wave")
+    return prev
+
+
+def set_fuse_linattn(on):
+    prev = load().dsc_get_fuse_linattn() == 1
+    check(load().dsc_set_fuse_linattn(1 if on else 0), "dsc_set_fuse_linattn")
     return prev
 
 
diff --git a/diffuscene_amd/csrc/gemm_mfma.hip b/diffuscene_amd/csrc/gemm_mfma.hip
--- a/diffuscene_amd/csrc/gemm_mfma.hip
+++ b/diffuscene_amd/csrc/gemm_mfma.hip
@@ -8,7 +8,7 @@
 constexpr int BK = 32;
 
 int check_common(const dsc_gemm_args* a) {
-    if (!a || !a->a1 || !a->w || !a->y) return DSC_EINVAL;
+    if (!a || !a->a1 || !a->w || (!a->y && !a->la_out)) return DSC_EINVAL;
     if (a->m <= 0 || a->n <= 0 || a->k1 <= 0 || a->k2 < 0) return DSC_EINVAL;
     if ((a->k1 % BK) || (a->k2 % BK)) return DSC_EINVAL;
     if (a->k2 > 0 && !a->a2) return DSC_EINVAL;
@@ -176,6 +176,7 @@
     hipStream_t s = static_cast<hipStream_t>(stream);
     rc = dsc_gemm_try_split(a, false, s);
     if (rc != DSC_SPLIT_NOT_TAKEN) return rc;
+    if (a->la_out) return DSC_ENOTFUSED;
     if (a->preact || a->actgrad_x || a->gnb_z) return DSC_EINVAL;
     {
         SkinnyPlan sp;
@@ -193,6 +194,7 @@
 extern "C" int dsc_gemm_gn_silu_f32(const dsc_gemm_args* a, dsc_stream_t stream) {
     int rc = check_common(a);
     if (rc) return rc;
+    if (a->la_out) return DSC_ENOTFUSED;
     if (!a->gamma || !a->beta || !a->bias) return DSC_EINVAL;
     const int N = a->tokens_per_scene;
     if (N < 4 || N > 160) return DSC_ERANGE;
@@ -243,6 +245,7 @@
                                    dsc_stream_t stream) {
     int rc = check_common(a);
     if (rc) return rc;
+    if (a->la_out) return DSC_ENOTFUSED;
     if (splits < 2 || splits > 64 || !workspace) return DSC_EINVAL;
     if (a->batch != 1 || a->k2 != 0 || a->act_out != DSC_ACT_NONE) return DSC_EINVAL;
     if (a->k1 % (BK * splits)) return DSC_EINVAL;
@@ -270,6 +273,7 @@
 extern "C" int dsc_gemm_layernorm_f32(const dsc_gemm_args* a, dsc_stream_t stream) {
     int rc = check_common(a);
     if (rc) return rc;
+    if (a->la_out) return DSC_ENOTFUSED;
     if (a->n != 512 || a->batch != 1 || a->act_out != DSC_ACT_NONE || !a->gamma) return DSC_EINVAL;
     if (!dsc_aligned16(a->gamma) || !dsc_aligned16(a->y) || (a->ldy & 3)) return DSC_EALIGN;
     if (a->residual && (!dsc_aligned16(a->residual) || (a->ldr & 3))) return DSC_EALIGN;
diff --git a/diffuscene_amd/csrc/gemm_split.hip b/diffuscene_amd/csrc/gemm_split.hip
--- a/diffuscene_amd/csrc/gemm_split.hip
+++ b/diffuscene_amd/csrc/gemm_split.hip
@@ -422,7 +422,7 @@
 
 }
 
-enum { T_GN_32 = 0, T_GN_80_W8, T_GN_80_W4, T_GN_48, T_GN_64, T_160x256, T_256x128, T_128x128, T_160x128_W4, T_64x256, T_WAVE_GN, T_WAVE_DENSE, T_WAVE_GN_64 };
+enum { T_GN_32 = 0, T_GN_80_W8, T_GN_80_W4, T_GN_48, T_GN_64, T_160x256, T_256x128, T_128x128, T_160x128_W4, T_64x256, T_WAVE_GN, T_WAVE_DENSE, T_WAVE_GN_64, T_WAVE_LINATTN };
 
 static std::atomic<int> g_gemm_arith{-1000};
 
@@ -458,6 +458,37 @@
     if (mode != 0 && mode != 1) return DSC_EINVAL;
     g_split_wave.store(mode, std::memory_order_relaxed);
     return 0;
+}
+
+static std::atomic<int> g_fuse_linattn{-1000};
+
+extern "C" int dsc_get_fuse_linattn(void) {
+    int m = g_fuse_linattn.load(std::memory_order_relaxed);
+    if (m == -1000) {
+        const char* e = getenv("DSC_FUSE_LINATTN");
+        m = (!e || !e[0] || !strcmp(e, "1")) ? 1 : !strcmp(e, "0") ? 0 : DSC_EINVAL;
+        g_fuse_linattn.store(m, std::memory_order_relaxed);
+    }
+    return m;
+}
+
+extern "C" int dsc_set_fuse_linattn(int32_t mode) {
+    if (mode != 0 && mode != 1) return DSC_EINVAL;
+    g_fuse_linattn.store(mode, std::memory_order_relaxed);
+    return 0;
+}
+
+static int select_linattn(const dsc_gemm_args* a, bool gn) {
+    if (dsc_get_split_wave() != 1 || dsc_get_fuse_linattn() != 1) return -1;
+    const int N = a->tokens_per_scene;
+    if (gn || a->batch != 1 || a->n != 3 * DSC_HEADS * DSC_DIM_HEAD || a->k2 != 0 || a->a2 || (a->k1 % 64) || a->k1 < 64) return -1;
+    if (N <= 64 || N > 80 || (a->m % N)) return -1;
+    if (a->bias || a->residual || a->preact || a->actgrad_x || a->gnb_z || a->act_out != DSC_ACT_NONE) return -1;
+    if (!dsc_aligned16(a->la_out) || (a->ld_la_out & 3) || a->ld_la_out < DSC_HEADS * DSC_DIM_HEAD) return -1;
+    if (a->la_qkv && (!dsc_aligned16(a->la_qkv) || (a->ld_la_qkv & 3) || a->ld_la_qkv < a->n)) return -1;
+    if (3LL * a->n * a->k1 * 2 >= 0x7fffffffLL || a->lda1 * 4 * 96 >= 0x7fffffffLL) return -1;
+    const long waves = (long)(a->m / N) * DSC_HEADS, rounds = (waves + 1023) / 1024;
+    return waves * 5 >= rounds * 1024 * 4 ? T_WAVE_LINATTN : -1;
 }
 
 static int select_wave(const dsc_gemm_args* a, bool gn) {
@@ -509,6 +540,7 @@
 static int select_tile(const dsc_gemm_args* a, bool gn, bool assume_planes = false) {
     if (dsc_get_gemm_arithmetic() != 1 || (!assume_planes && !a->w_planes)) return -1;
     if (a->flags & DSC_GEMM_ROW_INVARIANT) return -1;
+    if (a->la_out) return select_linattn(a, gn);
     const int w = select_wave(a, gn);
     return w >= 0 ? w : select_block_tile(a, gn);
 }
@@ -553,11 +585,12 @@
 
 int dsc_gemm_try_split(const dsc_gemm_args* a, bool gn, hipStream_t s) {
     using namespace dsc_split;
-    if (dsc_get_gemm_arithmetic() < 0 || dsc_get_split_wave() < 0) return DSC_EINVAL;
+    if (dsc_get_gemm_arithmetic() < 0 || dsc_get_split_wave() < 0 || dsc_get_fuse_linattn() < 0) return DSC_EINVAL;
     const int N = a->tokens_per_scene;
     const int tile = select_tile(a, gn);
+    if (a->la_out && tile != T_WAVE_LINATTN) return DSC_ENOTFUSED;
     if (tile < 0) return DSC_SPLIT_NOT_TAKEN;
-    const int want = (tile == T_WAVE_GN || tile == T_WAVE_DENSE || tile == T_WAVE_GN_64) ? DSC_PLANES_FRAGMENT : DSC_PLANES_ROWMAJOR;
+    const int want = (tile == T_WAVE_GN || tile == T_WAVE_DENSE || tile == T_WAVE_GN_64 || tile == T_WAVE_LINATTN) ? DSC_PLANES_FRAGMENT : DSC_PLANES_ROWMAJOR;
     if (a->w_planes_layout != want) return DSC_EINVAL;
     switch (tile) {
         case T_GN_32: return launch<true, 4, 2, 2>(a, N, s);
@@ -573,6 +606,7 @@
         case T_WAVE_DENSE:
             if (a->gnb_z) return dsc_wave::launch<false, 5, false, 8, true>(a, a->w_planes, N, s);
             return dsc_wave::launch<false, 5>(a, a->w_planes, 80, s);
+        case T_WAVE_LINATTN: return dsc_wave::launch<false, 5, false, 6, false, true>(a, a->w_planes, N, s);
         case T_WAVE_GN_64:
             return (a->ss_mode == DSC_SS_PER_TOKEN || a->ss_mode == DSC_SS_PER_SLOT) ? dsc_wave::launch<true, 5, true, 4>(a, a->w_planes, N, s)
                                                                                      : dsc_wave::launch<true, 5, false, 4>(a, a->w_planes, N, s);
@@ -603,7 +637,7 @@
 extern "C" int dsc_gemm_planes_layout(const dsc_gemm_args* a, int32_t gn) {
     if (!a || a->m <= 0 || a->n <= 0 || a->k1 <= 0) return DSC_EINVAL;
     const int tile = select_tile(a, gn != 0, true);
-    return tile < 0 ? DSC_PLANES_NONE : (tile == T_WAVE_GN || tile == T_WAVE_DENSE || tile == T_WAVE_GN_64) ? DSC_PLANES_FRAGMENT : DSC_PLANES_ROWMAJOR;
+    return tile < 0 ? DSC_PLANES_NONE : (tile == T_WAVE_GN || tile == T_WAVE_DENSE || tile == T_WAVE_GN_64 || tile == T_WAVE_LINATTN) ? DSC_PLANES_FRAGMENT : DSC_PLANES_ROWMAJOR;
 }
 
 extern "C" int dsc_split_bf16x3_f32(const dsc_split_item* items, int32_t count, dsc_stream_t stream) {
diff --git a/diffuscene_amd/csrc/gemm_split_wave.h b/diffuscene_amd/csrc/gemm_split_wave.h
--- a/diffuscene_amd/csrc/gemm_split_wave.h
+++ b/diffuscene_amd/csrc/gemm_split_wave.h
@@ -49,9 +49,10 @@
 template <int RB>
 constexpr int wave_smem_bytes() { return WAVES * 2 * 3 * (16 * RB) * 64; }
 
-template <bool GN, int RB, bool PERROW = false, int J = 8, bool GB = false>
+template <bool GN, int RB, bool PERROW = false, int J = 8, bool GB = false, bool LA = false>
 __global__ __launch_bounds__(64 * WAVES, 1) void gemm_split_wave_kernel(const dsc_gemm_args p, const uint16_t* const planes_f, const int ntok DSC_WAVE_STAMP_ARGS) {
-    static_assert(J == 8 || J == 4, "wave tile: 128 or 64 channels");
+    static_assert(J == 8 || J == 4 || (LA && J == 6), "wave tile: 128 or 64 channels (96: q, k, v of one attention head)");
+    static_assert(!LA || (!GN && !GB && J == 6 && RB == 5), "the linear-attention epilogue rides on a dense 80 x 96 form");
     static_assert(!GB || (!GN && J == 8), "the GroupNorm-backward epilogue rides on the dense 80 x 128 form");
     constexpr int NWF = 3 * J;
     constexpr int CW = 16 * J;
@@ -96,7 +97,8 @@
     const __amdgpu_buffer_rsrc_t rw = __builtin_amdgcn_make_buffer_rsrc(const_cast<uint16_t*>(planes_f), 0, (int)recw, 0x00020000);
 #endif
     const int plane_bytes = p.batch * p.n * K * 2;
-    const int nb0 = (z * p.n + col0) / 16;
+    const int nb0 = LA ? 2 * ch : (z * p.n + col0) / 16;
+    const int nbh = p.n / 48;
 
     const int q4 = lane & 3, r16 = lane >> 2, g = lane >> 4, l15 = lane & 15;
     const int tvo1 = (r16 * (int)p.lda1 + q4 * 8) * 4, tvo2 = (r16 * (int)p.lda2 + q4 * 8) * 4;
@@ -109,7 +111,7 @@
 #pragma unroll
     for (int j = 0; j < J; ++j) {
         f32x4 b4 = {0.f, 0.f, 0.f, 0.f};
-        if (bias) b4 = *reinterpret_cast<const f32x4*>(bias + col0 + j * 16 + 4 * g);
+        if (!LA && bias) b4 = *reinterpret_cast<const f32x4*>(bias + col0 + j * 16 + 4 * g);
 #pragma unroll
         for (int i = 0; i < RB; ++i) acc[i][j] = b4;
     }
@@ -137,7 +139,7 @@
     };
     auto load_w = [&](int kt, int j, int pl) -> bf16x8 {
 #if defined(__HIP_DEVICE_COMPILE__)
-        return __builtin_bit_cast(bf16x8, __builtin_amdgcn_raw_buffer_load_b128(rw, wvo, pl * plane_bytes + ((nb0 + j) * KT + kt) * 1024, 0));
+        return __builtin_bit_cast(bf16x8, __builtin_amdgcn_raw_buffer_load_b128(rw, wvo, pl * plane_bytes + ((LA ? nb0 + (j >> 1) * nbh + (j & 1) : nb0 + j) * KT + kt) * 1024, 0));
 #else
         (void)kt; (void)j; (void)pl;
         return bf16x8{};
@@ -156,7 +158,7 @@
             constexpr int i = decltype(ic)::value;
             constexpr int NR = 3;
             constexpr int W0 = i * PERW < NWF ? i * PERW : NWF, W1 = (i + 1) * PERW < NWF ? (i + 1) * PERW : NWF;
-            constexpr int VPS = J == 8 ? 2 : 4, NVS = 44 / VPS;
+            constexpr int VPS = J == 4 ? 4 : 2, NVS = 44 / VPS;
             constexpr int S0 = NR + (W1 - W0), S1 = S0 + NVS, S2 = S1 + 3, S3 = S2 + 1;
             static_assert(S3 <= NMMA, "one MFMA per filler slot");
             unsigned su1[4], su2[4], su3[4];
@@ -290,7 +292,184 @@
     };
     constexpr int NQ = ROWS / 4, QH = NQ % 10 == 0 ? 10 : NQ % 8 == 0 ? 8 : NQ % 6 == 0 ? 6 : 4;
     static_assert(NQ % QH == 0, "row groups per pass");
-    if constexpr (GB) {
+    if constexpr (LA) {
+        constexpr int LP = 36;
+        static_assert((2 * ROWS * LP) * 4 <= 2 * STAGE && ROWS * 96 * 4 <= 2 * STAGE, "k + v / the raw rows fit the wave's LDS image");
+        float* const img = reinterpret_cast<float*>(wl);
+        const bool vlast = (RB - 1) * 16 + l15 < rows_here;
+        if (p.la_qkv) {
+#pragma unroll
+            for (int i = 0; i < RB; ++i)
+#pragma unroll
+                for (int j = 0; j < J; ++j) {
+                    const int r = i * 16 + l15;
+                    *reinterpret_cast<f32x4*>(img + r * 96 + (((j * 4 + g) ^ (r & 7)) << 2)) = acc[i][j];
+                }
+            __builtin_amdgcn_wave_barrier();
+            float* const sb = p.la_qkv + (int64_t)row0 * p.ld_la_qkv + 32 * ch;
+            const int c8 = lane & 7, hid = p.n / 3;
+#pragma unroll 2
+            for (int r = lane >> 3; r < rows_here; r += 8) {
+#pragma unroll
+                for (int part = 0; part < 3; ++part) {
+                    const f32x4 v = *reinterpret_cast<const f32x4*>(img + r * 96 + (((part * 8 + c8) ^ (r & 7)) << 2));
+                    *reinterpret_cast<f32x4*>(sb + (int64_t)r * p.ld_la_qkv + part * hid + c8 * 4) = v;
+                }
+            }
+            __builtin_amdgcn_wave_barrier();
+        }
+        const bool hi8 = (l15 & 8) != 0;
+#pragma unroll
+        for (int jb = 2; jb < 4; ++jb)
+#pragma unroll
+            for (int e = 0; e < 4; ++e) {
+                float mx = -INFINITY;
+#pragma unroll
+                for (int i = 0; i < RB; ++i) mx = fmaxf(mx, (i < RB - 1 || vlast) ? acc[i][jb][e] : -INFINITY);
+                mx = fmaxf(mx, __shfl_xor(mx, 1, 64));
+                mx = fmaxf(mx, __shfl_xor(mx, 2, 64));
+                mx = fmaxf(mx, __shfl_xor(mx, 4, 64));
+                mx = fmaxf(mx, __shfl_xor(mx, 8, 64));
+                float ev[RB], pe[RB];
+#pragma unroll
+                for (int i = 0; i < RB; ++i) ev[i] = (i < RB - 1 || vlast) ? expf(acc[i][jb][e] - mx) : 0.f;
+#pragma unroll
+                for (int i = 0; i < RB; ++i) pe[i] = __shfl_xor(ev[i], 8, 64);
+                float sm = 0.f;
+#pragma unroll
+                for (int i = 0; i < RB; ++i) {
+                    sm += hi8 ? pe[i] : ev[i];
+                    sm += hi8 ? ev[i] : pe[i];
+                }
+                sm += __shfl_xor(sm, 1, 64);
+                sm += __shfl_xor(sm, 2, 64);
+                sm += __shfl_xor(sm, 4, 64);
+                const float inv = 1.0f / sm;
+#pragma unroll
+                for (int i = 0; i < RB; ++i) acc[i][jb][e] = ev[i] * inv;
+            }
+        DSC_WAVE_STAMP_KERNEL(3)
+        float* const Ks = img;
+        float* const Vs = img + ROWS * LP;
+#pragma unroll
+        for (int i = 0; i < RB; ++i)
+#pragma unroll
+            for (int jb = 0; jb < 2; ++jb) {
+                const int o = (i * 16 + l15) * LP + jb * 16 + 4 * g;
+                *reinterpret_cast<f32x4*>(Ks + o) = acc[i][2 + jb];
+                *reinterpret_cast<f32x4*>(Vs + o) = acc[i][4 + jb];
+            }
+        __builtin_amdgcn_wave_barrier();
+        const int cd0 = (lane >> 3) * 4, ce0 = (lane & 7) * 4;
+        f32x2 cx[4][2];
+#pragma unroll
+        for (int t = 0; t < 4; ++t) cx[t][0] = cx[t][1] = f32x2{0.f, 0.f};
+        dsc_static_for<RB>([&](auto uc) {
+            constexpr int u = decltype(uc)::value;
+            f32x4 kk[16], vv[16];
+#pragma unroll
+            for (int jj = 0; jj < 16; ++jj) {
+                kk[jj] = *reinterpret_cast<const f32x4*>(Ks + (u * 16 + jj) * LP + cd0);
+                vv[jj] = *reinterpret_cast<const f32x4*>(Vs + (u * 16 + jj) * LP + ce0);
+            }
+#pragma unroll
+            for (int jj = 0; jj < 16; ++jj) {
+                if (u < RB - 1 || u * 16 + jj < rows_here) {
+                    const f32x2 v0 = {vv[jj][0], vv[jj][1]}, v1 = {vv[jj][2], vv[jj][3]};
+#pragma unroll
+                    for (int t = 0; t < 4; ++t) {
+                        const f32x2 kd = {kk[jj][t], kk[jj][t]};
+                        cx[t][0] += kd * v0;
+                        cx[t][1] += kd * v1;
+                    }
+                }
+            }
+        });
+        DSC_WAVE_STAMP_KERNEL(4)
+        __builtin_amdgcn_wave_barrier();
+        float* const ctx = img;
+        float* const Qs = img + 32 * LP;
+#pragma unroll
+        for (int t = 0; t < 4; ++t) *reinterpret_cast<f32x4*>(ctx + (cd0 + t) * LP + ce0) = f32x4{cx[t][0][0], cx[t][0][1], cx[t][1][0], cx[t][1][1]};
+#pragma unroll
+        for (int i = 0; i < RB; ++i)
+#pragma unroll
+            for (int jb = 0; jb < 2; ++jb) *reinterpret_cast<f32x4*>(Qs + (i * 16 + l15) * LP + jb * 16 + 4 * g) = acc[i][jb];
+        __builtin_amdgcn_wave_barrier();
+        const int part = lane & 3, tq = lane >> 2;
+        const float scale = p.la_scale;
+#pragma unroll
+        for (int u = 0; u < RB; ++u) {
+            const int i = u * 16 + tq;
+            const bool ok = i < rows_here;
+            float qv[8];
+            float mx = -INFINITY;
+            if (ok) {
+                const f32x4 a = *reinterpret_cast<const f32x4*>(Qs + i * LP + part * 8);
+                const f32x4 c = *reinterpret_cast<const f32x4*>(Qs + i * LP + part * 8 + 4);
+#pragma unroll
+                for (int e = 0; e < 4; ++e) { qv[e] = a[e]; qv[4 + e] = c[e]; }
+#pragma unroll
+                for (int e = 0; e < 8; ++e) mx = fmaxf(mx, qv[e]);
+            }
+            mx = fmaxf(mx, __shfl_xor(mx, 1, 64));
+            mx = fmaxf(mx, __shfl_xor(mx, 2, 64));
+            float sm = 0.f;
+            if (ok) {
+#pragma unroll
+                for (int e = 0; e < 8; ++e) { qv[e] = expf(qv[e] - mx); sm += qv[e]; }
+            }
+            sm += __shfl_xor(sm, 1, 64);
+            sm += __shfl_xor(sm, 2, 64);
+            if (ok) {
+                const float inv = scale / sm;
+                f32x4 a, c;
+#pragma unroll
+                for (int e = 0; e < 4; ++e) { a[e] = qv[e] * inv; c[e] = qv[4 + e] * inv; }
+                *reinterpret_cast<f32x4*>(Qs + i * LP + part * 8) = a;
+                *reinterpret_cast<f32x4*>(Qs + i * LP + part * 8 + 4) = c;
+            }
+        }
+        __builtin_amdgcn_wave_barrier();
+        f32x2 oo[RB][4];
+#pragma unroll
+        for (int u = 0; u < RB; ++u)
+#pragma unroll
+            for (int h = 0; h < 4; ++h) oo[u][h] = f32x2{0.f, 0.f};
+#pragma unroll
+        for (int d0 = 0; d0 < 32; d0 += 8) {
+            f32x4 qq[RB][2], cc[8][2];
+#pragma unroll
+            for (int u = 0; u < RB; ++u) {
+                qq[u][0] = *reinterpret_cast<const f32x4*>(Qs + (u * 16 + tq) * LP + d0);
+                qq[u][1] = *reinterpret_cast<const f32x4*>(Qs + (u * 16 + tq) * LP + d0 + 4);
+            }
+#pragma unroll
+            for (int dd = 0; dd < 8; ++dd) {
+                cc[dd][0] = *reinterpret_cast<const f32x4*>(ctx + (d0 + dd) * LP + part * 8);
+                cc[dd][1] = *reinterpret_cast<const f32x4*>(ctx + (d0 + dd) * LP + part * 8 + 4);
+            }
+#pragma unroll
+            for (int dd = 0; dd < 8; ++dd)
+#pragma unroll
+                for (int u = 0; u < RB; ++u) {
+                    const float q1 = qq[u][dd >> 2][dd & 3];
+                    const f32x2 qd = {q1, q1};
+#pragma unroll
+                    for (int h = 0; h < 4; ++h) oo[u][h] += f32x2{cc[dd][h >> 1][2 * (h & 1)], cc[dd][h >> 1][2 * (h & 1) + 1]} * qd;
+                }
+        }
+        float* const ob = p.la_out + (int64_t)row0 * p.ld_la_out + 32 * ch + part * 8;
+#pragma unroll
+        for (int u = 0; u < RB; ++u) {
+            const int i = u * 16 + tq;
+            if (i < rows_here) {
+                *reinterpret_cast<f32x4*>(ob + (int64_t)i * p.ld_la_out) = f32x4{oo[u][0][0], oo[u][0][1], oo[u][1][0], oo[u][1][1]};
+                *reinterpret_cast<f32x4*>(ob + (int64_t)i * p.ld_la_out + 4) = f32x4{oo[u][2][0], oo[u][2][1], oo[u][3][0], oo[u][3][1]};
+            }
+        }
+        DSC_WAVE_STAMP_KERNEL(5)
+    } else if constexpr (GB) {
         const float inv_cnt = 1.f / (float)(ntok * 64);
         const bool per_scene = p.ss_mode == DSC_SS_PER_SCENE && p.scale_shift;
 #if defined(__HIP_DEVICE_COMPILE__)
@@ -510,12 +689,12 @@
     DSC_WAVE_STAMP_END
 }
 
-template <bool GN, int RB, bool PERROW = false, int J = 8, bool GB = false>
+template <bool GN, int RB, bool PERROW = false, int J = 8, bool GB = false, bool LA = false>
 int launch(const dsc_gemm_args* a, const uint16_t* planes_f, int ntok, hipStream_t s) {
     const int scenes = (a->m + ntok - 1) / ntok;
     const unsigned grid = (unsigned)(((scenes + WAVES - 1) / WAVES) * (a->n / (16 * J)));
     DSC_CLEAR_STALE_ERROR();
-    hipLaunchKernelGGL((gemm_split_wave_kernel<GN, RB, PERROW, J, GB>), dim3(grid, (unsigned)a->batch), dim3(64 * WAVES), 0, s, *a, planes_f, ntok DSC_WAVE_STAMP_PASS);
+    hipLaunchKernelGGL((gemm_split_wave_kernel<GN, RB, PERROW, J, GB, LA>), dim3(grid, (unsigned)a->batch), dim3(64 * WAVES), 0, s, *a, planes_f, ntok DSC_WAVE_STAMP_PASS);
     DSC_LAUNCH_CHECK();
     return 0;
 }
diff --git a/diffuscene_amd/engine.py b/diffuscene_amd/engine.py
--- a/diffuscene_amd/engine.py
+++ b/diffuscene_amd/engine.py
@@ -190,15 +190,30 @@
         M, B, N = self.M, self.B, self.N
         att = blk.fn.fn
         y = self.layernorm(x, blk.fn.norm.g, self.pool.get(M, D))
-        qkv = self.gemm(y, att.to_qkv.weight, self.pool.get(M, 3 * HID))
+        a = self.pool.get(M, HID)
+        if not self.linattn_fused(y, att, a):
+            qkv = self.gemm(y, att.to_qkv.weight, self.pool.get(M, 3 * HID))
+            self.call("dsc_linear_attention_f32", qkv.data_ptr(), 3 * HID, qkv.data_ptr() + 4 * HID, 3 * HID,
+                      qkv.data_ptr() + 8 * HID, 3 * HID, a.data_ptr(), HID, B, N, N, float(att.scale), keep=(qkv, a))
+            self.pool.put(qkv)
         self.pool.put(y)
-        a = self.pool.get(M, HID)
-        self.call("dsc_linear_attention_f32", qkv.data_ptr(), 3 * HID, qkv.data_ptr() + 4 * HID, 3 * HID,
-                  qkv.data_ptr() + 8 * HID, 3 * HID, a.data_ptr(), HID, B, N, N, float(att.scale), keep=(qkv, a))
-        self.pool.put(qkv)
         out = self.out_proj_ln(a, att.to_out[0], att.to_out[1].g, x)
         self.pool.put(a)
         return out
+
+    def linattn_fused(self, y, att, a):
+        if att.to_qkv.bias is not None:
+            return False
+        w = att.to_qkv.weight
+        g = ops.make_gemm_args(y, w, None, linattn=dict(out=a, scale=float(att.scale), tokens_per_scene=self.N))
+        lay = ops.planes_layout(g)
+        pl = self.eng.planes_of(w, lay) if lay == ops.PLANES_FRAGMENT else None
+        if pl is None:
+            return False
+        ops.attach_planes(g, pl, layout=lay)
+        self.keep.append(_own((g, y, w, a, pl)))
+        self.steps.append((_lib.fn("dsc_gemm_f32"), (C.byref(g),)))
+        return True
 
     def crossattn(self, blk, x):
         M, B, N, L = self.M, self.B, self.N, self.L
diff --git a/diffuscene_amd/ops.py b/diffuscene_amd/ops.py
--- a/diffuscene_amd/ops.py
+++ b/diffuscene_amd/ops.py
@@ -34,7 +34,7 @@
 
 def make_gemm_args(a, w, y, bias=None, a2=None, residual=None, act_in=ACT_NONE, act_out=ACT_NONE,
                    gamma=None, beta=None, eps=1e-5, tokens_per_scene=0, scale_shift=None, ss_mode=SS_NONE, preact=None,
-                   ss_index=None, w_planes=None, actgrad_x=None, gnb=None, row_invariant=False):
+                   ss_index=None, w_planes=None, actgrad_x=None, gnb=None, row_invariant=False, linattn=None):
     g = GemmArgs()
     g.a1, g.lda1 = _mat(a, "a")
     g.k1 = a.shape[1]
@@ -48,9 +48,22 @@
     if w2.shape[1] != g.k1 + g.k2:
         raise RuntimeError("weight K (%d) != activation K (%d)" % (w2.shape[1], g.k1 + g.k2))
     g.m, g.n = a.shape[0], w2.shape[0]
-    g.y, g.ldy = _mat(y, "y")
-    if tuple(y.shape) != (g.m, g.n):
-        raise RuntimeError("output shape %s != (%d, %d)" % (tuple(y.shape), g.m, g.n))
+    if linattn is not None:
+        if y is not None:
+            raise RuntimeError("a launch with the linear-attention epilogue writes linattn['out'] (and linattn['qkv']), not y")
+        g.la_out, g.ld_la_out = _mat(linattn["out"], "linattn out")
+        if tuple(linattn["out"].shape) != (g.m, g.n // 3):
+            raise RuntimeError("linattn out shape %s != (%d, %d)" % (tuple(linattn["out"].shape), g.m, g.n // 3))
+        if linattn.get("qkv") is not None:
+            g.la_qkv, g.ld_la_qkv = _mat(linattn["qkv"], "linattn qkv")
+            if tuple(linattn["qkv"].shape) != (g.m, g.n):
+                raise RuntimeError("linattn qkv shape %s != (%d, %d)" % (tuple(linattn["qkv"].shape), g.m, g.n))
+        g.la_scale = linattn["scale"]
+        g.tokens_per_scene = linattn["tokens_per_scene"]
+    else:
+        g.y, g.ldy = _mat(y, "y")
+        if tuple(y.shape) != (g.m, g.n):
+            raise RuntimeError("output shape %s != (%d, %d)" % (tuple(y.shape), g.m, g.n))
     if bias is not None:
         g.bias = _dev(bias, "bias").data_ptr()
     if residual is not None:
diff --git a/diffuscene_amd/train_plan.py b/diffuscene_amd/train_plan.py
--- a/diffuscene_amd/train_plan.py
+++ b/diffuscene_amd/train_plan.py
@@ -215,6 +215,27 @@
             raise RuntimeError("HipBackend.gemm_gnbwd: planned for a launch the wave-autonomous kernel does not take")
         ops.attach_planes(g, pl, layout=lay)
         return self._call("dsc_gemm_f32", C.byref(g), keep=(g, dy, wt, dz, gn["z"], gn["gamma"], gn["beta"], gn["ss"], gn["dss"], part, pl))
+
+    def _linattn_args(self, a, w, qkv, la):
+        from . import ops
+        return ops.make_gemm_args(a, w, None, linattn=dict(out=la["out"], qkv=qkv, scale=la["scale"], tokens_per_scene=la["tokens_per_scene"]))
+
+    def fuse_linattn_ok(self, a, w, qkv, la):
+        from . import ops
+        if not self.split:
+            return False
+        g = self._linattn_args(a, w, qkv, la)
+        return ops.planes_layout(g) == ops.PLANES_FRAGMENT and self.planes_of(w, a.shape[0], ops.PLANES_FRAGMENT) is not None
+
+    def gemm_linattn(self, a, w, qkv, la):
+        from . import ops
+        g = self._linattn_args(a, w, qkv, la)
+        lay = ops.planes_layout(g)
+        pl = self.planes_of(w, a.shape[0], lay) if lay == ops.PLANES_FRAGMENT else None
+        if pl is None:
+            raise RuntimeError("HipBackend.gemm_linattn: planned for a launch the wave-autonomous kernel does not take")
+        ops.attach_planes(g, pl, layout=lay)
+        return self._call("dsc_gemm_f32", C.byref(g), keep=(g, a, w, qkv, la["out"], pl))
 
     def gemm_long_k(self, a, w, out, residual=None):
         from . import ops
@@ -754,7 +775,7 @@
         self._transposes.append((w2d, buf[:, :n]))
         return buf
 
-    def linear(self, a, weight, bias, a2=None, residual=None, out=None, act_out=ACT_NONE, wt=None, act=None):
+    def linear(self, a, weight, bias, a2=None, residual=None, out=None, act_out=ACT_NONE, wt=None, act=None, linattn=None):
         w2 = _as2d(weight)
         n, K = w2.shape
         rows = a.t.shape[0]
@@ -763,7 +784,10 @@
         assert act_out == ACT_NONE, "training keeps the pre-activation (its backward needs it): use act="
         fused = (act is not None and residual is None and out is None and hasattr(self.be, "fuse_act_ok")
                  and self.be.fuse_act_ok(a.t, w2, y.t, a2.t if a2 is not None else None, bias=bias, preact=y.t))
-        if fused:
+        if linattn is not None:
+            assert bias is None and a2 is None and residual is None and act is None
+            self.emit(self.be.gemm_linattn(a.t, w2, y.t, linattn))
+        elif fused:
             ya_t = self.new(rows, n)
             self.emit(self.be.gemm(a.t, w2, ya_t, bias, a2.t if a2 is not None else None, None, act, preact=y.t))
         else:
@@ -927,10 +951,17 @@
         att = blk.fn.fn
         B, N = self.B, self.N
         y = self.layernorm(a, blk.fn.norm.g)
-        qkv = self.linear(y, att.to_qkv.weight, None)
         o = H(self.new(self.M, HID))
-        q, k, v = qkv.t[:, :HID], qkv.t[:, HID:2 * HID], qkv.t[:, 2 * HID:]
-        self.emit(self.be.linattn(q, k, v, o.t, B, N, N, float(att.scale)))
+        buf = self.new(self.M, 3 * HID)
+        la = dict(out=o.t, scale=float(att.scale), tokens_per_scene=N)
+        fuse = getattr(self.be, "fuse_linattn_ok", None)
+        if fuse is not None and att.to_qkv.bias is None and fuse(y.t, _as2d(att.to_qkv.weight), buf, la):
+            qkv = self.linear(y, att.to_qkv.weight, None, out=buf, linattn=la)
+            q, k, v = qkv.t[:, :HID], qkv.t[:, HID:2 * HID], qkv.t[:, 2 * HID:]
+        else:
+            qkv = self.linear(y, att.to_qkv.weight, None, out=buf)
+            q, k, v = qkv.t[:, :HID], qkv.t[:, HID:2 * HID], qkv.t[:, 2 * HID:]
+            self.emit(self.be.linattn(q, k, v, o.t, B, N, N, float(att.scale)))
 
         def bw():
             if o.g is None:
diff --git a/include/diffuscene_hip.h b/include/diffuscene_hip.h
--- a/include/diffuscene_hip.h
+++ b/include/diffuscene_hip.h
@@ -11,6 +11,7 @@
 
 #define DSC_EINVAL   (-1)
 #define DSC_EALIGN   (-2)
+#define DSC_ENOTFUSED (-4)
 #define DSC_ERANGE   (-3)
 
 #define DSC_ACT_NONE 0
@@ -53,6 +54,9 @@
     float* gnb_dgamma; float* gnb_dbeta; float* gnb_dbias; int64_t gnb_pstride;
     float* gnb_dss; int64_t ld_gnb_dss;
     int32_t flags;
+    float* la_out; int64_t ld_la_out;
+    float* la_qkv; int64_t ld_la_qkv;
+    float la_scale;
 } dsc_gemm_args;
 #define DSC_GEMM_ROW_INVARIANT 1
 #define DSC_PLANES_ROWMAJOR 0
@@ -76,6 +80,7 @@
 #define DSC_TILE_WAVE_GN     10
 #define DSC_TILE_WAVE_DENSE  11
 #define DSC_TILE_WAVE_GN_64  12
+#define DSC_TILE_WAVE_LINATTN 13
 int dsc_gemm_split_tile(const dsc_gemm_args* args, int32_t gn);
 
 #define DSC_F32_TILE_160x256 0
@@ -89,6 +94,9 @@
 
 int dsc_get_split_wave(void);
 int dsc_set_split_wave(int32_t mode);
+
+int dsc_get_fuse_linattn(void);
+int dsc_set_fuse_linattn(int32_t mode);
 
 int dsc_gemm_skinny(const dsc_gemm_args* args, int32_t gn);
 int dsc_get_skinny(void);
```

New measurement: 64.08 steps/s (median of 6 runs). About the same (+0.8%).
